# kenm-28/Semilayer-Wise-Mixed-Precision-Quantization

Hardware: NVIDIA B200
Metric: ResNet-50 mixed 8/4-bit images/s (higher is better)
Workload: dtype u8

## Files before the change

include/slq.h:

```cpp
#ifndef SLQ_H_
#define SLQ_H_

#include <stdint.h>

#ifdef __cplusplus
extern "C" {
#endif

#define SLQ_ABI_VERSION 1

#if defined(__GNUC__)
#define SLQ_API __attribute__((visibility("default")))
#else
#define SLQ_API
#endif

#define SLQ_OK 0
#define SLQ_ERR_INVALID 1
#define SLQ_ERR_CUDA 2
#define SLQ_ERR_ZERO_RANGE 3
#define SLQ_ERR_UNSUPPORTED 4

#define SLQ_ROW_OK 0
#define SLQ_ROW_ZERO_RANGE 1
#define SLQ_ROW_CODE_RANGE 2

#define SLQ_DIV_TRUE 0
#define SLQ_DIV_RECIP 1

SLQ_API const char *slq_last_error(void);
SLQ_API int slq_abi_version(void);
SLQ_API int slq_device_info(int32_t *sm_count, int32_t *cc_major, int32_t *cc_minor);


SLQ_API int64_t slq_packed_row_bytes(int64_t K, int32_t bit);

SLQ_API int slq_quantize_rows(float *w, int64_t n_rows, int64_t K, const int32_t *rows, const int32_t *bits,
                      int32_t n_jobs, int32_t div_mode, int32_t write_back, uint8_t *codes,
                      const int64_t *code_offsets, int32_t *z, float *s32, int32_t *status,
                      void *stream);

SLQ_API int slq_quantize_rows_host(float *w, int64_t n_rows, int64_t K, const int32_t *rows,
                           const int32_t *bits, int32_t n_jobs, int32_t div_mode, int32_t write_back,
                           uint8_t *codes, const int64_t *code_offsets, int32_t *z, float *s32,
                           int32_t *status);

typedef struct slq_qjob {
  float *row;
  uint8_t *codes;
  int32_t K;
  int32_t bit;
} slq_qjob;
SLQ_API int slq_quantize_jobs(const slq_qjob *jobs, int32_t n_small, int32_t n_mid, int32_t n_large,
                              int32_t div_mode, int32_t write_back, int32_t *z, float *s32, int32_t *status,
                              void *stream);

SLQ_API int slq_decode_rows(const uint8_t *codes, const int64_t *code_offsets, const int32_t *bit,
                            const int32_t *z, const float *s, int64_t n_rows, int64_t K, float *w, void *stream);

SLQ_API int slq_classify_rows(const float *w, int64_t n_rows, int64_t K, int32_t *bit, int32_t *z, float *s,
                      int32_t *exact, void *stream);

SLQ_API int slq_encode_rows(const float *w, int64_t n_rows, int64_t K, const int32_t *bit, const int32_t *z,
                    const float *s, uint8_t *codes, const int64_t *code_offsets, void *stream);


#define SLQ_IMPL_UMMA 0
#define SLQ_IMPL_SIMT 1

#define SLQ_A_AUTO 0
#define SLQ_A_IM2COL 1
#define SLQ_A_TILED 2

#define SLQ_OUT_U8 0
#define SLQ_OUT_F32 1
#define SLQ_OUT_ACC 2
#define SLQ_OUT_S8 3

typedef struct slq_conv_desc {
  int32_t N, H, W, Cin;
  int32_t Cout, kh, kw, stride, pad;
  int32_t w16;
  int32_t impl;
  int32_t a_mode;
} slq_conv_desc;

typedef struct slq_conv slq_conv;

SLQ_API int64_t slq_gemm_weight_rows(const slq_conv_desc *d);

SLQ_API int slq_build_gemm_weights(const slq_conv_desc *d, const uint8_t *codes, const int64_t *code_offsets,
                           const int32_t *bit, uint8_t *wg, void *stream);

SLQ_API int slq_conv_create(const slq_conv_desc *d, const uint8_t *in, const uint8_t *wg, slq_conv **out);

SLQ_API int slq_conv_tiling(const slq_conv_desc *d, int32_t *bn_cols, int32_t *n_tiles, int32_t *k_block,
                            int32_t *num_kb, int32_t *resident);
SLQ_API int slq_build_packed_gemm_weights(const slq_conv_desc *d, const uint8_t *codes, const int64_t *code_offsets,
                                          const int32_t *bit, const int64_t *tile_base, const int32_t *seg_bytes,
                                          const uint16_t *row_offsets, uint8_t *wgp, void *stream);
SLQ_API int slq_conv_set_packed_weights(slq_conv *c, const uint8_t *wgp, const int64_t *tile_base,
                                        const int32_t *seg_bytes, const uint16_t *row_offsets);
SLQ_API void slq_conv_destroy(slq_conv *c);

typedef struct slq_epilogue {
  const float *wscale;
  const float *zf;
  const float *bias;
  const float *act_scales;
  int32_t in_id, out_id, res_id;
  const uint8_t *res;
  int32_t res_signed;
  void *out;
  int32_t *out_S;
  int32_t out_mode;
  int32_t relu;
  const uint32_t *in_rowsum;
  uint32_t *out_rowsum;
  int32_t in_planes;
  int64_t in_plane_stride;
} slq_epilogue;

SLQ_API int slq_debug_set_trace(int64_t *buf, int32_t capacity_events);

SLQ_API int32_t slq_conv_rowsum_planes(const slq_conv *c, int32_t has_residual);
SLQ_API int32_t slq_conv_needs_rowsum(const slq_conv *c, int32_t has_residual);

SLQ_API int slq_conv_launch(slq_conv *c, const slq_epilogue *e, void *stream);

typedef struct slq_blocktail_desc {
  int32_t N, H, W, Cin;
  int32_t stride;
  int32_t Cmid;
  int32_t Cout;
  int32_t impl;
} slq_blocktail_desc;

typedef struct slq_blocktail slq_blocktail;

typedef struct slq_blocktail_epilogue {
  const float *wscale3, *zf3, *bias3;
  const float *wscaled, *zfd, *biasd;
  const float *act_scales;
  int32_t in3_id, ind_id, out_id;
  void *out;
  int32_t out_mode;
  uint32_t *out_rowsum;
} slq_blocktail_epilogue;

SLQ_API int slq_blocktail_create(const slq_blocktail_desc *d, const uint8_t *y2, const uint8_t *x, const uint8_t *wg3,
                                 const uint8_t *wgd, slq_blocktail **out);
SLQ_API void slq_blocktail_destroy(slq_blocktail *h);
SLQ_API int32_t slq_blocktail_rowsum_planes(const slq_blocktail *h);
SLQ_API int slq_blocktail_launch(slq_blocktail *h, const slq_blocktail_epilogue *e, void *stream);


SLQ_API int slq_stem_forward(const float *x, int32_t N, int32_t H, int32_t W, const float *w,
                     const float *bn_a, const float *bn_b, const float *act_scales, int32_t out_id,
                     float *scratch, void *out, int32_t out_mode, uint32_t *out_rowsum, void *stream);

typedef struct slq_stem slq_stem;
SLQ_API int64_t slq_stem_workspace_bytes(int32_t N, int32_t H, int32_t W);
SLQ_API int slq_stem_create(int32_t N, int32_t H, int32_t W, void *workspace, slq_stem **out);
SLQ_API void slq_stem_destroy(slq_stem *s);
SLQ_API int slq_stem_set_weights(slq_stem *s, const float *w, void *stream);
SLQ_API int slq_stem_launch(slq_stem *s, const float *x, const float *bn_a, const float *bn_b,
                            const float *act_scales, int32_t out_id, void *out, int32_t out_mode,
                            float *f32_scratch, uint32_t *out_rowsum, void *stream);
#define SLQ_IN_F32 0
#define SLQ_IN_F16 1
#define SLQ_IN_U8 2
SLQ_API int slq_stem_launch_in(slq_stem *s, const void *x, int32_t in_kind, const float *norm,
                               const float *bn_a, const float *bn_b, const float *act_scales, int32_t out_id,
                               void *out, int32_t out_mode, float *f32_scratch, uint32_t *out_rowsum, void *stream);

SLQ_API int64_t slq_tail_workspace_bytes(int32_t N, int32_t C, int32_t O);
SLQ_API int slq_tail_split_weights(const float *fc_w, int32_t O, int32_t C, float *fc_w_split, void *stream);
SLQ_API int slq_tail_forward(const uint8_t *x, int32_t N, int32_t HW, int32_t C, const float *act_scales,
                     int32_t in_id, const float *fc_w_split, const float *fc_b, int32_t O, float *workspace,
                     float *logits, void *stream);

SLQ_API int slq_absmax_scale(const float *y, int64_t n, float *act_scales, int32_t id, int32_t qmax,
                     uint32_t *tmp, void *stream);
SLQ_API int slq_quantize_act(const float *y, int64_t n, const float *act_scales, int32_t id,
                     int32_t is_signed, uint8_t *out, void *stream);


SLQ_API int slq_eval_tail(const float *logits, const int64_t *labels, int32_t B, int32_t C, float *probs_out,
                          const float *ref_probs, float *rows, double *accum, void *stream);
SLQ_API int slq_kl_rows(const float *p, const float *q, int32_t B, int32_t C, float *rows, double *accum,
                        void *stream);


SLQ_API int slq_probe_i8_peak(int32_t iters, int64_t *ops_out, void *stream);

#ifdef __cplusplus
}
#endif
#endif
```

semilayer-wise-mixed-precision-quantization_b200/csrc/block_tail.cu:

```cuda
#include <algorithm>
#include <new>

#include "conv_common.cuh"
#include "umma_ptx.cuh"

struct slq_blocktail {
  slq_blocktail_desc d;
  int Ho, Wo, swz, k3_blocks, kd_blocks, stages, smem_bytes, grid, n_tiles;
  long long M;
  const uint8_t *y2, *x, *wg3, *wgd;
  CUtensorMap tmA3, tmAd, tmB3, tmBd, tmO;
  const void *out_ptr;
};

namespace slq {

constexpr int kBtThreads = 640;
constexpr int kBtCrew = 512;
constexpr int kBtStage = 3;
constexpr int kBtN3 = 80;
constexpr int kBtNd = 144;
constexpr int kBtAccCols = 256;
constexpr int kBtMaxStages = 4;

struct BtArgs {
  long long M;
  int N, H, W, Ho, Wo, stride, Cin, Cmid, Cout;
  int k3_blocks, kd_blocks, stages, m_tiles, n_tiles, d_im2col;
  int b3_off, bd_off, ring_off, out_off, prm_off, bar_off;
  const float *wscale3, *zf3, *bias3, *wscaled, *zfd, *biasd, *act_scales;
  int in3_id, ind_id, out_id, out_mode;
  void *out;
  uint32_t *out_rowsum;
  long long *stats;
  int dbg;
};
#define BT_DBG(a) (kDebugTrace ? (a).dbg : 0)
__device__ __forceinline__ void bt_wait(uint32_t bar, uint32_t parity, long long *acc, bool on) {
  if (!kDebugTrace || !on) { mbar_wait(bar, parity); return; }
  const long long t0 = clock64();
  mbar_wait(bar, parity);
  *acc += clock64() - t0;
}

struct BtChan { float a3, z3, ad, zd, b; };
__host__ __device__ inline BtChan bt_chan(float wscale3, float zf3, float bias3, float wscaled, float zfd, float biasd,
                                          float s_y2, float s_x, float inv, bool quantised) {
  BtChan c;
#ifdef __CUDA_ARCH__
  c.a3 = __fmul_rn(wscale3, s_y2);
  c.ad = __fmul_rn(wscaled, s_x);
  c.b = __fadd_rn(bias3, biasd);
  if (quantised) { c.a3 = __fmul_rn(c.a3, inv); c.ad = __fmul_rn(c.ad, inv); c.b = __fmul_rn(c.b, inv); }
  c.z3 = __fmul_rn(zf3, c.a3);
  c.zd = __fmul_rn(zfd, c.ad);
#else
  c.a3 = wscale3 * s_y2; c.ad = wscaled * s_x; c.b = bias3 + biasd;
  if (quantised) { c.a3 *= inv; c.ad *= inv; c.b *= inv; }
  c.z3 = zf3 * c.a3; c.zd = zfd * c.ad;
#endif
  return c;
}

template <int SWZ, int OUT>
__global__ void __launch_bounds__(kBtThreads, 1)
block_tail_kernel(const __grid_constant__ CUtensorMap tmA3, const __grid_constant__ CUtensorMap tmAd,
                  const __grid_constant__ CUtensorMap tmB3, const __grid_constant__ CUtensorMap tmBd,
                  const __grid_constant__ CUtensorMap tmO, const BtArgs a) {
  extern __shared__ uint8_t smem_raw[];
  const uint32_t smem_base = (smem_u32(smem_raw) + 1023u) & ~1023u;
  uint8_t *smem = smem_raw + (smem_base - smem_u32(smem_raw));
  constexpr int kABytes = kTileM * SWZ;
  const uint32_t bar_base = smem_base + a.bar_off;
  auto full_bar = [&](int p, int s) { return bar_base + 8u * (p * 2 * kBtMaxStages + s); };
  auto empty_bar = [&](int p, int s) { return bar_base + 8u * (p * 2 * kBtMaxStages + kBtMaxStages + s); };
  auto tfull_bar = [&](int p) { return bar_base + 8u * (4 * kBtMaxStages + p); };
  auto tempty_bar = [&](int p) { return bar_base + 8u * (4 * kBtMaxStages + 2 + p); };
  const uint32_t bfull_bar = bar_base + 8u * (4 * kBtMaxStages + 4);
  volatile uint32_t *tmem_slot = reinterpret_cast<volatile uint32_t *>(smem + a.bar_off + 8 * (4 * kBtMaxStages + 5));
  const int warp = __shfl_sync(0xffffffffu, (int)(threadIdx.x >> 5), 0), lane = threadIdx.x & 31;

  const int per_n = (int)gridDim.x / a.n_tiles;
  const int my_n = (int)blockIdx.x % a.n_tiles;
  const int first_m = (int)blockIdx.x / a.n_tiles;
  const int count = first_m < a.m_tiles ? (a.m_tiles - first_m + per_n - 1) / per_n : 0;
  const int kb_tile = a.k3_blocks + a.kd_blocks;

  asm volatile("griddepcontrol.launch_dependents;" ::: "memory");
  if (warp == 0 && lane == 0) {
    prefetch_tmap(&tmA3); prefetch_tmap(&tmAd); prefetch_tmap(&tmB3); prefetch_tmap(&tmBd);
    if (OUT == SLQ_OUT_U8) prefetch_tmap(&tmO);
  }
  if (warp == 1 && lane == 0) {
    for (int p = 0; p < 2; ++p) {
      for (int s = 0; s < a.stages; ++s) { mbar_init(full_bar(p, s), 1); mbar_init(empty_bar(p, s), 1); }
      mbar_init(tfull_bar(p), 1);
      mbar_init(tempty_bar(p), kBtCrew / 32);
    }
    mbar_init(bfull_bar, 1);
    fence_barrier_init();
  }
  if (warp == 2) {
    asm volatile("tcgen05.alloc.cta_group::1.sync.aligned.shared::cta.b32 [%0], %1;" ::"r"(
                     smem_u32((const void *)tmem_slot)), "r"(512) : "memory");
    asm volatile("tcgen05.relinquish_alloc_permit.cta_group::1.sync.aligned;" ::: "memory");
  }
  for (int i = threadIdx.x; i < kb_tile * 16 * (SWZ / 16); i += blockDim.x) {
    const int t = i / (16 * (SWZ / 16)), rem = i % (16 * (SWZ / 16));
    const int row = rem / (SWZ / 16), chunk = rem % (SWZ / 16);
    const uint4 v = row == 0 ? make_uint4(0x01010101u, 0x01010101u, 0x01010101u, 0x01010101u) : make_uint4(0, 0, 0, 0);
    const int base = t < a.k3_blocks ? a.b3_off + t * (kBtN3 * SWZ) + 64 * SWZ
                                     : a.bd_off + (t - a.k3_blocks) * (kBtNd * SWZ) + 128 * SWZ;
    *reinterpret_cast<uint4 *>(smem + base + row * SWZ + chunk * 16) = v;
  }
  fence_proxy_async_smem();
  tc_fence_before();
  __syncthreads();
  tc_fence_after();
  const uint32_t tmem_base = *tmem_slot;

  if (warp == 0 || warp == 2) {
    const int p = warp >> 1;
    if (p == 0 && count > 0) {
      if (elect_one()) {
        mbar_expect_tx(bfull_bar, (uint32_t)(a.k3_blocks * 64 * SWZ + a.kd_blocks * 128 * SWZ));
        for (int kb = 0; kb < a.k3_blocks; ++kb)
          tma_load_2d(smem_base + a.b3_off + kb * (kBtN3 * SWZ), &tmB3, bfull_bar, kb * SWZ, my_n * 64);
        for (int kb = 0; kb < a.kd_blocks; ++kb)
          tma_load_2d(smem_base + a.bd_off + kb * (kBtNd * SWZ), &tmBd, bfull_bar, kb * SWZ, my_n * 128);
      }
      __syncwarp();
    }
    grid_dependency_wait();
    int c = 0;
    long long w_empty = 0;
    const bool st_on = kDebugTrace && a.stats != nullptr && blockIdx.x == 0;
    const long long t_begin = clock64();
    for (int i = p; i < count; i += 2) {
      const int m0 = (first_m + i * per_n) * kTileM;
      int dn = 0, dh = 0, dw = 0;
      if (a.d_im2col) {
        const int hw = a.Ho * a.Wo;
        dn = m0 / hw;
        const int rem = m0 - dn * hw, ph = rem / a.Wo;
        dh = ph * a.stride;
        dw = (rem - ph * a.Wo) * a.stride;
      }
      for (int kb = 0; kb < kb_tile; ++kb, ++c) {
        const int s = c % a.stages;
        bt_wait(empty_bar(p, s), (uint32_t)(((c / a.stages) & 1) ^ 1), &w_empty, st_on);
        if (elect_one()) {
          const uint32_t dst = smem_base + a.ring_off + (p * a.stages + s) * kABytes;
          mbar_expect_tx(full_bar(p, s), kABytes);
          if (kb < a.k3_blocks) tma_load_2d(dst, &tmA3, full_bar(p, s), kb * SWZ, m0);
          else if (a.d_im2col) tma_load_im2col_4d(dst, &tmAd, full_bar(p, s), (kb - a.k3_blocks) * SWZ, dw, dh, dn, 0, 0);
          else tma_load_2d(dst, &tmAd, full_bar(p, s), (kb - a.k3_blocks) * SWZ, m0);
        }
        __syncwarp();
      }
    }
    if (st_on && lane == 0) { a.stats[p] = w_empty; a.stats[2 + p] = clock64() - t_begin; }
  } else if (warp == 1 || warp == 3) {
    const int p = warp >> 1;
    const uint32_t tmem_u = __shfl_sync(0xffffffffu, tmem_base, 0) + p * kBtAccCols;
    const uint32_t idesc3 = (2u << 4) | ((uint32_t)(kBtN3 >> 3) << 17) | ((uint32_t)(kTileM >> 4) << 24);
    const uint32_t idescd = (2u << 4) | ((uint32_t)(kBtNd >> 3) << 17) | ((uint32_t)(kTileM >> 4) << 24);
    if (count > p) {
      mbar_wait(bfull_bar, 0);
      tc_fence_after();
    }
    int c = 0, t = 0;
    long long w_full = 0, w_tempty = 0;
    const bool st_on = kDebugTrace && a.stats != nullptr && blockIdx.x == 0;
    const long long t_begin = clock64();
    for (int i = p; i < count; i += 2, ++t) {
      if (t >= 1) bt_wait(tempty_bar(p), (uint32_t)((t - 1) & 1), &w_tempty, st_on);
      tc_fence_after();
      for (int kb = 0; kb < kb_tile; ++kb, ++c) {
        const int s = c % a.stages;
        bt_wait(full_bar(p, s), (uint32_t)((c / a.stages) & 1), &w_full, st_on);
        tc_fence_after();
        if (elect_one()) {
          const uint64_t da = make_smem_desc<SWZ>(smem_base + a.ring_off + (p * a.stages + s) * kABytes);
          const bool is3 = kb < a.k3_blocks;
          const uint64_t db = make_smem_desc<SWZ>(smem_base + (is3 ? a.b3_off + kb * (kBtN3 * SWZ)
                                                                   : a.bd_off + (kb - a.k3_blocks) * (kBtNd * SWZ)));
          const bool first = is3 ? kb == 0 : kb == a.k3_blocks;
#pragma unroll
          for (int k = 0; k < SWZ / 32 && !(!is3 && (BT_DBG(a) & 8)); ++k)
            umma_i8(tmem_u + (is3 ? 0 : kBtN3), da + 2 * k, db + 2 * k, is3 ? idesc3 : idescd, (uint32_t)(!first || k != 0));
          umma_commit(empty_bar(p, s));
          if (kb == kb_tile - 1) umma_commit(tfull_bar(p));
        }
        __syncwarp();
      }
    }
    if (st_on && lane == 0) { a.stats[4 + p] = w_full; a.stats[6 + p] = w_tempty; a.stats[8 + p] = clock64() - t_begin; }
  } else if (warp >= 4) {
    grid_dependency_wait();
    const int slice = (warp - 4) >> 2;
    const int wq = warp & 3;
    const int et = threadIdx.x - 128;
    const int row = wq * 32 + lane;
    constexpr bool kQuant = OUT == SLQ_OUT_U8;
    float *prm = reinterpret_cast<float *>(smem + a.prm_off);
    const uint32_t prm_s = smem_base + a.prm_off + (uint32_t)slice * 64;
    volatile uint32_t *rs_base = reinterpret_cast<volatile uint32_t *>(smem + a.prm_off + 5 * 64 * 4);
    const uint32_t row_byte = (uint32_t)(row * 64), row_sw = (uint32_t)((row >> 1) & 3);
    if (et < 64) {
      const int oc = my_n * 64 + et;
      const float inv = kQuant ? __fdiv_rn(1.0f, a.act_scales[a.out_id]) : 1.0f;
      const BtChan c = bt_chan(a.wscale3[oc], a.zf3[oc], a.bias3[oc], a.wscaled[oc], a.zfd[oc], a.biasd[oc],
                               a.act_scales[a.in3_id], a.act_scales[a.ind_id], inv, kQuant);
      prm[et] = c.a3; prm[64 + et] = c.z3; prm[128 + et] = c.ad; prm[192 + et] = c.zd; prm[256 + et] = c.b;
    }
    named_bar_sync(1, kBtCrew);
    const uint32_t tlane = tmem_base + ((uint32_t)(wq * 32) << 16);
    const int c0 = slice * 16;
    const bool want_rs = kQuant && a.out_rowsum != nullptr;
    long long w_tfull = 0, w_bar = 0, seg[6] = {0, 0, 0, 0, 0, 0}, tseg = 0;
#define BT_SEG(k) do { if (st_on) { const long long now__ = clock64(); seg[k] += now__ - tseg; tseg = now__; } } while (0)
    const bool st_on = kDebugTrace && a.stats != nullptr && blockIdx.x == 0 && et == 0;
    const long long t_begin = clock64();
    for (int i = 0; i < count; ++i) {
      const int p = i & 1, t = i >> 1;
      const int m_tile = first_m + i * per_n;
      const long long m = (long long)m_tile * kTileM + row;
      const bool valid = m < a.M;
      const uint32_t tcol = tlane + p * kBtAccCols;
      bt_wait(tfull_bar(p), (uint32_t)(t & 1), &w_tfull, st_on);
      if (st_on) tseg = clock64();
      tc_fence_after();
      uint32_t a3[16], lo[16], hi[16];
      tmem_ld16(tcol + c0, a3);
      if (!(BT_DBG(a) & 2)) {
        tmem_ld16(tcol + kBtN3 + c0, lo);
        tmem_ld16(tcol + kBtN3 + 64 + c0, hi);
      } else {
#pragma unroll
        for (int j = 0; j < 16; ++j) { lo[j] = a3[(j + 1) & 15]; hi[j] = a3[(j + 2) & 15]; }
      }
      const float S3 = (float)(int)tmem_ld1(tcol + 64);
      const float Sd = (float)(int)tmem_ld1(tcol + kBtN3 + 128);
      tmem_ld_wait();
      BT_SEG(0);
      tc_fence_before();
      __syncwarp();
      if (lane == 0) mbar_arrive(tempty_bar(p));
      BT_SEG(1);
      uint32_t pk[4];
      float *of = reinterpret_cast<float *>(a.out) + m * a.Cout + my_n * 64 + c0;
#pragma unroll
      for (int q4 = 0; q4 < 4; ++q4) {
        const uint32_t pofs = prm_s + (uint32_t)q4 * 16;
        uint4 pa3, pz3, pad, pzd, pb;
        if (!(BT_DBG(a) & 1)) {
          pa3 = lds128(pofs); pz3 = lds128(pofs + 256); pad = lds128(pofs + 512); pzd = lds128(pofs + 768); pb = lds128(pofs + 1024);
        } else {
          pa3 = pz3 = pad = pzd = pb = make_uint4(0x3a000000u + q4, 0x3a100000u, 0x3a200000u, 0x3a300000u);
        }
        const uint32_t va3[4] = {pa3.x, pa3.y, pa3.z, pa3.w}, vz3[4] = {pz3.x, pz3.y, pz3.z, pz3.w};
        const uint32_t vad[4] = {pad.x, pad.y, pad.z, pad.w}, vzd[4] = {pzd.x, pzd.y, pzd.z, pzd.w};
        const uint32_t vb[4] = {pb.x, pb.y, pb.z, pb.w};
        float v[4];
#pragma unroll
        for (int b = 0; b < 4; b += 2) {
          const int j = 4 * q4 + b;
          const float2 f3 = make_float2((float)(int)a3[j], (float)(int)a3[j + 1]);
          const float2 fd = ffma2(make_float2((float)(int)hi[j], (float)(int)hi[j + 1]), make_float2(256.0f, 256.0f),
                                  make_float2((float)(int)lo[j], (float)(int)lo[j + 1]));
          float2 y = ffma2(make_float2(S3, S3), make_float2(__uint_as_float(vz3[b]), __uint_as_float(vz3[b + 1])),
                           make_float2(__uint_as_float(vb[b]), __uint_as_float(vb[b + 1])));
          y = ffma2(make_float2(Sd, Sd), make_float2(__uint_as_float(vzd[b]), __uint_as_float(vzd[b + 1])), y);
          y = ffma2(f3, make_float2(__uint_as_float(va3[b]), __uint_as_float(va3[b + 1])), y);
          y = ffma2(fd, make_float2(__uint_as_float(vad[b]), __uint_as_float(vad[b + 1])), y);
          v[b] = y.x; v[b + 1] = y.y;
        }
        if (BT_DBG(a) & 32) { v[0] = __uint_as_float(a3[4 * q4] ^ lo[4 * q4]); v[1] = v[2] = v[3] = __uint_as_float(hi[4 * q4]); }
        if (!kQuant) {
          if (valid) reinterpret_cast<float4 *>(of)[q4] = make_float4(fmaxf(v[0], 0.f), fmaxf(v[1], 0.f), fmaxf(v[2], 0.f), fmaxf(v[3], 0.f));
        } else {
          pk[q4] = epi_pack4<false>(v[0], v[1], v[2], v[3]);
        }
      }
      if (kQuant) {
        const uint32_t stg = smem_base + a.out_off + (uint32_t)(i % kBtStage) * (kTileM * 64);
        if (!(BT_DBG(a) & 4)) sts128(stg + row_byte + (((uint32_t)slice ^ row_sw) << 4), make_uint4(pk[0], pk[1], pk[2], pk[3]));
        else if ((pk[0] ^ pk[1] ^ pk[2] ^ pk[3]) == 0x12345679u) sts128(stg, make_uint4(pk[0], pk[1], pk[2], pk[3]));
        uint32_t rsum = 0;
        volatile uint32_t *rs_scratch = rs_base + (i & 1) * 384;
        if (want_rs) {
          rsum = __dp4a(pk[0], 0x01010101u, __dp4a(pk[1], 0x01010101u, __dp4a(pk[2], 0x01010101u, __dp4a(pk[3], 0x01010101u, 0u))));
          if (slice != 0) rs_scratch[(slice - 1) * 128 + row] = rsum;
        }
        BT_SEG(2);
        fence_proxy_async_smem();
        BT_SEG(3);
        const long long tb0 = st_on ? clock64() : 0;
        named_bar_sync(1, kBtCrew);
        if (st_on) w_bar += clock64() - tb0;
        BT_SEG(4);
        if (et == 0 && !(BT_DBG(a) & 4)) {
          tma_store_2d(&tmO, stg, my_n * 64, m_tile * kTileM);
          tma_store_commit();
          asm volatile("cp.async.bulk.wait_group.read 1;" ::: "memory");
        }
        if (want_rs && slice == 0) {
          if (valid) a.out_rowsum[(long long)my_n * a.M + m] = rsum + rs_scratch[row] + rs_scratch[128 + row] + rs_scratch[256 + row];
        }
        BT_SEG(5);
      }
    }
    if (st_on) {
      a.stats[10] = w_tfull; a.stats[11] = w_bar; a.stats[12] = clock64() - t_begin; a.stats[13] = count;
      for (int k = 0; k < 6; ++k) a.stats[16 + k] = seg[k];
    }
    if (kQuant && et == 0) tma_store_wait_all();
  }
  tc_fence_before();
  __syncthreads();
  if (warp == 2) {
    tc_fence_after();
    asm volatile("tcgen05.dealloc.cta_group::1.sync.aligned.b32 %0, %1;" ::"r"(tmem_base), "r"(512) : "memory");
  }
}

__global__ void __launch_bounds__(128) block_tail_simt_kernel(BtArgs a, const uint8_t *__restrict__ y2,
                                                              const uint8_t *__restrict__ x,
                                                              const uint8_t *__restrict__ wg3,
                                                              const uint8_t *__restrict__ wgd) {
  const int oc = blockIdx.y * 32 + (threadIdx.x & 31);
  const long long m = (long long)blockIdx.x * 4 + (threadIdx.x >> 5);
  if (m >= a.M || oc >= a.Cout) return;
  const int wo = (int)(m % a.Wo), ho = (int)((m / a.Wo) % a.Ho), n = (int)(m / ((long long)a.Wo * a.Ho));
  unsigned acc3 = 0, S3 = 0, lo = 0, hi = 0, Sd = 0;
  const uint32_t *yp = reinterpret_cast<const uint32_t *>(y2 + m * a.Cmid);
  const uint32_t *w3 = reinterpret_cast<const uint32_t *>(wg3 + (long long)oc * a.Cmid);
  for (int c4 = 0; c4 < a.Cmid / 4; ++c4) {
    const uint32_t v = __ldg(yp + c4);
    acc3 = __dp4a(v, __ldg(w3 + c4), acc3);
    S3 = __dp4a(v, 0x01010101u, S3);
  }
  const uint32_t *xp = reinterpret_cast<const uint32_t *>(x + (((long long)n * a.H + ho * a.stride) * a.W + wo * a.stride) * a.Cin);
  const uint32_t *wl = reinterpret_cast<const uint32_t *>(wgd + (long long)gemm_row_of(oc, 0, 1) * a.Cin);
  const uint32_t *wh = reinterpret_cast<const uint32_t *>(wgd + (long long)gemm_row_of(oc, 1, 1) * a.Cin);
  for (int c4 = 0; c4 < a.Cin / 4; ++c4) {
    const uint32_t v = __ldg(xp + c4);
    lo = __dp4a(v, __ldg(wl + c4), lo);
    hi = __dp4a(v, __ldg(wh + c4), hi);
    Sd = __dp4a(v, 0x01010101u, Sd);
  }
  const bool quantised = a.out_mode == SLQ_OUT_U8;
  const float inv = quantised ? __fdiv_rn(1.0f, a.act_scales[a.out_id]) : 1.0f;
  const BtChan c = bt_chan(a.wscale3[oc], a.zf3[oc], a.bias3[oc], a.wscaled[oc], a.zfd[oc], a.biasd[oc],
                           a.act_scales[a.in3_id], a.act_scales[a.ind_id], inv, quantised);
  const float fd = __fmaf_rn((float)(int)hi, 256.0f, (float)(int)lo);
  float y = __fmaf_rn((float)(int)S3, c.z3, c.b);
  y = __fmaf_rn((float)(int)Sd, c.zd, y);
  y = __fmaf_rn((float)(int)acc3, c.a3, y);
  y = __fmaf_rn(fd, c.ad, y);
  if (quantised) reinterpret_cast<uint8_t *>(a.out)[m * a.Cout + oc] = (uint8_t)epi_quant_u8(y);
  else reinterpret_cast<float *>(a.out)[m * a.Cout + oc] = fmaxf(y, 0.f);
}

typedef CUresult (*BtEncodeTiledFn)(CUtensorMap *, CUtensorMapDataType, cuuint32_t, void *, const cuuint64_t *,
                                    const cuuint64_t *, const cuuint32_t *, const cuuint32_t *, CUtensorMapInterleave,
                                    CUtensorMapSwizzle, CUtensorMapL2promotion, CUtensorMapFloatOOBfill);
typedef CUresult (*BtEncodeIm2colFn)(CUtensorMap *, CUtensorMapDataType, cuuint32_t, void *, const cuuint64_t *,
                                     const cuuint64_t *, const int *, const int *, cuuint32_t, cuuint32_t,
                                     const cuuint32_t *, CUtensorMapInterleave, CUtensorMapSwizzle,
                                     CUtensorMapL2promotion, CUtensorMapFloatOOBfill);

static int bt_encoders(BtEncodeTiledFn *tiled, BtEncodeIm2colFn *im2col) {
  static BtEncodeTiledFn f_tiled = nullptr;
  static BtEncodeIm2colFn f_im2col = nullptr;
  if (!f_tiled || !f_im2col) {
    void *p = nullptr;
    cudaDriverEntryPointQueryResult qr;
    SLQ_CUDA(cudaGetDriverEntryPoint("cuTensorMapEncodeTiled", &p, cudaEnableDefault, &qr));
    SLQ_CHECK_ARG(qr == cudaDriverEntryPointSuccess && p, "cuTensorMapEncodeTiled not available from the driver");
    f_tiled = (BtEncodeTiledFn)p;
    p = nullptr;
    SLQ_CUDA(cudaGetDriverEntryPoint("cuTensorMapEncodeIm2col", &p, cudaEnableDefault, &qr));
    SLQ_CHECK_ARG(qr == cudaDriverEntryPointSuccess && p, "cuTensorMapEncodeIm2col not available from the driver");
    f_im2col = (BtEncodeIm2colFn)p;
  }
  *tiled = f_tiled;
  *im2col = f_im2col;
  return SLQ_OK;
}

static int bt_tiled_u8(CUtensorMap *tm, const void *ptr, long long rows, int cols, int box_cols, int box_rows,
                       CUtensorMapSwizzle sw, const char *what) {
  BtEncodeTiledFn enc;
  BtEncodeIm2colFn enc2;
  int rc = bt_encoders(&enc, &enc2);
  if (rc != SLQ_OK) return rc;
  cuuint64_t dims[2] = {(cuuint64_t)cols, (cuuint64_t)rows};
  cuuint64_t strides[1] = {(cuuint64_t)cols};
  cuuint32_t box[2] = {(cuuint32_t)box_cols, (cuuint32_t)box_rows};
  cuuint32_t es[2] = {1, 1};
  const CUresult r = enc(tm, CU_TENSOR_MAP_DATA_TYPE_UINT8, 2, const_cast<void *>(ptr), dims, strides, box, es,
                         CU_TENSOR_MAP_INTERLEAVE_NONE, sw, CU_TENSOR_MAP_L2_PROMOTION_L2_256B, CU_TENSOR_MAP_FLOAT_OOB_FILL_NONE);
  if (r != CUDA_SUCCESS) {
    set_error("cuTensorMapEncodeTiled(%s) failed: CUresult %d", what, (int)r);
    return SLQ_ERR_CUDA;
  }
  return SLQ_OK;
}

template <int SWZ, int OUT>
static int bt_launch(slq_blocktail *h, const BtArgs &a, cudaStream_t st) {
  static bool attr_done[kMaxDevices] = {false};
  const int dev = current_device();
  if (dev >= kMaxDevices || !attr_done[dev]) {
    SLQ_CUDA(cudaFuncSetAttribute(block_tail_kernel<SWZ, OUT>, cudaFuncAttributeMaxDynamicSharedMemorySize, 232448));
    if (dev < kMaxDevices) attr_done[dev] = true;
  }
  cudaLaunchConfig_t cfg = {};
  cfg.gridDim = dim3((unsigned)h->grid);
  cfg.blockDim = dim3(kBtThreads);
  cfg.dynamicSmemBytes = (size_t)h->smem_bytes;
  cfg.stream = st;
  cudaLaunchAttribute attr[1];
  attr[0].id = cudaLaunchAttributeProgrammaticStreamSerialization;
  attr[0].val.programmaticStreamSerializationAllowed = 1;
  cfg.attrs = attr;
  cfg.numAttrs = 1;
  SLQ_CUDA(cudaLaunchKernelEx(&cfg, block_tail_kernel<SWZ, OUT>, h->tmA3, h->tmAd, h->tmB3, h->tmBd, h->tmO, a));
  return SLQ_OK;
}

}

using namespace slq;

static int bt_plan(const slq_blocktail_desc *d, int swz, int *stages, int off[6]) {
  const int k3 = d->Cmid / swz, kd = d->Cin / swz;
  const int b3 = k3 * kBtN3 * swz, bd = kd * kBtNd * swz;
  const int fixed = b3 + bd + kBtStage * kTileM * 64 + (5 * 64 * 4 + 2 * 3 * 128 * 4) + 512 + 1024;
  const int a_bytes = kTileM * swz;
  int st = std::min(kBtMaxStages, (232448 - fixed) / (2 * a_bytes));
  if (st < 2) return -1;
  *stages = st;
  off[0] = 0;
  off[1] = b3;
  off[2] = b3 + bd;
  off[3] = off[2] + 2 * st * a_bytes;
  off[4] = off[3] + kBtStage * kTileM * 64;
  off[5] = off[4] + 5 * 64 * 4 + 2 * 3 * 128 * 4;
  return 1024 + off[5] + 512;
}

extern "C" int slq_blocktail_create(const slq_blocktail_desc *d, const uint8_t *y2, const uint8_t *x, const uint8_t *wg3,
                                    const uint8_t *wgd, slq_blocktail **out) {
  SLQ_CHECK_ARG(d && y2 && x && wg3 && wgd && out, "slq_blocktail_create: null pointer argument");
  SLQ_CHECK_ARG(d->N > 0 && d->H > 0 && d->W > 0 && (d->stride == 1 || d->stride == 2), "slq_blocktail_create: bad shape");
  SLQ_CHECK_ARG(d->Cin % 64 == 0 && d->Cmid % 64 == 0 && d->Cout % 64 == 0 && d->Cin > 0 && d->Cmid > 0 && d->Cout > 0,
                "slq_blocktail_create: channel counts must be multiples of 64");
  SLQ_CHECK_ARG(d->impl == SLQ_IMPL_UMMA || d->impl == SLQ_IMPL_SIMT, "slq_blocktail_create: impl %d", d->impl);
  const int swz = (d->Cmid % 128 == 0 && d->Cin % 128 == 0) ? 128 : 64;
  int stages = 0, off[6];
  const int smem = bt_plan(d, swz, &stages, off);
  if (smem < 0) {
    set_error("slq_blocktail_create: the weights of one n-tile (Cmid %d, Cin %d) do not fit in shared memory", d->Cmid, d->Cin);
    return SLQ_ERR_UNSUPPORTED;
  }
  slq_blocktail *h = new (std::nothrow) slq_blocktail();
  SLQ_CHECK_ARG(h != nullptr, "slq_blocktail_create: out of host memory");
  h->d = *d;
  h->Ho = (d->H - 1) / d->stride + 1;
  h->Wo = (d->W - 1) / d->stride + 1;
  h->M = (long long)d->N * h->Ho * h->Wo;
  h->swz = swz;
  h->k3_blocks = d->Cmid / swz;
  h->kd_blocks = d->Cin / swz;
  h->stages = stages;
  h->smem_bytes = smem;
  h->n_tiles = d->Cout / 64;
  h->y2 = y2; h->x = x; h->wg3 = wg3; h->wgd = wgd;
  h->out_ptr = nullptr;
  const long long m_tiles = ceil_div(h->M, kTileM);
  h->grid = (int)(std::min<long long>(std::max(sm_count() / h->n_tiles, 1), m_tiles)) * h->n_tiles;
  if (d->impl == SLQ_IMPL_UMMA) {
    const CUtensorMapSwizzle sw = swz == 128 ? CU_TENSOR_MAP_SWIZZLE_128B : CU_TENSOR_MAP_SWIZZLE_64B;
    int rc = bt_tiled_u8(&h->tmA3, y2, h->M, d->Cmid, swz, kTileM, sw, "y2");
    if (rc == SLQ_OK) rc = bt_tiled_u8(&h->tmB3, wg3, d->Cout, d->Cmid, swz, 64, sw, "W3");
    if (rc == SLQ_OK) rc = bt_tiled_u8(&h->tmBd, wgd, (long long)h->n_tiles * 128, d->Cin, swz, 128, sw, "Wd");
    if (rc == SLQ_OK) {
      if (d->stride == 1) {
        rc = bt_tiled_u8(&h->tmAd, x, h->M, d->Cin, swz, kTileM, sw, "x");
      } else {
        BtEncodeTiledFn enc;
        BtEncodeIm2colFn enc2;
        rc = bt_encoders(&enc, &enc2);
        if (rc == SLQ_OK) {
          cuuint64_t dims[4] = {(cuuint64_t)d->Cin, (cuuint64_t)d->W, (cuuint64_t)d->H, (cuuint64_t)d->N};
          cuuint64_t strides[3] = {(cuuint64_t)d->Cin, (cuuint64_t)d->W * d->Cin, (cuuint64_t)d->H * d->W * d->Cin};
          int lower[2] = {0, 0}, upper[2] = {0, 0};
          cuuint32_t es[4] = {1, (cuuint32_t)d->stride, (cuuint32_t)d->stride, 1};
          const CUresult r = enc2(&h->tmAd, CU_TENSOR_MAP_DATA_TYPE_UINT8, 4, const_cast<uint8_t *>(x), dims, strides, lower, upper,
                                  (cuuint32_t)swz, (cuuint32_t)kTileM, es, CU_TENSOR_MAP_INTERLEAVE_NONE, sw,
                                  CU_TENSOR_MAP_L2_PROMOTION_L2_256B, CU_TENSOR_MAP_FLOAT_OOB_FILL_NONE);
          if (r != CUDA_SUCCESS) {
            set_error("cuTensorMapEncodeIm2col(x) failed: CUresult %d", (int)r);
            rc = SLQ_ERR_CUDA;
          }
          int drv = 0;
          if (rc == SLQ_OK && cudaDriverGetVersion(&drv) == cudaSuccess && drv <= 13010 &&
              (long long)d->N * d->H * d->W * d->Cin < 131072)
            reinterpret_cast<uint64_t *>(&h->tmAd)[1] &= ~(1ull << 21);
        }
      }
    }
    if (rc != SLQ_OK) {
      delete h;
      return rc;
    }
    h->tmO = h->tmB3;
  }
  *out = h;
  return SLQ_OK;
}

extern "C" void slq_blocktail_destroy(slq_blocktail *h) { delete h; }

extern "C" int32_t slq_blocktail_rowsum_planes(const slq_blocktail *h) {
  return (h && h->d.impl == SLQ_IMPL_UMMA) ? h->n_tiles : 0;
}

extern "C" int slq_blocktail_launch(slq_blocktail *h, const slq_blocktail_epilogue *e, void *stream) {
  SLQ_CHECK_ARG(h && e, "slq_blocktail_launch: null handle/epilogue");
  SLQ_CHECK_ARG(e->wscale3 && e->zf3 && e->bias3 && e->wscaled && e->zfd && e->biasd && e->act_scales && e->out,
                "slq_blocktail_launch: epilogue vectors missing");
  SLQ_CHECK_ARG(e->out_mode == SLQ_OUT_U8 || e->out_mode == SLQ_OUT_F32, "slq_blocktail_launch: out_mode %d", e->out_mode);
  SLQ_CHECK_ARG(reinterpret_cast<uintptr_t>(e->out) % 16 == 0, "slq_blocktail_launch: out must be 16-byte aligned");
  const slq_blocktail_desc &d = h->d;
  BtArgs a{};
  a.M = h->M; a.N = d.N; a.H = d.H; a.W = d.W; a.Ho = h->Ho; a.Wo = h->Wo; a.stride = d.stride;
  a.Cin = d.Cin; a.Cmid = d.Cmid; a.Cout = d.Cout;
  a.k3_blocks = h->k3_blocks; a.kd_blocks = h->kd_blocks; a.stages = h->stages;
  a.m_tiles = (int)ceil_div(h->M, kTileM); a.n_tiles = h->n_tiles; a.d_im2col = d.stride != 1;
  a.wscale3 = e->wscale3; a.zf3 = e->zf3; a.bias3 = e->bias3; a.wscaled = e->wscaled; a.zfd = e->zfd; a.biasd = e->biasd;
  a.act_scales = e->act_scales; a.in3_id = e->in3_id; a.ind_id = e->ind_id; a.out_id = e->out_id; a.out_mode = e->out_mode;
  a.out = e->out; a.out_rowsum = e->out_mode == SLQ_OUT_U8 ? e->out_rowsum : nullptr;
  a.dbg = 0;
  a.stats = nullptr;
#if SLQ_DEBUG_TRACE
  {
    int cap = 0;
    debug_trace_buffer(&a.stats, &cap);
    if (cap > -16) a.stats = nullptr;
  }
  if (const char *d = getenv("SLQ_BT_DBG")) a.dbg = atoi(d);
#endif
  cudaStream_t st = (cudaStream_t)stream;
  if (d.impl == SLQ_IMPL_SIMT) {
    dim3 grid((unsigned)ceil_div(h->M, 4), (unsigned)ceil_div(d.Cout, 32));
    block_tail_simt_kernel<<<grid, 128, 0, st>>>(a, h->y2, h->x, h->wg3, h->wgd);
    SLQ_LAUNCH_CHECK();
    return SLQ_OK;
  }
  int stages = 0, off[6];
  bt_plan(&d, h->swz, &stages, off);
  a.b3_off = off[0]; a.bd_off = off[1]; a.ring_off = off[2]; a.out_off = off[3]; a.prm_off = off[4]; a.bar_off = off[5];
  if (e->out_mode == SLQ_OUT_U8 && h->out_ptr != e->out) {
    int rc = bt_tiled_u8(&h->tmO, e->out, h->M, d.Cout, 64, kTileM, CU_TENSOR_MAP_SWIZZLE_64B, "out");
    if (rc != SLQ_OK) return rc;
    h->out_ptr = e->out;
  }
  if (h->swz == 128)
    return e->out_mode == SLQ_OUT_U8 ? bt_launch<128, SLQ_OUT_U8>(h, a, st) : bt_launch<128, SLQ_OUT_F32>(h, a, st);
  return e->out_mode == SLQ_OUT_U8 ? bt_launch<64, SLQ_OUT_U8>(h, a, st) : bt_launch<64, SLQ_OUT_F32>(h, a, st);
}
```

semilayer-wise-mixed-precision-quantization_b200/csrc/conv_common.cuh:

```cuda
#pragma once
#include <cuda.h>

#include "common.cuh"
#include "epilogue.cuh"

namespace slq {

constexpr int kTileM = 128;

struct ConvGeom {
  int N, H, W, Cin, Cout, kh, kw, stride, pad;
  int Ho, Wo, w16;
  int bn_ch;
  int bn_cols;
  int n_tiles;
  int gemm_rows;
  long long M;
  int Ktot;
};

inline ConvGeom make_geom(const slq_conv_desc &d, int wide = 0) {
  ConvGeom g{};
  g.N = d.N; g.H = d.H; g.W = d.W; g.Cin = d.Cin; g.Cout = d.Cout;
  g.kh = d.kh; g.kw = d.kw; g.stride = d.stride; g.pad = d.pad; g.w16 = d.w16 ? 1 : 0;
  g.Ho = (d.H + 2 * d.pad - d.kh) / d.stride + 1;
  g.Wo = (d.W + 2 * d.pad - d.kw) / d.stride + 1;
  g.bn_ch = g.w16 ? 64 : (d.Cout > 64 ? 128 : 64);
  if (wide && !g.w16 && d.Cout % 256 == 0) g.bn_ch = 256;
  g.bn_cols = g.w16 ? 128 : g.bn_ch;
  g.n_tiles = (d.Cout + g.bn_ch - 1) / g.bn_ch;
  g.gemm_rows = g.n_tiles * g.bn_cols;
  g.M = (long long)d.N * g.Ho * g.Wo;
  g.Ktot = d.kh * d.kw * d.Cin;
  return g;
}

__host__ __device__ inline int gemm_row_of(int oc, int limb, int w16) {
  return w16 ? ((oc >> 6) * 128 + limb * 64 + (oc & 63)) : oc;
}

int validate_desc(const slq_conv_desc *d);

void debug_trace_buffer(long long **buf, int *cap);

int launch_conv_simt(const ConvGeom &g, const uint8_t *in, const uint8_t *wg, const EpiDev &e,
                     cudaStream_t st);

int launch_stem_pool(const float *y, int N, int Hc, int Wc, int Hp, int Wp, const float *act_scales,
                     int out_id, void *out, int out_mode, uint32_t *out_rowsum, cudaStream_t st);

}

struct slq_conv {
  slq_conv_desc desc;
  slq::ConvGeom g;
  slq::ConvGeom g_wide;
  int wide_ok;
  CUtensorMap tmB_wide;
  const uint8_t *wgp;
  const long long *wgp_tile;
  const int *wgp_seg;
  const uint16_t *wgp_rowoff;
  const uint8_t *in;
  const uint8_t *wg;
  int a_im2col;
  int swizzle;
  CUtensorMap tmA;
  CUtensorMap tmB;
  CUtensorMap tmO;
  CUtensorMap tmR;
  const void *out_ptr;
  const void *res_ptr;
  int num_ctas;
  int smem_bytes;
};
```

semilayer-wise-mixed-precision-quantization_b200/csrc/conv_umma.cu:

```cuda
#include <algorithm>
#include <cstdlib>
#include <new>

#include "conv_common.cuh"
#include "umma_ptx.cuh"

namespace slq {

constexpr int kThreads = 640;
constexpr int kTeam = 256;
inline int out_tile_bytes(const ConvGeom &g) {
#ifdef SLQ_OUT_TILE_16K
  return kTileM * 128;
#endif
  return kTileM * (g.bn_ch < 128 ? g.bn_ch : 128);
}

constexpr int kMaxStages = 8;
constexpr int kSmemLimit = 232448;

struct SmemPlan {
  int stages;
  int stage_bytes;
  int group;
  int a_bytes;
  int b_tile_bytes;
  int b_resident;
  int mma_warps;
  int b_off;
  int res_bufs;
  int out_bufs;
  int out_tile;
  int out_off, res_off, prm_off, bar_off;
  int total;
};

constexpr int kMaxResBufs = 4;
constexpr int kPrmBytes = 2 * 3 * 256 * 4 + 4 * 128 * 4;
constexpr int kMaxGroup = 4;

inline SmemPlan make_plan(const ConvGeom &g, int swz, bool has_res) {
  SmemPlan p{};
  p.a_bytes = kTileM * swz;
  const int kOutTileBytes = p.out_tile = out_tile_bytes(g);
  p.b_tile_bytes = (g.bn_cols + (g.bn_cols < 256 ? 16 : 0)) * swz;
  const int num_kb = g.Ktot / swz;
  const long long b_all = (long long)num_kb * p.b_tile_bytes;
#if SLQ_DEBUG_TRACE
  static const int force_group = getenv("SLQ_GROUP") ? atoi(getenv("SLQ_GROUP")) : 0;
  static const int force_mma = getenv("SLQ_MMA_WARPS") ? atoi(getenv("SLQ_MMA_WARPS")) : 0;
#else
  constexpr int force_group = 0, force_mma = 0;
#endif
  p.stages = 0;
  for (int rb = has_res ? kMaxResBufs : 0; g.bn_ch != 256 && p.stages == 0 && rb >= (has_res ? 2 : 0); rb -= 2) {
    const int fixed = (2 + rb) * kOutTileBytes + kPrmBytes + 512 + 1024;
    const long long room = (long long)kSmemLimit - fixed - b_all;
    for (int grp = std::min(kMaxGroup, num_kb); grp >= 1; --grp) {
      if (num_kb % grp != 0 || (force_group && grp > force_group)) continue;
      const int st = (int)std::min<long long>(kMaxStages, room / ((long long)grp * p.a_bytes)) & ~1;
      if (st >= (grp == 1 ? 4 : 4)) {
        p.b_resident = 1; p.group = grp; p.stages = st; p.stage_bytes = grp * p.a_bytes; p.res_bufs = rb; p.out_bufs = 2;
        const int st4 = (int)std::min<long long>(kMaxStages, (room - 2 * kOutTileBytes) / ((long long)grp * p.a_bytes)) & ~1;
        if (st4 >= st || (has_res && st4 >= 4)) { p.out_bufs = 4; p.stages = st4; }
        break;
      }
    }
    if (!has_res) break;
  }
  if (p.stages == 0) {
    p.res_bufs = has_res ? kMaxResBufs : 0;
    p.out_bufs = g.bn_ch == 256 ? 0 : 1;
    const int fixed = (p.out_bufs + p.res_bufs) * kOutTileBytes + kPrmBytes + 512 + 1024;
    p.b_resident = 0;
    p.group = 1;
    p.stage_bytes = p.a_bytes + p.b_tile_bytes;
    p.stages = std::min(kMaxStages, (kSmemLimit - fixed) / p.stage_bytes) & ~1;
  }
  p.mma_warps = force_mma ? force_mma : 2;
  p.b_off = p.stages * p.stage_bytes;
  p.out_off = p.b_off + (p.b_resident ? (int)b_all : 0);
  p.res_off = p.out_off + p.out_bufs * kOutTileBytes;
  p.prm_off = p.res_off + p.res_bufs * kOutTileBytes;
  p.bar_off = p.prm_off + kPrmBytes;
  p.total = 1024 + p.bar_off + 512;
  return p;
}

inline int plan_grid(const ConvGeom &g, const SmemPlan &p, int sms) {
  const long long m_tiles = (g.M + kTileM - 1) / kTileM;
  if (p.b_resident) {
    const int per_n = (int)std::min<long long>(std::max(sms / g.n_tiles, 1), m_tiles);
    return per_n * g.n_tiles;
  }
  return (int)std::min<long long>(m_tiles * g.n_tiles, sms);
}

struct KernelArgs {
  ConvGeom g;
  EpiDev e;
  SmemPlan sp;
  int a_im2col;
  int num_kb;
  int num_grp;
  int chunks_per_tap;
  int tma_out;
  int mma_warps_per_tile;
  int tile_alt;
  int acc_bufs, acc_stride;
  const uint8_t *wgp;
  const long long *wgp_tile;
  const int *wgp_seg;
  const uint16_t *wgp_rowoff;
  long long m_tiles;
  int half_b;
  long long *trace;
  int trace_cap;
};

constexpr int kTraceIssuers = 24;
__device__ __forceinline__ void mbar_wait_stat(uint32_t bar, uint32_t parity, long long &sum, bool stats) {
  if (!kDebugTrace || !stats) { mbar_wait(bar, parity); return; }
  const long long t0 = clock64();
  mbar_wait(bar, parity);
  sum += clock64() - t0;
}
__device__ __forceinline__ void trace_ev(const KernelArgs &a, int issuer, int &n, int ev, int idx) {
  if (!kDebugTrace || a.trace == nullptr || a.trace_cap < 0 || blockIdx.x != 0) return;
  const int per = a.trace_cap / kTraceIssuers;
  if (n < per) {
    long long *p = a.trace + 3LL * (issuer * per + n);
    p[0] = ev + 1;
    p[1] = idx;
    p[2] = clock64();
    ++n;
  }
}

struct TileWalk {
  int count, first_m, step_m;
  int first, step;
  int n_tiles, fixed_n, my_n;
  __device__ TileWalk(const KernelArgs &a) {
    n_tiles = a.g.n_tiles;
    fixed_n = a.sp.b_resident;
    const int m_tiles = (int)a.m_tiles;
    if (fixed_n) {
      const int per_n = (int)gridDim.x / n_tiles;
      my_n = (int)blockIdx.x % n_tiles;
      first_m = (int)blockIdx.x / n_tiles;
      step_m = per_n;
      count = first_m < m_tiles ? (m_tiles - first_m + per_n - 1) / per_n : 0;
      first = step = 0;
    } else {
      const int total = m_tiles * n_tiles;
      first = (int)blockIdx.x;
      step = (int)gridDim.x;
      count = first < total ? (total - first + step - 1) / step : 0;
      my_n = 0; first_m = step_m = 0;
    }
  }
  __device__ void at(int i, int &m_tile, int &n_tile) const {
    if (fixed_n) { n_tile = my_n; m_tile = first_m + i * step_m; }
    else { const int t = first + i * step; m_tile = t / n_tiles; n_tile = t - m_tile * n_tiles; }
  }
};

constexpr int kTileBars = 6;
constexpr int kTmemCols = 512;

__device__ __forceinline__ uint32_t stage_off(int r, int c, int bn_ch) {
  return bn_ch == 128 ? (uint32_t)(r * 128 + ((c ^ (r & 7)) << 4))
                      : (uint32_t)(r * 64 + ((c ^ ((r >> 1) & 3)) << 4));
}

__device__ __forceinline__ float2 res_pair(uint32_t w, int b, bool is_signed) {
  const uint32_t b0 = (w >> (8 * b)) & 255u, b1 = (w >> (8 * b + 8)) & 255u;
  if (is_signed) return make_float2((float)(int)(int8_t)b0, (float)(int)(int8_t)b1);
  if (b == 2) return make_float2((float)b0, (float)b1);
  const uint32_t m0 = __byte_perm(w, 0x4B000000u, 0x7440), m1 = __byte_perm(w, 0x4B000000u, 0x7441);
  return ffma2(make_float2(__uint_as_float(m0), __uint_as_float(m1)), make_float2(1.0f, 1.0f),
               make_float2(-8388608.0f, -8388608.0f));
}

constexpr int kResNone = 0, kResU8 = 1, kResS8 = 2, kResDyn = 3;
constexpr int kResWide = 4;

template <int SWZ, bool W16, int OUT, int RES>
__global__ void __launch_bounds__(kThreads, 1)
conv_umma_kernel(const __grid_constant__ CUtensorMap tmA, const __grid_constant__ CUtensorMap tmB,
                 const __grid_constant__ CUtensorMap tmO, const __grid_constant__ CUtensorMap tmR,
                 const KernelArgs a) {
  extern __shared__ uint8_t smem_raw[];
  const uint32_t smem_base = (smem_u32(smem_raw) + 1023u) & ~1023u;
  uint8_t *smem = smem_raw + (smem_base - smem_u32(smem_raw));
  const SmemPlan &sp = a.sp;
  const uint32_t bar_base = smem_base + sp.bar_off;
  auto full_bar = [&](int s) { return bar_base + 8u * s; };
  auto empty_bar = [&](int s) { return bar_base + 8u * (kMaxStages + s); };
  auto tfull_bar = [&](int b) { return bar_base + 8u * (2 * kMaxStages + b); };
  auto tempty_bar = [&](int b) { return bar_base + 8u * (2 * kMaxStages + kTileBars + b); };
  auto tstart_bar = [&](int b) { return bar_base + 8u * (2 * kMaxStages + 2 * kTileBars + b); };
  auto rfull_bar = [&](int b) { return bar_base + 8u * (2 * kMaxStages + 3 * kTileBars + b); };
  auto rempty_bar = [&](int b) { return bar_base + 8u * (2 * kMaxStages + 3 * kTileBars + kMaxResBufs + b); };
  const uint32_t bfull_bar = bar_base + 8u * (2 * kMaxStages + 3 * kTileBars + 2 * kMaxResBufs);
  auto stfree_bar = [&](int t) { return bar_base + 8u * (2 * kMaxStages + 3 * kTileBars + 2 * kMaxResBufs + 2 + t); };
  const uint32_t bready_bar = bar_base + 8u * (2 * kMaxStages + 3 * kTileBars + 2 * kMaxResBufs + 4);
  volatile uint32_t *tmem_slot = reinterpret_cast<volatile uint32_t *>(
      smem + sp.bar_off + 8 * (2 * kMaxStages + 3 * kTileBars + 2 * kMaxResBufs + 1));

  const int warp = __shfl_sync(0xffffffffu, (int)(threadIdx.x >> 5), 0), lane = threadIdx.x & 31;
  const ConvGeom &g = a.g;
  const EpiDev &e = a.e;
  const int bn_cols = g.bn_cols;
  const bool ones_row = bn_cols < 256;
  const int umma_n = bn_cols + (ones_row ? 16 : 0);
  constexpr bool kWide = RES == kResWide;
  const bool has_res = RES == kResDyn ? (e.res != nullptr) : (RES != kResNone && RES != kResWide);
  const TileWalk walk(a);

  asm volatile("griddepcontrol.launch_dependents;" ::: "memory");
  const long long t_entry = clock64();
  if (warp == 0 && lane == 0) {
    prefetch_tmap(&tmA);
    prefetch_tmap(&tmB);
    if (!kWide && a.tma_out) prefetch_tmap(&tmO);
    if (has_res) prefetch_tmap(&tmR);
  }
  if (warp == 1 && lane == 0) {
    for (int s = 0; s < sp.stages; ++s) {
      mbar_init(full_bar(s), 1);
      mbar_init(empty_bar(s), 1);
    }
    for (int b = 0; b < kTileBars; ++b) {
      mbar_init(tfull_bar(b), (uint32_t)a.mma_warps_per_tile);
      mbar_init(tempty_bar(b), kTeam / 32);
      mbar_init(tstart_bar(b), 1);
    }
    for (int b = 0; b < sp.res_bufs; ++b) {
      mbar_init(rfull_bar(b), 1);
      mbar_init(rempty_bar(b), kTeam / 32);
    }
    mbar_init(bfull_bar, 1);
    mbar_init(bready_bar, 2 * kTeam);
    mbar_init(stfree_bar(0), 1);
    mbar_init(stfree_bar(1), 1);
    fence_barrier_init();
  }
  if (warp == 2) {
    asm volatile("tcgen05.alloc.cta_group::1.sync.aligned.shared::cta.b32 [%0], %1;" ::"r"(
                     smem_u32((const void *)tmem_slot)),
                 "r"(kTmemCols)
                 : "memory");
    asm volatile("tcgen05.relinquish_alloc_permit.cta_group::1.sync.aligned;" ::: "memory");
  }
  if (ones_row) {
    const int b_tiles = sp.b_resident ? a.num_kb : sp.stages;
    const int b_stride = sp.b_resident ? sp.b_tile_bytes : sp.stage_bytes;
    const int b_first = sp.b_resident ? sp.b_off : sp.a_bytes;
    for (int i = threadIdx.x; i < b_tiles * 16 * (SWZ / 16); i += blockDim.x) {
      const int t = i / (16 * (SWZ / 16));
      const int rem = i % (16 * (SWZ / 16));
      const int row = rem / (SWZ / 16), chunk = rem % (SWZ / 16);
      uint4 v = row == 0 ? make_uint4(0x01010101u, 0x01010101u, 0x01010101u, 0x01010101u) : make_uint4(0, 0, 0, 0);
      *reinterpret_cast<uint4 *>(smem + b_first + t * b_stride + (bn_cols + row) * SWZ + chunk * 16) = v;
    }
  }
  fence_proxy_async_smem();
  tc_fence_before();
  __syncthreads();
  tc_fence_after();
  const uint32_t tmem_base = *tmem_slot;

  const int w_mma1 = sp.mma_warps == 2 ? 3 : -1;
  const int a_idx = warp == 0 ? 0 : (warp == 2 ? 1 : -1);
  if (a_idx >= 0) {
    const uint32_t b_bytes = (uint32_t)(bn_cols * SWZ);
    const int grp = sp.group;
    const uint32_t tx_bytes = (uint32_t)(grp * sp.a_bytes) + (sp.b_resident ? 0u : b_bytes);
    if (warp == 0 && sp.b_resident && walk.count > 0) {
      if (elect_one()) {
        if (a.wgp != nullptr) {
          const uint32_t seg = (uint32_t)a.wgp_seg[walk.my_n];
          const uint8_t *src = a.wgp + a.wgp_tile[walk.my_n];
          mbar_expect_tx(bfull_bar, seg * (uint32_t)a.num_kb);
          for (int kb = 0; kb < a.num_kb; ++kb)
            bulk_g2s(smem_base + sp.b_off + kb * sp.b_tile_bytes + bn_cols * SWZ - seg, src + (long long)kb * seg, seg, bfull_bar);
        } else {
          mbar_expect_tx(bfull_bar, b_bytes * (uint32_t)a.num_kb);
          for (int kb = 0; kb < a.num_kb; ++kb)
            tma_load_2d(smem_base + sp.b_off + kb * sp.b_tile_bytes, &tmB, bfull_bar, kb * SWZ, walk.my_n * bn_cols);
        }
      }
      __syncwarp();
    }
    grid_dependency_wait();
    const int ngrp = a.num_grp, cpt = a.chunks_per_tap;
    const int items = walk.count * ngrp;
    int tn = 0;
    const int tid_ = a_idx * 4;
    const int first = a_idx;
    constexpr int step = 2;
    int i = first / ngrp, gi = first - i * ngrp;
    int stage = first % sp.stages;
    uint32_t phase = (uint32_t)((first / sp.stages) & 1);
    uint32_t sa = smem_base + (uint32_t)(stage * sp.stage_bytes);
    const uint32_t sa_step = (uint32_t)(step * sp.stage_bytes), sa_end = smem_base + (uint32_t)(sp.stages * sp.stage_bytes);
    int cur_i = -1, n_tile = 0, m0 = 0, cw = 0, chh = 0, cn = 0;
    int kb0 = 0, tap_r = 0, tap_s = 0, cchunk = 0;
    const int kb_step = step * grp;
    const bool tracing = kDebugTrace && a.trace != nullptr && a.trace_cap >= 0;
    const bool stats = kDebugTrace && a.trace != nullptr && a.trace_cap < 0 && blockIdx.x == 0;
    long long wsum = 0;
    const long long tstart_clk = clock64();
    const bool im2col = a.a_im2col != 0, streamed = !sp.b_resident;
    const int kw = g.kw;
    const bool res_warp = has_res && warp == 0;
    const uint32_t res_bytes = (uint32_t)(kTileM * g.bn_ch);
    int res_next = 0, res_buf = 0;
    uint32_t res_ph = 0;
    auto issue_residuals = [&](int upto) {
      for (; res_next <= upto && res_next < walk.count; ++res_next) {
        int mt, nt;
        walk.at(res_next, mt, nt);
        mbar_wait(rempty_bar(res_buf), res_ph ^ 1);
        if (elect_one()) {
          mbar_expect_tx(rfull_bar(res_buf), res_bytes);
          tma_load_2d(smem_base + sp.res_off + res_buf * sp.out_tile, &tmR, rfull_bar(res_buf), nt * g.bn_ch,
                      mt * kTileM);
        }
        __syncwarp();
        if (++res_buf == sp.res_bufs) { res_buf = 0; res_ph ^= 1; }
      }
    };
    for (int c = first; c < items; c += step) {
      if (i != cur_i) {
        if (res_warp) issue_residuals(i + sp.res_bufs - 3);
        int m_tile;
        walk.at(i, m_tile, n_tile);
        m0 = m_tile * kTileM;
        kb0 = gi * grp;
        if (im2col) {
          const int hw = g.Wo * g.Ho;
          cn = m0 / hw;
          const int rem = m0 - cn * hw;
          const int p = rem / g.Wo;
          cw = (rem - p * g.Wo) * g.stride - g.pad;
          chh = p * g.stride - g.pad;
          const int tap = kb0 / cpt;
          cchunk = kb0 - tap * cpt;
          tap_r = tap / kw;
          tap_s = tap - tap_r * kw;
        }
        cur_i = i;
      }
      const uint32_t fb = full_bar(stage);
      mbar_wait_stat(empty_bar(stage), phase ^ 1, wsum, stats);
      if (tracing && lane == 0) trace_ev(a, tid_, tn, 0, c);
      const bool skip_b = kDebugTrace && a.half_b && (c & 2);
      if (elect_one()) {
        mbar_expect_tx(fb, skip_b ? tx_bytes - b_bytes : tx_bytes);
        if (im2col) {
          int cc = cchunk, ts = tap_s, tr = tap_r;
          for (int j = 0; j < grp; ++j) {
            tma_load_im2col_4d(sa + j * sp.a_bytes, &tmA, fb, cc * SWZ, cw, chh, cn, (uint16_t)ts, (uint16_t)tr);
            if (++cc == cpt) { cc = 0; if (++ts == kw) { ts = 0; ++tr; } }
          }
        } else {
          for (int j = 0; j < grp; ++j) tma_load_2d(sa + j * sp.a_bytes, &tmA, fb, (kb0 + j) * SWZ, m0);
        }
        if (streamed && !skip_b) tma_load_2d(sa + sp.a_bytes, &tmB, fb, kb0 * SWZ, n_tile * bn_cols);
      }
      __syncwarp();
      if (tracing && lane == 0) trace_ev(a, tid_, tn, 1, c);
      gi += step;
      kb0 += kb_step;
      if (gi >= ngrp) {
        do { gi -= ngrp; ++i; } while (gi >= ngrp);
      } else if (im2col) {
        cchunk += kb_step;
        while (cchunk >= cpt) { cchunk -= cpt; if (++tap_s == kw) { tap_s = 0; ++tap_r; } }
      }
      stage += step; sa += sa_step;
      if (stage >= sp.stages) { stage -= sp.stages; sa -= sa_end - smem_base; phase ^= 1; }
    }
    if (res_warp) issue_residuals(walk.count - 1);
    if (stats && lane == 0) { a.trace[a_idx] = wsum; a.trace[8 + a_idx] = clock64() - tstart_clk; if (a_idx == 0) a.trace[14] = tstart_clk - t_entry; }
  } else if (warp == 1 || warp == w_mma1) {
    const int w = warp == 1 ? 0 : 1;
    const int nmw = sp.mma_warps;
    const uint32_t idesc = (2u << 4) | ((uint32_t)(umma_n >> 3) << 17) | ((uint32_t)(kTileM >> 4) << 24);
    const uint32_t tmem_u = __shfl_sync(0xffffffffu, tmem_base, 0);
    const uint64_t desc_hi = make_smem_desc<SWZ>(0) & 0xffffffff00000000ull;
    const uint32_t desc_lo0 = (uint32_t)(make_smem_desc<SWZ>(0) & 0xffffffffull);
    const int n_stages = sp.stages, ngrp = a.num_grp, grp = sp.group;
    const int nw = a.mma_warps_per_tile;
    const uint32_t stage16 = (uint32_t)sp.stage_bytes >> 4, a16 = (uint32_t)sp.a_bytes >> 4;
    const uint32_t btile16 = (uint32_t)sp.b_tile_bytes >> 4;
    const uint32_t a_lo_first = desc_lo0 | ((smem_base & 0x3FFFFu) >> 4);
    const uint32_t b_lo_first = desc_lo0 | (((smem_base + (uint32_t)sp.b_off) & 0x3FFFFu) >> 4);
    const bool resident = sp.b_resident != 0;
    const bool tracing = kDebugTrace && a.trace != nullptr && a.trace_cap >= 0;
    const bool stats = kDebugTrace && a.trace != nullptr && a.trace_cap < 0 && blockIdx.x == 0;
    long long wfull = 0, wacc = 0;
    const long long tstart_clk = clock64();
    const int items = walk.count * ngrp;
    int tn = 0;
    if (resident && walk.count > 0) {
      mbar_wait(a.wgp != nullptr ? bready_bar : bfull_bar, 0);
      tc_fence_after();
    }
    const bool tile_alt = a.tile_alt != 0;
    int i = tile_alt ? w : w / ngrp, gi = tile_alt ? 0 : w - i * ngrp;
    int c0 = tile_alt ? w * ngrp : w;
    int stage = c0 % n_stages;
    uint32_t phase = (uint32_t)((c0 / n_stages) & 1);
    int cur_i = -1, acc = 0, tb = 0;
    for (int c = c0; c < items;) {
      if (i != cur_i) {
        cur_i = i;
        acc = i % a.acc_bufs;
        tb = i % kTileBars;
        if (gi == 0) {
          if (i >= a.acc_bufs) mbar_wait_stat(tempty_bar((i - a.acc_bufs) % kTileBars), (uint32_t)(((i - a.acc_bufs) / kTileBars) & 1), wacc, stats);
        } else {
          mbar_wait_stat(tstart_bar(tb), (uint32_t)((i / kTileBars) & 1), wacc, stats);
        }
        tc_fence_after();
      }
      const uint32_t tmem_d = tmem_u + acc * a.acc_stride;
      const uint32_t a_lo = a_lo_first + (uint32_t)stage * stage16;
      const uint32_t b_lo = resident ? b_lo_first + (uint32_t)(gi * grp) * btile16 : a_lo + a16;
      const bool last_mine = tile_alt ? gi + 1 == ngrp : gi + nmw >= ngrp;
      if (tracing && lane == 0) trace_ev(a, 16 + 3 * w, tn, 7, c);
      mbar_wait_stat(full_bar(stage), phase, wfull, stats);
      tc_fence_after();
      if (tracing && lane == 0) trace_ev(a, 16 + 3 * w, tn, 4, c);
      if (elect_one()) {
        for (int j = 0; j < grp; ++j) {
          const uint64_t da = desc_hi | (a_lo + (uint32_t)j * a16), db = desc_hi | (b_lo + (uint32_t)j * btile16);
#pragma unroll
          for (int k = 0; k < SWZ / 32; ++k)
            umma_i8(tmem_d, da + 2 * k, db + 2 * k, idesc, (uint32_t)(gi | j | k) != 0u);
        }
        umma_commit(empty_bar(stage));
        if (gi == 0 && nw > 1) umma_commit(tstart_bar(tb));
        if (last_mine) umma_commit(tfull_bar(tb));
      }
      __syncwarp();
      if (tile_alt) {
        int adv = 1;
        if (++gi == ngrp) { gi = 0; i += 2; adv += ngrp; }
        c += adv; stage += adv;
        while (stage >= n_stages) { stage -= n_stages; phase ^= 1; }
      } else {
        c += nmw;
        gi += nmw;
        while (gi >= ngrp) { gi -= ngrp; ++i; }
        stage += nmw;
        if (stage >= n_stages) { stage -= n_stages; phase ^= 1; }
      }
    }
    if (stats && lane == 0) { a.trace[2 + w] = wfull; a.trace[4 + w] = wacc; a.trace[10 + w] = clock64() - tstart_clk; }
  } else if (warp >= 4) {
    grid_dependency_wait();
    constexpr bool kQuant = OUT == SLQ_OUT_U8 || OUT == SLQ_OUT_S8;
    constexpr int CW = W16 ? 16 : 32;
    const int team = (warp - 4) >> 3;
    const int half = ((warp - 4) >> 2) & 1;
    const int wq = warp & 3;
    const int et = threadIdx.x - 128 - team * kTeam;
    const int row = wq * 32 + lane;
    float *prm = reinterpret_cast<float *>(smem + sp.prm_off) + team * 768;
    volatile uint32_t *rs_base = reinterpret_cast<volatile uint32_t *>(smem + sp.prm_off + 2 * 3072) + team * 256;
    const uint32_t prm_s = smem_base + sp.prm_off + team * 3072;
    const bool shared_stg = sp.out_bufs == 1;
    const bool dbl_stg = sp.out_bufs == 4;
    const uint32_t stg_base = smem_base + sp.out_off + (shared_stg ? 0 : team * (dbl_stg ? 2 : 1)) * sp.out_tile;
    float s_in = 1.f, s_res = 0.f, inv_out = 1.f;
    if (OUT != SLQ_OUT_ACC) {
      s_in = e.act_scales[e.in_id];
      if (kQuant) inv_out = __fdiv_rn(1.0f, e.act_scales[e.out_id]);
      if (has_res) s_res = kQuant ? __fmul_rn(e.act_scales[e.res_id], inv_out) : e.act_scales[e.res_id];
    }
    const bool res_signed = RES == kResDyn ? (e.res_signed != 0) : (RES == kResS8);
    const uint32_t row_byte = (uint32_t)(row * g.bn_ch);
    const uint32_t row_sw = g.bn_ch == 128 ? (uint32_t)(row & 7) : (uint32_t)((row >> 1) & 3);
    const int units = g.bn_ch / CW;
    const int u0 = half * (units >> 1), u1 = u0 + (units >> 1);
    int last_n_tile = -1;
    int tn = 0;
    long long wepi = 0;
    const long long tstart_clk = clock64();
    const bool same_grid = g.kh == 1 && g.stride == 1;
    const float inv_hw = __frcp_rn((float)(g.Ho * g.Wo)), inv_wo = __frcp_rn((float)g.Wo);
    auto window_sum = [&](int mm) -> uint32_t {
      if (mm >= g.M) return 0u;
      if (same_grid) {
        uint32_t sum = 0;
        for (int pl = 0; pl < e.in_planes; ++pl) sum += __ldg(e.in_rowsum + (long long)pl * e.in_plane_stride + mm);
        return sum;
      }
      const int hw = g.Ho * g.Wo;
      int n_img, rem, ho, wo;
      if (g.M < (1 << 24)) {
        n_img = (int)((float)mm * inv_hw);
        rem = mm - n_img * hw;
        if (rem < 0) { --n_img; rem += hw; } else if (rem >= hw) { ++n_img; rem -= hw; }
        ho = (int)((float)rem * inv_wo);
        wo = rem - ho * g.Wo;
        if (wo < 0) { --ho; wo += g.Wo; } else if (wo >= g.Wo) { ++ho; wo -= g.Wo; }
      } else {
        n_img = mm / hw; rem = mm - n_img * hw;
        ho = rem / g.Wo; wo = rem - ho * g.Wo;
      }
      uint32_t sum = 0;
      for (int pl = 0; pl < e.in_planes; ++pl) {
        const uint32_t *rs = e.in_rowsum + (long long)pl * e.in_plane_stride + (long long)n_img * g.H * g.W;
        if (g.kh == 1) { sum += __ldg(rs + (ho * g.stride) * g.W + wo * g.stride); continue; }
        const int h0 = ho * g.stride - g.pad, w0 = wo * g.stride - g.pad;
#pragma unroll
        for (int r = 0; r < 3; ++r) {
          const int hi = h0 + r;
          if (hi < 0 || hi >= g.H) continue;
#pragma unroll
          for (int q = 0; q < 3; ++q) {
            const int wi = w0 + q;
            if (wi >= 0 && wi < g.W) sum += __ldg(rs + hi * g.W + wi);
          }
        }
      }
      return sum;
    };
    if (a.wgp != nullptr && sp.b_resident && walk.count > 0) {
      const int tid = threadIdx.x - 128;
      constexpr int kChunks = SWZ / 16;
      const int n_chunks = bn_cols * kChunks;
      const uint32_t seg = (uint32_t)a.wgp_seg[walk.my_n];
      const uint16_t *rowoff = a.wgp_rowoff + (long long)walk.my_n * (bn_cols + 1);
      uint32_t src_off[4], src_len[4];
#pragma unroll
      for (int j = 0; j < 4; ++j) {
        const int idx = tid + 512 * j;
        src_off[j] = 0; src_len[j] = 0;
        if (idx < n_chunks) {
          const int r = idx / kChunks, c = idx % kChunks;
          const uint32_t o0 = rowoff[r], o1 = rowoff[r + 1];
          const bool half = (o1 - o0) == (uint32_t)(SWZ / 2);
          src_len[j] = half ? 8u : 16u;
          src_off[j] = o0 + (uint32_t)c * src_len[j];
        }
      }
      mbar_wait(bfull_bar, 0);
      for (int kb = 0; kb < a.num_kb; ++kb) {
        const uint32_t tile_s = smem_base + sp.b_off + kb * sp.b_tile_bytes;
        const uint32_t raw_s = tile_s + (uint32_t)(bn_cols * SWZ) - seg;
        uint4 v[4];
#pragma unroll
        for (int j = 0; j < 4; ++j) {
          if (src_len[j] == 16u) v[j] = lds128(raw_s + src_off[j]);
          else if (src_len[j] == 8u) {
            uint2 w;
            asm volatile("ld.shared.v2.u32 {%0, %1}, [%2];" : "=r"(w.x), "=r"(w.y) : "r"(raw_s + src_off[j]));
            const uint32_t l0 = w.x & 0x0f0f0f0fu, h0 = (w.x >> 4) & 0x0f0f0f0fu;
            const uint32_t l1 = w.y & 0x0f0f0f0fu, h1 = (w.y >> 4) & 0x0f0f0f0fu;
            v[j] = make_uint4(__byte_perm(l0, h0, 0x5140), __byte_perm(l0, h0, 0x7362), __byte_perm(l1, h1, 0x5140),
                              __byte_perm(l1, h1, 0x7362));
          }
        }
        named_bar_sync(3, 2 * kTeam);
#pragma unroll
        for (int j = 0; j < 4; ++j) {
          const int idx = tid + 512 * j;
          if (src_len[j] != 0u) {
            const int r = idx / kChunks, c = idx % kChunks;
            const uint32_t sw = SWZ == 128 ? (uint32_t)(c ^ (r & 7)) : (uint32_t)(c ^ ((r >> 1) & 3));
            sts128(tile_s + (uint32_t)r * SWZ + (sw << 4), v[j]);
          }
        }
      }
      fence_proxy_async_smem();
      mbar_arrive(bready_bar);
    }
    const bool seg_on = kDebugTrace && a.trace != nullptr && a.trace_cap < 0 && blockIdx.x == 0 && warp == 4;
    long long seg_t = 0, seg_sum[6] = {0, 0, 0, 0, 0, 0};
    auto seg = [&](int k) {
      if (seg_on) { const long long t = clock64(); seg_sum[k] += t - seg_t; seg_t = t; }
    };
    if (seg_on) seg_t = clock64();
    uint32_t S_next = 0;
    if (!ones_row && team < walk.count) {
      int mt0, nt0;
      walk.at(team, mt0, nt0);
      S_next = window_sum(mt0 * kTileM + row);
    }
    for (int it = team; it < walk.count; it += 2) {
      int m_tile, n_tile;
      walk.at(it, m_tile, n_tile);
      const int acc = it % a.acc_bufs, tb = it % kTileBars;
      const uint32_t ph = (uint32_t)((it / kTileBars) & 1);
      const uint32_t stg = stg_base + (dbl_stg ? (uint32_t)((it >> 1) & 1) * sp.out_tile : 0u);
      volatile uint32_t *rs_scratch = rs_base + ((it >> 1) & 1) * 128;
      if ((!dbl_stg && (kWide || a.tma_out)) || (n_tile != last_n_tile && OUT != SLQ_OUT_ACC)) {
        if (!kWide && a.tma_out && et == 0 && !dbl_stg) tma_store_wait_read();
        named_bar_sync(1 + team, kTeam);
      }
      if (n_tile != last_n_tile && OUT != SLQ_OUT_ACC) {
        if (et < g.bn_ch) {
          const int oc = n_tile * g.bn_ch + et;
          ChanParam p = {0.f, 0.f, 0.f, 0.f};
          if (oc < g.Cout) p = make_chan_param(e.wscale[oc], e.zf[oc], e.bias[oc], s_in, inv_out, kQuant);
          prm[et] = p.wsc; prm[256 + et] = p.zw; prm[512 + et] = p.bias;
        }
        last_n_tile = n_tile;
        named_bar_sync(1 + team, kTeam);
      }
      const long long m = (long long)m_tile * kTileM + row;
      const bool valid = m < g.M;
      uint32_t S_raw = S_next;
      if (!ones_row && it + 2 < walk.count) {
        int mt2, nt2;
        walk.at(it + 2, mt2, nt2);
        S_next = window_sum(mt2 * kTileM + row);
      }
      seg(0);
      mbar_wait_stat(tfull_bar(tb), ph, wepi, kDebugTrace && a.trace != nullptr && a.trace_cap < 0 && blockIdx.x == 0);
      tc_fence_after();
      seg(1);
      if (kDebugTrace && a.trace != nullptr && et == 0) trace_ev(a, 17 + team, tn, 5, (int)it);
      const int rbuf = has_res ? (int)(it % sp.res_bufs) : 0;
      const uint32_t rsb = smem_base + sp.res_off + rbuf * sp.out_tile;
      if (has_res) mbar_wait(rfull_bar(rbuf), (uint32_t)((it / sp.res_bufs) & 1));
      const uint32_t trow = tmem_base + ((uint32_t)(wq * 32) << 16) + acc * a.acc_stride;
      if (ones_row) {
        S_raw = tmem_ld1(trow + bn_cols);
        tmem_ld_wait();
      }
      seg(2);
      const float Sf = (float)S_raw;
      uint32_t rsum = 0;
      const bool want_rs_any = e.out_rowsum != nullptr;
      if (OUT == SLQ_OUT_ACC && e.out_S && valid && n_tile == 0 && half == 0) e.out_S[m] = (int)S_raw;
      for (int u = u0; u < u1; ++u) {
        uint32_t lo[CW], hi[CW];
        tmem_ld<CW>(trow + u * CW, lo);
        if constexpr (W16) tmem_ld<CW>(trow + 64 + u * CW, hi);
        uint32_t rw[CW / 4];
        if (has_res) {
#pragma unroll
          for (int i = 0; i < CW / 16; ++i) {
            const uint4 r = lds128(rsb + row_byte + ((((uint32_t)(u * (CW / 16) + i)) ^ row_sw) << 4));
            rw[4 * i] = r.x; rw[4 * i + 1] = r.y; rw[4 * i + 2] = r.z; rw[4 * i + 3] = r.w;
          }
        }
        tmem_ld_wait();
        const int cb = n_tile * g.bn_ch + u * CW;
        if (OUT == SLQ_OUT_ACC) {
          if (!valid || cb >= g.Cout) continue;
          const long long ld = (long long)(W16 ? 2 : 1) * g.Cout;
          int4 *o = reinterpret_cast<int4 *>(reinterpret_cast<int32_t *>(e.out) + m * ld + cb);
#pragma unroll
          for (int j = 0; j < CW / 4; ++j) o[j] = make_int4(lo[4 * j], lo[4 * j + 1], lo[4 * j + 2], lo[4 * j + 3]);
          if (W16) {
            int4 *oh = reinterpret_cast<int4 *>(reinterpret_cast<int32_t *>(e.out) + m * ld + g.Cout + cb);
#pragma unroll
            for (int j = 0; j < CW / 4; ++j) oh[j] = make_int4(hi[4 * j], hi[4 * j + 1], hi[4 * j + 2], hi[4 * j + 3]);
          }
          continue;
        }
        const bool store_ok = valid && cb < g.Cout;
        float4 *of = reinterpret_cast<float4 *>(reinterpret_cast<float *>(e.out) + m * g.Cout + cb);
        uint32_t pk[CW / 4];
        const float2 S2 = make_float2(Sf, Sf), R2 = make_float2(s_res, s_res);
#pragma unroll
        for (int q4 = 0; q4 < CW / 4; ++q4) {
          float v[4];
          const uint32_t pofs = prm_s + (uint32_t)(u * CW + 4 * q4) * 4;
          const uint4 pa = lds128(pofs), pz = lds128(pofs + 1024), pb = lds128(pofs + 2048);
          const uint32_t pav[4] = {pa.x, pa.y, pa.z, pa.w}, pzv[4] = {pz.x, pz.y, pz.z, pz.w}, pbv[4] = {pb.x, pb.y, pb.z, pb.w};
#pragma unroll
          for (int b = 0; b < 4; b += 2) {
            const int j = 4 * q4 + b;
            float2 accf = make_float2((float)(int)lo[j], (float)(int)lo[j + 1]);
            if (W16) accf = ffma2(make_float2((float)(int)hi[j], (float)(int)hi[j + 1]), make_float2(256.0f, 256.0f), accf);
            const float2 c2 = ffma2(S2, make_float2(__uint_as_float(pzv[b]), __uint_as_float(pzv[b + 1])),
                                    make_float2(__uint_as_float(pbv[b]), __uint_as_float(pbv[b + 1])));
            float2 y = ffma2(accf, make_float2(__uint_as_float(pav[b]), __uint_as_float(pav[b + 1])), c2);
            if (has_res) {
              y = ffma2(res_pair(rw[q4], b, res_signed), R2, y);
            }
            v[b] = y.x; v[b + 1] = y.y;
          }
          if (!kQuant) {
            if (e.relu) {
#pragma unroll
              for (int b = 0; b < 4; ++b) v[b] = fmaxf(v[b], 0.f);
            }
            if (store_ok) of[q4] = make_float4(v[0], v[1], v[2], v[3]);
          } else {
            pk[q4] = epi_pack4<OUT == SLQ_OUT_S8>(v[0], v[1], v[2], v[3]);
          }
        }
        if (OUT == SLQ_OUT_U8 && want_rs_any) {
#pragma unroll
          for (int q4 = 0; q4 < CW / 4; ++q4) rsum = __dp4a(pk[q4], 0x01010101u, rsum);
        }
        if (kQuant) {
          if (!kWide && a.tma_out) {
            if (shared_stg && u == u0 && it >= 1) mbar_wait(stfree_bar(team ^ 1), (uint32_t)(((it - 1) >> 1) & 1));
#pragma unroll
            for (int i = 0; i < CW / 16; ++i)
              sts128(stg + row_byte + ((((uint32_t)(u * (CW / 16) + i)) ^ row_sw) << 4),
                     make_uint4(pk[4 * i], pk[4 * i + 1], pk[4 * i + 2], pk[4 * i + 3]));
          } else if (store_ok) {
            uint4 *o = reinterpret_cast<uint4 *>(reinterpret_cast<uint8_t *>(e.out) + m * g.Cout + cb);
#pragma unroll
            for (int i = 0; i < CW / 16; ++i) o[i] = make_uint4(pk[4 * i], pk[4 * i + 1], pk[4 * i + 2], pk[4 * i + 3]);
          }
        }
      }
      seg(3);
      const bool want_rs = OUT == SLQ_OUT_U8 && e.out_rowsum != nullptr;
      if (want_rs && half == 1) rs_scratch[row] = rsum;
      tc_fence_before();
      if (kDebugTrace && a.trace != nullptr && et == 0) trace_ev(a, 17 + team, tn, 6, (int)it);
      __syncwarp();
      if (lane == 0) {
        mbar_arrive(tempty_bar(tb));
        if (has_res) mbar_arrive(rempty_bar(rbuf));
      }
      if (kWide || !a.tma_out) {
        if (want_rs) named_bar_sync(1 + team, kTeam);
      } else {
        fence_proxy_async_smem();
        if (dbl_stg && et == 0) tma_store_wait_read();
        named_bar_sync(1 + team, kTeam);
        if (et == 0) {
          tma_store_2d(&tmO, stg, n_tile * g.bn_ch, (int)(m_tile * kTileM));
          tma_store_commit();
          if (shared_stg) {
            tma_store_wait_read();
            mbar_arrive(stfree_bar(team));
          }
        }
      }
      seg(4);
      if (OUT == SLQ_OUT_U8 && e.out_rowsum != nullptr && half == 0 && valid)
        e.out_rowsum[(long long)n_tile * g.M + m] = rsum + rs_scratch[row];
      seg(5);
    }
    if (seg_on && lane == 0) {
      for (int k = 0; k < 6; ++k) a.trace[56 + k] = seg_sum[k];
      a.trace[62] = (walk.count + 1 - team) / 2;
    }
    if (!kWide && a.tma_out && et == 0) tma_store_wait_all();
    if (kDebugTrace && a.trace != nullptr && a.trace_cap < 0 && blockIdx.x == 0 && et == 0) { a.trace[6 + team] = wepi; a.trace[12 + team] = clock64() - tstart_clk; }
  }

  tc_fence_before();
  __syncthreads();
  if (kDebugTrace && a.trace != nullptr && a.trace_cap < 0 && threadIdx.x == 0) {
    if (blockIdx.x == 0) a.trace[15] = clock64() - t_entry;
    if (blockIdx.x < 32) a.trace[16 + blockIdx.x] = clock64() - t_entry;
    if (blockIdx.x >= gridDim.x - 8) a.trace[48 + blockIdx.x - (gridDim.x - 8)] = clock64() - t_entry;
  }
  if (warp == 2) {
    tc_fence_after();
    asm volatile("tcgen05.dealloc.cta_group::1.sync.aligned.b32 %0, %1;" ::"r"(tmem_base), "r"(kTmemCols) : "memory");
  }
}

typedef CUresult (*EncodeTiledFn)(CUtensorMap *, CUtensorMapDataType, cuuint32_t, void *, const cuuint64_t *,
                                  const cuuint64_t *, const cuuint32_t *, const cuuint32_t *,
                                  CUtensorMapInterleave, CUtensorMapSwizzle, CUtensorMapL2promotion,
                                  CUtensorMapFloatOOBfill);
typedef CUresult (*EncodeIm2colFn)(CUtensorMap *, CUtensorMapDataType, cuuint32_t, void *, const cuuint64_t *,
                                   const cuuint64_t *, const int *, const int *, cuuint32_t, cuuint32_t,
                                   const cuuint32_t *, CUtensorMapInterleave, CUtensorMapSwizzle,
                                   CUtensorMapL2promotion, CUtensorMapFloatOOBfill);

static int get_encoders(EncodeTiledFn *tiled, EncodeIm2colFn *im2col) {
  static EncodeTiledFn f_tiled = nullptr;
  static EncodeIm2colFn f_im2col = nullptr;
  if (!f_tiled || !f_im2col) {
    void *p = nullptr;
    cudaDriverEntryPointQueryResult qr;
    SLQ_CUDA(cudaGetDriverEntryPoint("cuTensorMapEncodeTiled", &p, cudaEnableDefault, &qr));
    if (qr != cudaDriverEntryPointSuccess || !p) {
      set_error("cuTensorMapEncodeTiled not available from the driver");
      return SLQ_ERR_CUDA;
    }
    f_tiled = (EncodeTiledFn)p;
    p = nullptr;
    SLQ_CUDA(cudaGetDriverEntryPoint("cuTensorMapEncodeIm2col", &p, cudaEnableDefault, &qr));
    if (qr != cudaDriverEntryPointSuccess || !p) {
      set_error("cuTensorMapEncodeIm2col not available from the driver");
      return SLQ_ERR_CUDA;
    }
    f_im2col = (EncodeIm2colFn)p;
  }
  *tiled = f_tiled;
  *im2col = f_im2col;
  return SLQ_OK;
}

static int encode_out_map(CUtensorMap *tm, const void *ptr, const ConvGeom &g, const char *what) {
  EncodeTiledFn enc_tiled;
  EncodeIm2colFn enc_im2col;
  int rc = get_encoders(&enc_tiled, &enc_im2col);
  if (rc != SLQ_OK) return rc;
  cuuint64_t dims[2] = {(cuuint64_t)g.Cout, (cuuint64_t)g.M};
  cuuint64_t strides[1] = {(cuuint64_t)g.Cout};
  cuuint32_t box[2] = {(cuuint32_t)g.bn_ch, (cuuint32_t)kTileM};
  cuuint32_t es[2] = {1, 1};
  CUresult r = enc_tiled(tm, CU_TENSOR_MAP_DATA_TYPE_UINT8, 2, const_cast<void *>(ptr), dims, strides, box, es,
                         CU_TENSOR_MAP_INTERLEAVE_NONE,
                         g.bn_ch == 128 ? CU_TENSOR_MAP_SWIZZLE_128B : CU_TENSOR_MAP_SWIZZLE_64B,
                         CU_TENSOR_MAP_L2_PROMOTION_L2_256B, CU_TENSOR_MAP_FLOAT_OOB_FILL_NONE);
  if (r != CUDA_SUCCESS) {
    set_error("cuTensorMapEncodeTiled(%s) failed: CUresult %d", what, (int)r);
    return SLQ_ERR_CUDA;
  }
  return SLQ_OK;
}

static int build_tensor_maps(slq_conv *c) {
  EncodeTiledFn enc_tiled;
  EncodeIm2colFn enc_im2col;
  int rc = get_encoders(&enc_tiled, &enc_im2col);
  if (rc != SLQ_OK) return rc;
  const ConvGeom &g = c->g;
  const int swz = c->swizzle;
  const CUtensorMapSwizzle sw = swz == 128 ? CU_TENSOR_MAP_SWIZZLE_128B : CU_TENSOR_MAP_SWIZZLE_64B;
  CUresult r;
  for (int wide = 0; wide <= (c->wide_ok ? 1 : 0); ++wide) {
    const ConvGeom &gb = wide ? c->g_wide : c->g;
    cuuint64_t dims[2] = {(cuuint64_t)gb.Ktot, (cuuint64_t)gb.gemm_rows};
    cuuint64_t strides[1] = {(cuuint64_t)gb.Ktot};
    cuuint32_t box[2] = {(cuuint32_t)swz, (cuuint32_t)gb.bn_cols};
    cuuint32_t es[2] = {1, 1};
    r = enc_tiled(wide ? &c->tmB_wide : &c->tmB, CU_TENSOR_MAP_DATA_TYPE_UINT8, 2, (void *)c->wg, dims, strides, box, es,
                  CU_TENSOR_MAP_INTERLEAVE_NONE, sw, CU_TENSOR_MAP_L2_PROMOTION_L2_256B,
                  CU_TENSOR_MAP_FLOAT_OOB_FILL_NONE);
    if (r != CUDA_SUCCESS) {
      set_error("cuTensorMapEncodeTiled(B) failed: CUresult %d", (int)r);
      return SLQ_ERR_CUDA;
    }
  }
  if (!c->a_im2col) {
    cuuint64_t dims[2] = {(cuuint64_t)g.Cin, (cuuint64_t)g.M};
    cuuint64_t strides[1] = {(cuuint64_t)g.Cin};
    cuuint32_t box[2] = {(cuuint32_t)swz, (cuuint32_t)kTileM};
    cuuint32_t es[2] = {1, 1};
    r = enc_tiled(&c->tmA, CU_TENSOR_MAP_DATA_TYPE_UINT8, 2, (void *)c->in, dims, strides, box, es,
                  CU_TENSOR_MAP_INTERLEAVE_NONE, sw, CU_TENSOR_MAP_L2_PROMOTION_L2_256B,
                  CU_TENSOR_MAP_FLOAT_OOB_FILL_NONE);
    if (r != CUDA_SUCCESS) {
      set_error("cuTensorMapEncodeTiled(A) failed: CUresult %d", (int)r);
      return SLQ_ERR_CUDA;
    }
  } else {
    cuuint64_t dims[4] = {(cuuint64_t)g.Cin, (cuuint64_t)g.W, (cuuint64_t)g.H, (cuuint64_t)g.N};
    cuuint64_t strides[3] = {(cuuint64_t)g.Cin, (cuuint64_t)g.W * g.Cin, (cuuint64_t)g.H * g.W * g.Cin};
    int lower[2] = {-g.pad, -g.pad};
    int upper[2] = {g.pad - (g.kw - 1), g.pad - (g.kh - 1)};
    cuuint32_t es[4] = {1, (cuuint32_t)g.stride, (cuuint32_t)g.stride, 1};
    r = enc_im2col(&c->tmA, CU_TENSOR_MAP_DATA_TYPE_UINT8, 4, (void *)c->in, dims, strides, lower, upper,
                   (cuuint32_t)swz, (cuuint32_t)kTileM, es, CU_TENSOR_MAP_INTERLEAVE_NONE, sw,
                   CU_TENSOR_MAP_L2_PROMOTION_L2_256B, CU_TENSOR_MAP_FLOAT_OOB_FILL_NONE);
    if (r != CUDA_SUCCESS) {
      set_error("cuTensorMapEncodeIm2col(A) failed: CUresult %d", (int)r);
      return SLQ_ERR_CUDA;
    }
    int drv = 0;
    if (cudaDriverGetVersion(&drv) == cudaSuccess && drv <= 13010 &&
        (long long)g.N * g.H * g.W * g.Cin < 131072)
      reinterpret_cast<uint64_t *>(&c->tmA)[1] &= ~(1ull << 21);
  }
  return SLQ_OK;
}

static long long *g_trace = nullptr;
static int g_trace_cap = 0;
void debug_trace_buffer(long long **buf, int *cap) { *buf = g_trace; *cap = g_trace_cap; }

template <int SWZ, bool W16, int OUT, int RES>
static int launch_one(slq_conv *c, const EpiDev &e, int tma_out, cudaStream_t st) {
  static bool attr_done[kMaxDevices] = {false};
  const int dev = current_device();
  if (dev >= kMaxDevices || !attr_done[dev]) {
    SLQ_CUDA(cudaFuncSetAttribute(conv_umma_kernel<SWZ, W16, OUT, RES>,
                                  cudaFuncAttributeMaxDynamicSharedMemorySize, kSmemLimit));
    if (dev < kMaxDevices) attr_done[dev] = true;
  }
  const bool wide = c->wide_ok && e.res == nullptr && !W16;
  const ConvGeom &geom = wide ? c->g_wide : c->g;
  KernelArgs a;
  a.g = geom;
  a.e = e;
  a.sp = make_plan(geom, SWZ, e.res != nullptr);
  a.acc_bufs = wide ? 2 : 3;
  a.acc_stride = wide ? 256 : 160;
  const bool packed = c->wgp != nullptr && a.sp.b_resident && !W16 && !wide;
  a.wgp = packed ? c->wgp : nullptr;
  a.wgp_tile = c->wgp_tile; a.wgp_seg = c->wgp_seg; a.wgp_rowoff = c->wgp_rowoff;
  if (wide) tma_out = 0;
  const int grid = plan_grid(geom, a.sp, sm_count());
  a.trace = g_trace;
  a.trace_cap = g_trace_cap;
  a.half_b = 0;
#if SLQ_DEBUG_TRACE
  a.half_b = getenv("SLQ_HALF_B") != nullptr;
#endif
  a.a_im2col = c->a_im2col;
  a.chunks_per_tap = geom.Cin / SWZ;
  a.num_kb = geom.kh * geom.kw * a.chunks_per_tap;
  a.num_grp = a.num_kb / a.sp.group;
  a.tile_alt = (a.sp.mma_warps == 2 && a.num_grp >= 2 && a.sp.stages % (2 * a.num_grp) == 0) ? 1 : 0;
  a.mma_warps_per_tile = (a.sp.mma_warps == 2 && a.num_grp >= 2 && !a.tile_alt) ? 2 : 1;
  a.m_tiles = ceil_div(geom.M, kTileM);
  a.tma_out = tma_out;
  const bool pdl = true;
  cudaLaunchConfig_t cfg = {};
  cfg.gridDim = dim3((unsigned)grid);
  cfg.blockDim = dim3(kThreads);
  cfg.dynamicSmemBytes = (size_t)a.sp.total;
  cfg.stream = st;
  cudaLaunchAttribute attr[1];
  attr[0].id = cudaLaunchAttributeProgrammaticStreamSerialization;
  attr[0].val.programmaticStreamSerializationAllowed = 1;
  cfg.attrs = attr;
  cfg.numAttrs = pdl ? 1 : 0;
  SLQ_CUDA(cudaLaunchKernelEx(&cfg, conv_umma_kernel<SWZ, W16, OUT, RES>, c->tmA, wide ? c->tmB_wide : c->tmB, c->tmO,
                              c->tmR, a));
  return SLQ_OK;
}

template <int SWZ, bool W16>
static int launch_umma(slq_conv *c, const EpiDev &e, int tma_out, cudaStream_t st) {
  const int res = e.res == nullptr ? kResNone : (e.res_signed ? kResS8 : kResU8);
  if constexpr (SWZ == 128 && !W16) {
    if (c->wide_ok && res == kResNone) {
      if (e.out_mode == SLQ_OUT_U8) return launch_one<SWZ, W16, SLQ_OUT_U8, kResWide>(c, e, 0, st);
      if (e.out_mode == SLQ_OUT_S8) return launch_one<SWZ, W16, SLQ_OUT_S8, kResWide>(c, e, 0, st);
    }
  }
  switch (e.out_mode) {
    case SLQ_OUT_U8:
      if (res == kResNone) return launch_one<SWZ, W16, SLQ_OUT_U8, kResNone>(c, e, tma_out, st);
      if (res == kResU8) return launch_one<SWZ, W16, SLQ_OUT_U8, kResU8>(c, e, tma_out, st);
      return launch_one<SWZ, W16, SLQ_OUT_U8, kResS8>(c, e, tma_out, st);
    case SLQ_OUT_S8:
      if (res == kResNone) return launch_one<SWZ, W16, SLQ_OUT_S8, kResNone>(c, e, tma_out, st);
      if (res == kResU8) return launch_one<SWZ, W16, SLQ_OUT_S8, kResU8>(c, e, tma_out, st);
      return launch_one<SWZ, W16, SLQ_OUT_S8, kResS8>(c, e, tma_out, st);
    case SLQ_OUT_F32:
      return launch_one<SWZ, W16, SLQ_OUT_F32, kResDyn>(c, e, tma_out, st);
    default:
      return launch_one<SWZ, W16, SLQ_OUT_ACC, kResNone>(c, e, tma_out, st);
  }
}

}

using namespace slq;

extern "C" int slq_conv_create(const slq_conv_desc *d, const uint8_t *in, const uint8_t *wg, slq_conv **out) {
  int rc = validate_desc(d);
  if (rc != SLQ_OK) return rc;
  SLQ_CHECK_ARG(in && wg && out, "slq_conv_create: null pointer argument");
  SLQ_CHECK_ARG(d->impl == SLQ_IMPL_UMMA || d->impl == SLQ_IMPL_SIMT, "slq_conv_create: impl %d", d->impl);
  SLQ_CHECK_ARG(reinterpret_cast<uintptr_t>(in) % 16 == 0 && reinterpret_cast<uintptr_t>(wg) % 16 == 0,
                "slq_conv_create: buffers must be 16-byte aligned");
  slq_conv *c = new (std::nothrow) slq_conv();
  SLQ_CHECK_ARG(c != nullptr, "slq_conv_create: out of host memory");
  c->desc = *d;
  c->g = make_geom(*d);
  if (c->g.M > 0x7fff0000LL) {
    delete c;
    set_error("slq_conv_create: more than 2^31 output pixels");
    return SLQ_ERR_UNSUPPORTED;
  }
  c->in = in;
  c->wg = wg;
  c->swizzle = (d->Cin % 128 == 0) ? 128 : 64;
  c->g_wide = make_geom(*d, 1);
  c->wide_ok = (d->impl == SLQ_IMPL_UMMA && c->g_wide.bn_ch == 256 && c->swizzle == 128 &&
                !make_plan(c->g, c->swizzle, false).b_resident) ? 1 : 0;
#if SLQ_DEBUG_TRACE
  if (getenv("SLQ_NO_WIDE")) c->wide_ok = 0;
#endif
  c->out_ptr = nullptr;
  c->res_ptr = nullptr;
  c->wgp = nullptr; c->wgp_tile = nullptr; c->wgp_seg = nullptr; c->wgp_rowoff = nullptr;
  const bool can_tile = d->kh == 1 && d->kw == 1 && d->stride == 1 && d->pad == 0;
  if (d->a_mode == SLQ_A_TILED && !can_tile) {
    delete c;
    set_error("slq_conv_create: SLQ_A_TILED needs a 1x1 stride-1 layer");
    return SLQ_ERR_INVALID;
  }
  c->a_im2col = (d->a_mode == SLQ_A_IM2COL) ? 1 : (d->a_mode == SLQ_A_TILED ? 0 : (can_tile ? 0 : 1));
  if (d->impl == SLQ_IMPL_UMMA) {
    if (d->Cout % 64 != 0) {
      delete c;
      set_error("slq_conv_create: the tcgen05 path needs Cout %% 64 == 0 (got %d)", d->Cout);
      return SLQ_ERR_UNSUPPORTED;
    }
    rc = build_tensor_maps(c);
    if (rc != SLQ_OK) {
      delete c;
      return rc;
    }
    c->tmO = c->tmB;
    c->tmR = c->tmB;
    const long long tiles = ceil_div(c->g.M, kTileM) * c->g.n_tiles;
    c->num_ctas = (int)std::min<long long>(tiles, sm_count());
    c->smem_bytes = make_plan(c->g, c->swizzle, true).total;
  }
  *out = c;
  return SLQ_OK;
}

extern "C" void slq_conv_destroy(slq_conv *c) { delete c; }

extern "C" int slq_debug_set_trace(int64_t *buf, int32_t capacity_events) {
  if (!kDebugTrace && buf != nullptr) {
    set_error("slq_debug_set_trace: this library was built without SLQ_DEBUG_TRACE (python slq_build.py --debug)");
    return SLQ_ERR_UNSUPPORTED;
  }
  g_trace = reinterpret_cast<long long *>(buf);
  g_trace_cap = buf ? capacity_events : 0;
  return SLQ_OK;
}

extern "C" int slq_conv_launch(slq_conv *c, const slq_epilogue *ep, void *stream) {
  SLQ_CHECK_ARG(c && ep, "slq_conv_launch: null handle/epilogue");
  SLQ_CHECK_ARG(ep->out != nullptr, "slq_conv_launch: out is NULL");
  SLQ_CHECK_ARG(ep->out_mode >= SLQ_OUT_U8 && ep->out_mode <= SLQ_OUT_S8, "slq_conv_launch: out_mode %d", ep->out_mode);
  if (ep->out_mode != SLQ_OUT_ACC) {
    SLQ_CHECK_ARG(ep->wscale && ep->zf && ep->bias && ep->act_scales, "slq_conv_launch: epilogue vectors missing");
    SLQ_CHECK_ARG(!ep->res || ep->res_id >= 0, "slq_conv_launch: residual without res_id");
  }
  SLQ_CHECK_ARG(reinterpret_cast<uintptr_t>(ep->out) % 16 == 0 &&
                    (!ep->res || reinterpret_cast<uintptr_t>(ep->res) % 16 == 0),
                "slq_conv_launch: out/res must be 16-byte aligned");
  EpiDev e;
  e.wscale = ep->wscale; e.zf = ep->zf; e.bias = ep->bias; e.act_scales = ep->act_scales;
  e.in_rowsum = ep->in_rowsum; e.out_rowsum = ep->out_rowsum;
  e.in_planes = ep->in_planes; e.in_plane_stride = ep->in_plane_stride;
  e.res = ep->out_mode == SLQ_OUT_ACC ? nullptr : ep->res;
  e.out = ep->out; e.out_S = ep->out_S;
  e.in_id = ep->in_id; e.out_id = ep->out_id; e.res_id = ep->res_id;
  e.out_mode = ep->out_mode; e.relu = ep->relu; e.res_signed = ep->res_signed;
  e.Cout = c->g.Cout; e.w16 = c->g.w16; e.M = c->g.M;
  cudaStream_t st = (cudaStream_t)stream;
  if (c->desc.impl == SLQ_IMPL_SIMT) return launch_conv_simt(c->g, c->in, c->wg, e, st);
  const bool wide_launch = c->wide_ok && ep->res == nullptr && !c->g.w16;
  SLQ_CHECK_ARG(!wide_launch || (ep->in_rowsum != nullptr && ep->in_planes >= 1 &&
                                 ep->in_plane_stride >= (int64_t)c->g.N * c->g.H * c->g.W),
                "slq_conv_launch: this layer runs 256-channel tiles and needs in_rowsum (per-pixel channel sums of its "
                "input: planes, plane stride; slq_conv_needs_rowsum)");
  const int tma_out = (ep->out_mode == SLQ_OUT_U8 || ep->out_mode == SLQ_OUT_S8) ? 1 : 0;
  if (tma_out && c->out_ptr != ep->out) {
    int rc = encode_out_map(&c->tmO, ep->out, c->g, "out");
    if (rc != SLQ_OK) return rc;
    c->out_ptr = ep->out;
  }
  if (e.res && c->res_ptr != e.res) {
    int rc = encode_out_map(&c->tmR, e.res, c->g, "residual");
    if (rc != SLQ_OK) return rc;
    c->res_ptr = e.res;
  }
  if (c->swizzle == 128)
    return c->g.w16 ? launch_umma<128, true>(c, e, tma_out, st) : launch_umma<128, false>(c, e, tma_out, st);
  return c->g.w16 ? launch_umma<64, true>(c, e, tma_out, st) : launch_umma<64, false>(c, e, tma_out, st);
}

extern "C" int slq_conv_tiling(const slq_conv_desc *d, int32_t *bn_cols, int32_t *n_tiles, int32_t *k_block,
                               int32_t *num_kb, int32_t *resident) {
  int rc = validate_desc(d);
  if (rc != SLQ_OK) return rc;
  const ConvGeom g = make_geom(*d);
  const int swz = (d->Cin % 128 == 0) ? 128 : 64;
  if (bn_cols) *bn_cols = g.bn_cols;
  if (n_tiles) *n_tiles = g.n_tiles;
  if (k_block) *k_block = swz;
  if (num_kb) *num_kb = g.Ktot / swz;
  if (resident) *resident = (make_plan(g, swz, true).b_resident && make_plan(g, swz, false).b_resident && !g.w16) ? 1 : 0;
  return SLQ_OK;
}

extern "C" int slq_conv_set_packed_weights(slq_conv *c, const uint8_t *wgp, const int64_t *tile_base,
                                           const int32_t *seg_bytes, const uint16_t *row_offsets) {
  SLQ_CHECK_ARG(c != nullptr, "slq_conv_set_packed_weights: null handle");
  SLQ_CHECK_ARG(wgp == nullptr || (tile_base && seg_bytes && row_offsets), "slq_conv_set_packed_weights: layout tables missing");
  SLQ_CHECK_ARG(reinterpret_cast<uintptr_t>(wgp) % 16 == 0, "slq_conv_set_packed_weights: wgp must be 16-byte aligned");
  c->wgp = wgp;
  c->wgp_tile = reinterpret_cast<const long long *>(tile_base);
  c->wgp_seg = seg_bytes;
  c->wgp_rowoff = row_offsets;
  return SLQ_OK;
}

extern "C" int32_t slq_conv_needs_rowsum(const slq_conv *c, int32_t has_residual) {
  if (!c || c->desc.impl != SLQ_IMPL_UMMA) return 0;
  return (c->wide_ok && !has_residual && !c->g.w16) ? 1 : 0;
}

extern "C" int32_t slq_conv_rowsum_planes(const slq_conv *c, int32_t has_residual) {
  if (!c) return -1;
  if (c->desc.impl != SLQ_IMPL_UMMA) return 0;
  return (c->wide_ok && !has_residual && !c->g.w16) ? c->g_wide.n_tiles : c->g.n_tiles;
}
```

semilayer-wise-mixed-precision-quantization_b200/csrc/epilogue.cuh:

```cuda
#pragma once
#include <cstdint>

#include "slq.h"

namespace slq {

struct EpiDev {
  const float *wscale, *zf, *bias, *act_scales;
  const uint8_t *res;
  void *out;
  int32_t *out_S;
  const uint32_t *in_rowsum;
  uint32_t *out_rowsum;
  int in_planes;
  long long in_plane_stride;
  int in_id, out_id, res_id;
  int out_mode, relu, res_signed;
  int Cout, w16;
  long long M;
};

struct ChanParam {
  float wsc, zw, bias, pad;
};

__device__ __forceinline__ ChanParam make_chan_param(float wscale, float zf, float bias, float s_in,
                                                     float inv_out, bool quantised) {
  ChanParam p;
  p.wsc = __fmul_rn(wscale, s_in);
  p.zw = __fmul_rn(zf, p.wsc);
  p.bias = bias;
  p.pad = 0.f;
  if (quantised) {
    p.wsc = __fmul_rn(p.wsc, inv_out);
    p.zw = __fmul_rn(p.zw, inv_out);
    p.bias = __fmul_rn(p.bias, inv_out);
  }
  return p;
}

template <bool W16>
__device__ __forceinline__ float epi_value(int acc_lo, int acc_hi, float Sf, const ChanParam &p) {
  float accf = (float)acc_lo;
  if (W16) accf = __fmaf_rn((float)acc_hi, 256.0f, accf);
  const float c2 = __fmaf_rn(Sf, p.zw, p.bias);
  return __fmaf_rn(accf, p.wsc, c2);
}

__device__ __forceinline__ float epi_add_res(float y, uint32_t res_byte, bool res_signed, float s_res) {
  const float r = res_signed ? (float)(int)(int8_t)res_byte : (float)res_byte;
  return __fmaf_rn(r, s_res, y);
}

__device__ __forceinline__ float2 ffma2(float2 a, float2 b, float2 c) {
#ifdef SLQ_NO_FFMA2
  return make_float2(__fmaf_rn(a.x, b.x, c.x), __fmaf_rn(a.y, b.y, c.y));
#endif
  uint64_t ra, rb, rc, rd;
  asm("mov.b64 %0, {%1, %2};" : "=l"(ra) : "f"(a.x), "f"(a.y));
  asm("mov.b64 %0, {%1, %2};" : "=l"(rb) : "f"(b.x), "f"(b.y));
  asm("mov.b64 %0, {%1, %2};" : "=l"(rc) : "f"(c.x), "f"(c.y));
  asm("fma.rn.f32x2 %0, %1, %2, %3;" : "=l"(rd) : "l"(ra), "l"(rb), "l"(rc));
  float2 d;
  asm("mov.b64 {%0, %1}, %2;" : "=f"(d.x), "=f"(d.y) : "l"(rd));
  return d;
}

__device__ __forceinline__ uint32_t epi_quant_u8(float y) {
  uint32_t q;
  asm("cvt.rni.sat.u8.f32 %0, %1;" : "=r"(q) : "f"(y));
  return q;
}
__device__ __forceinline__ uint32_t epi_quant_s8(float y) {
  int q;
  asm("cvt.rni.sat.s8.f32 %0, %1;" : "=r"(q) : "f"(y));
  return (uint32_t)q & 0xffu;
}
template <bool SIGNED>
__device__ __forceinline__ uint32_t epi_pack4(float y0, float y1, float y2, float y3) {
  int i0, i1, i2, i3;
  asm("cvt.rni.s32.f32 %0, %1;" : "=r"(i0) : "f"(y0));
  asm("cvt.rni.s32.f32 %0, %1;" : "=r"(i1) : "f"(y1));
  asm("cvt.rni.s32.f32 %0, %1;" : "=r"(i2) : "f"(y2));
  asm("cvt.rni.s32.f32 %0, %1;" : "=r"(i3) : "f"(y3));
  uint32_t hi2, w;
  if (SIGNED) {
    asm("cvt.pack.sat.s8.s32.b32 %0, %1, %2, 0;" : "=r"(hi2) : "r"(i3), "r"(i2));
    asm("cvt.pack.sat.s8.s32.b32 %0, %1, %2, %3;" : "=r"(w) : "r"(i1), "r"(i0), "r"(hi2));
  } else {
    asm("cvt.pack.sat.u8.s32.b32 %0, %1, %2, 0;" : "=r"(hi2) : "r"(i3), "r"(i2));
    asm("cvt.pack.sat.u8.s32.b32 %0, %1, %2, %3;" : "=r"(w) : "r"(i1), "r"(i0), "r"(hi2));
  }
  return w;
}

}
```

semilayer-wise-mixed-precision-quantization_b200/slq_build.py:

```python
import hashlib
import os
import subprocess
import sys

HERE = os.path.dirname(os.path.abspath(__file__))
ROOT = os.path.dirname(HERE)
CSRC = os.path.join(HERE, "csrc")
LIB = os.path.join(HERE, "libslq_b200.so")
STAMP = os.path.join(HERE, "build", "sources.sha256")
SOURCES = ["quantizer.cu", "layers.cu", "conv_umma.cu", "stem_umma.cu", "eval_tail.cu", "probe.cu", "tail_umma.cu",
           "block_tail.cu"]
NVCC_FLAGS = [
    "-gencode", "arch=compute_100a,code=sm_100a", "-lineinfo", "-O3", "-std=c++17",
    "-Xcompiler", "-fPIC", "-Xcompiler", "-fvisibility=hidden",
    "-I", os.path.join(ROOT, "include"), "-I", CSRC,
]


def _digest():
    h = hashlib.sha256()
    names = sorted(os.listdir(CSRC)) + ["../../include/slq.h"]
    for n in names:
        p = os.path.join(CSRC, n)
        if os.path.isfile(p):
            h.update(n.encode())
            h.update(open(p, "rb").read())
    h.update(" ".join(f.replace(ROOT, "<root>") for f in NVCC_FLAGS).encode())
    return h.hexdigest()


def needs_build():
    if not os.path.exists(LIB) or not os.path.exists(STAMP):
        return True
    return open(STAMP).read().strip() != _digest()


def build(force=False, verbose=False, debug=False):
    if debug:
        return _build_debug(verbose)
    if not force and not needs_build():
        return LIB
    os.makedirs(os.path.join(HERE, "build"), exist_ok=True)
    import fcntl
    with open(os.path.join(HERE, "build", ".lock"), "w") as lock:
        fcntl.flock(lock, fcntl.LOCK_EX)
        if not force and not needs_build():
            return LIB
        return _build_locked(verbose)


def _build_locked(verbose):
    nvcc = os.environ.get("NVCC", "/usr/local/cuda/bin/nvcc")
    objs = []
    procs = []
    for src in SOURCES:
        obj = os.path.join(HERE, "build", src.replace(".cu", ".o"))
        cmd = [nvcc] + NVCC_FLAGS + ["-c", os.path.join(CSRC, src), "-o", obj]
        if verbose:
            print(" ".join(cmd))
        procs.append((src, subprocess.Popen(cmd, stdout=subprocess.PIPE, stderr=subprocess.STDOUT)))
        objs.append(obj)
    for src, p in procs:
        out, _ = p.communicate()
        if p.returncode != 0:
            sys.stderr.write(out.decode())
            raise RuntimeError("nvcc failed on %s" % src)
    cmd = [nvcc, "-shared", "-o", LIB + ".tmp"] + objs + ["-gencode", "arch=compute_100a,code=sm_100a"]
    subprocess.check_call(cmd)
    os.replace(LIB + ".tmp", LIB)
    with open(STAMP, "w") as f:
        f.write(_digest())
    return LIB


LIB_DBG = os.path.join(HERE, "libslq_b200_dbg.so")


def _build_debug(verbose=False):
    stamp = os.path.join(HERE, "build", "dbg", "sources.sha256")
    if os.path.exists(LIB_DBG) and os.path.exists(stamp) and open(stamp).read().strip() == _digest():
        return LIB_DBG
    nvcc = os.environ.get("NVCC", "/usr/local/cuda/bin/nvcc")
    os.makedirs(os.path.join(HERE, "build", "dbg"), exist_ok=True)
    procs, objs = [], []
    for src in SOURCES:
        obj = os.path.join(HERE, "build", "dbg", src.replace(".cu", ".o"))
        cmd = [nvcc] + NVCC_FLAGS + ["-DSLQ_DEBUG_TRACE=1", "-c", os.path.join(CSRC, src), "-o", obj]
        if verbose:
            print(" ".join(cmd))
        procs.append((src, subprocess.Popen(cmd, stdout=subprocess.PIPE, stderr=subprocess.STDOUT)))
        objs.append(obj)
    for src, p in procs:
        out, _ = p.communicate()
        if p.returncode != 0:
            sys.stderr.write(out.decode())
            raise RuntimeError("nvcc failed on %s" % src)
    subprocess.check_call([nvcc, "-shared", "-o", LIB_DBG] + objs + ["-gencode", "arch=compute_100a,code=sm_100a"])
    with open(stamp, "w") as f:
        f.write(_digest())
    return LIB_DBG


def build_variant(name, defines, verbose=False):
    lib = os.path.join(HERE, "libslq_b200_%s.so" % name)
    nvcc = os.environ.get("NVCC", "/usr/local/cuda/bin/nvcc")
    bdir = os.path.join(HERE, "build", name)
    os.makedirs(bdir, exist_ok=True)
    procs, objs = [], []
    for src in SOURCES:
        obj = os.path.join(bdir, src.replace(".cu", ".o"))
        cmd = [nvcc] + NVCC_FLAGS + ["-D%s" % d for d in defines] + ["-c", os.path.join(CSRC, src), "-o", obj]
        if verbose:
            print(" ".join(cmd))
        procs.append((src, subprocess.Popen(cmd, stdout=subprocess.PIPE, stderr=subprocess.STDOUT)))
        objs.append(obj)
    for src, p in procs:
        out, _ = p.communicate()
        if p.returncode != 0:
            sys.stderr.write(out.decode())
            raise RuntimeError("nvcc failed on %s" % src)
    subprocess.check_call([nvcc, "-shared", "-o", lib] + objs + ["-gencode", "arch=compute_100a,code=sm_100a"])
    return lib


if __name__ == "__main__":
    if "--variant" in sys.argv:
        i = sys.argv.index("--variant")
        print(build_variant(sys.argv[i + 1], sys.argv[i + 2:], verbose=True))
        sys.exit(0)
    print(build(force="--force" in sys.argv, verbose=True, debug="--debug" in sys.argv))
```

semilayer-wise-mixed-precision-quantization_b200/slq_engine.py:

```python
import ctypes
import os

import numpy as np
import torch

import slq_lib as L


def engine_batch(net, n):
    for (N, _h, _w, _d), _eng in getattr(net, "_slq_engines", {}).items():
        if N >= n:
            return N
    return n


def _align(v, a):
    return (v + a - 1) // a * a


class PackedLayer:

    def __init__(self, bits, z, s, offsets, blob, K):
        self.bits, self.z, self.s, self.offsets, self.blob, self.K = bits, z, s, offsets, blob, K

    @property
    def nbytes(self):
        return int(self.blob.numel())


def packed_offsets(bits_host, K):
    lib = L.lib()
    sizes = np.array([_align(lib.slq_packed_row_bytes(K, int(b)), 16) for b in bits_host], np.int64)
    offs = np.zeros(len(sizes), np.int64)
    if len(sizes) > 1:
        offs[1:] = np.cumsum(sizes)[:-1]
    return offs, int(sizes.sum())


def classify_weights(weights, stream=None):
    lib = L.lib()
    stream = L.current_stream() if stream is None else stream
    metas = []
    for w in weights:
        rows, K = w.shape[0], w[0].numel()
        meta = torch.empty((2, rows), dtype=torch.int32, device=w.device)
        z = torch.empty(rows, dtype=torch.int32, device=w.device)
        s = torch.empty(rows, dtype=torch.float32, device=w.device)
        L.check(lib.slq_classify_rows(w.data_ptr(), rows, K, meta[0].data_ptr(), z.data_ptr(), s.data_ptr(),
                                      meta[1].data_ptr(), stream))
        metas.append((meta, z, s))
    all_meta = torch.cat([m[0] for m in metas], dim=1).cpu().numpy()
    out, pos = [], 0
    for (meta, z, s) in metas:
        n = meta.shape[1]
        out.append((meta[0], z, s, all_meta[0, pos:pos + n], bool(all_meta[1, pos:pos + n].all())))
        pos += n
    return out


class PackedGemm:

    def __init__(self, blob, tile_base, seg_bytes, row_offsets):
        self.blob, self.tile_base, self.seg_bytes, self.row_offsets = blob, tile_base, seg_bytes, row_offsets
        self.used_bytes = 0

    @property
    def nbytes(self):
        return self.used_bytes


def conv_tiling(desc):
    lib = L.lib()
    v = [ctypes.c_int32(0) for _ in range(5)]
    L.check(lib.slq_conv_tiling(ctypes.byref(desc), *[ctypes.addressof(x) for x in v]))
    return tuple(int(x.value) for x in v)


def alloc_packed_gemm(desc, device):
    bn_cols, n_tiles, k_block, num_kb, resident = conv_tiling(desc)
    if not resident:
        return None
    blob = torch.zeros(bn_cols * n_tiles * k_block * num_kb, dtype=torch.uint8, device=device)
    return PackedGemm(blob, torch.zeros(n_tiles, dtype=torch.int64, device=device),
                      torch.zeros(n_tiles, dtype=torch.int32, device=device),
                      torch.zeros((n_tiles, bn_cols + 1), dtype=torch.int16, device=device))


def build_packed_gemm(desc, packed, bits_host, device, stream=None, into=None):
    lib = L.lib()
    bn_cols, n_tiles, k_block, num_kb, resident = conv_tiling(desc)
    if not resident or int(bits_host.max()) > 8:
        return None
    stream = L.current_stream() if stream is None else stream
    pg = into if into is not None else alloc_packed_gemm(desc, device)
    rows = bn_cols * n_tiles
    bits = np.full(rows, 4, np.int64)
    bits[:len(bits_host)] = bits_host
    seg = np.where(bits <= 4, k_block // 2, k_block).reshape(n_tiles, bn_cols)
    row_off = np.zeros((n_tiles, bn_cols + 1), np.int64)
    row_off[:, 1:] = np.cumsum(seg, axis=1)
    seg_bytes = row_off[:, -1].astype(np.int32)
    tile_base = np.zeros(n_tiles, np.int64)
    tile_base[1:] = np.cumsum(num_kb * seg_bytes.astype(np.int64))[:-1]
    pg.used_bytes = int(num_kb * seg_bytes.astype(np.int64).sum())
    assert row_off.max() < 65536 and pg.used_bytes <= pg.blob.numel()
    pg.tile_base.copy_(torch.from_numpy(tile_base), non_blocking=False)
    pg.seg_bytes.copy_(torch.from_numpy(seg_bytes), non_blocking=False)
    pg.row_offsets.copy_(torch.from_numpy(row_off.astype(np.uint16).view(np.int16)), non_blocking=False)
    L.check(lib.slq_build_packed_gemm_weights(ctypes.byref(desc), packed.blob.data_ptr(), packed.offsets.data_ptr(),
                                              packed.bits.data_ptr(), pg.tile_base.data_ptr(), pg.seg_bytes.data_ptr(),
                                              pg.row_offsets.data_ptr(), pg.blob.data_ptr(), stream))
    return pg


def encode_weight(w, bit, z, s, bits_host, stream=None):
    lib = L.lib()
    stream = L.current_stream() if stream is None else stream
    rows, K = w.shape[0], w[0].numel()
    offs, total = packed_offsets(bits_host, K)
    offsets = torch.from_numpy(offs).to(w.device)
    blob = torch.empty(max(total, 16), dtype=torch.uint8, device=w.device)
    L.check(lib.slq_encode_rows(w.data_ptr(), rows, K, bit.data_ptr(), z.data_ptr(), s.data_ptr(),
                                blob.data_ptr(), offsets.data_ptr(), stream))
    return PackedLayer(bit, z, s, offsets, blob, K)


class _ConvOp:
    pass


class _BlockTail:

    def __init__(self, dop, op3):
        self.dop, self.op3 = dop, op3
        self.handle, self.unsupported, self.fused, self.epi = None, False, False, {}


class Engine:
    def __init__(self, net, N, H, W, device, impl=L.IMPL_UMMA, a_mode=L.A_AUTO, stem="umma", packed_b=True,
                 fuse_tail=True):
        if device.type != "cuda":
            raise RuntimeError("slq Engine needs a CUDA device")
        self.lib = L.lib()
        self.net, self.N, self.H, self.W, self.device = net, N, H, W, device
        self.impl, self.a_mode = impl, a_mode
        self.packed_b = packed_b
        self.fuse_tail = fuse_tail
        self.stem_kind = stem
        self.stem = None
        self.epoch = -1
        self.kernel_launches = 0
        self._graphs, self._seen = {}, set()
        self.use_graphs = os.environ.get("SLQ_NO_GRAPHS") is None
        with torch.cuda.device(device):
            self._plan()

    @classmethod
    def for_module(cls, net, x, **kw):
        key = (tuple(x.shape), x.device.index)
        cached = getattr(net, "_slq_engine", None)
        if cached is None or cached[0] != key:
            eng = cls(net, x.shape[0], x.shape[2], x.shape[3], x.device, **kw)
            net._slq_engine = cached = (key, eng)
        eng = cached[1]
        eng.sync_weights()
        if not eng.calibrated:
            eng.calibrate(x)
        return eng

    def _new_act(self, shape_nhwc, signed=False):
        self.act.append(None)
        self.act_shapes.append(tuple(int(v) for v in shape_nhwc))
        self.act_signed.append(signed)
        return len(self.act) - 1

    def _alloc_acts(self):
        sizes = [_align(int(np.prod(s)), 1024) for s in self.act_shapes]
        self.act_arena = torch.empty(max(sum(sizes), 1024), dtype=torch.uint8, device=self.device)
        off = 0
        for i, (s, n) in enumerate(zip(self.act_shapes, sizes)):
            self.act[i] = self.act_arena[off:off + int(np.prod(s))].view(s)
            off += n

    def _plan(self):
        net, N, dev = self.net, self.N, self.device
        if not net.conv1.weight.is_cuda:
            raise RuntimeError("model parameters must live on the CUDA device (call net.to(device))")
        Hc, Wc = (self.H + 6 - 7) // 2 + 1, (self.W + 6 - 7) // 2 + 1
        Hp, Wp = (Hc + 2 - 3) // 2 + 1, (Wc + 2 - 3) // 2 + 1
        self.act, self.act_shapes, self.act_signed, self.ops, self.tails, self.schedule = [], [], [], [], [], []
        self.stem_scratch = torch.empty(N * Hc * Wc * 64, dtype=torch.float32, device=dev)
        if self.stem_kind == "umma" and Wc > 128:
            self.stem_kind = "simt"
        if self.stem_kind == "umma":
            nbytes = self.lib.slq_stem_workspace_bytes(N, self.H, self.W)
            self.stem_ws = torch.empty(nbytes, dtype=torch.uint8, device=dev)
            h = ctypes.c_void_p()
            L.check(self.lib.slq_stem_create(N, self.H, self.W, self.stem_ws.data_ptr(), ctypes.byref(h)))
            self.stem = h
        x_id = self._new_act((N, Hp, Wp, 64))
        h, w = Hp, Wp
        max_out = N * Hp * Wp * 64
        for stage in (net.layer1, net.layer2, net.layer3, net.layer4):
            for blk in stage:
                convs = [c for c in ("conv1", "conv2", "conv3") if hasattr(blk, c)]
                res_id, res_signed = x_id, False
                cur, ch, cw = x_id, h, w
                pending = []
                for i, cname in enumerate(convs):
                    conv, bn = getattr(blk, cname), getattr(blk, "bn%d" % (i + 1))
                    op = self._make_op(conv, bn, cur, ch, cw, relu=True)
                    pending.append(op)
                    cur, ch, cw = op.out_id, op.Ho, op.Wo
                if blk.downsample is not None:
                    dop = self._make_op(blk.downsample[0], blk.downsample[1], x_id, h, w, relu=False, signed=True)
                    res_id, res_signed = dop.out_id, True
                    pending.insert(len(pending) - 1, dop)
                    if len(convs) == 3 and pending[-1].k == 1 and dop.k == 1:
                        self.tails.append(_BlockTail(dop, pending[-1]))
                last = pending[-1]
                last.res_id, last.res_signed = res_id, res_signed
                self.ops += pending
                x_id, h, w = last.out_id, last.Ho, last.Wo
        self._alloc_acts()
        for op in self.ops:
            max_out = max(max_out, op.M * op.Cout)
        self.final_id, self.final_hw, self.final_c = x_id, h * w, self.act[x_id].shape[3]
        self.rowsum, self.rowsum_planes = {}, {}
        self.f32_scratch = torch.empty(max_out, dtype=torch.float32, device=dev)
        self.act_scales = torch.ones(len(self.act), dtype=torch.float32, device=dev)
        self.absmax_tmp = torch.zeros(1, dtype=torch.int32, device=dev)
        self.tail_ws = torch.empty(self.lib.slq_tail_workspace_bytes(N, self.final_c, net.fc.out_features) // 4,
                                   dtype=torch.float32, device=dev)
        self.logits = torch.empty((N, net.fc.out_features), dtype=torch.float32, device=dev)
        self.stem_w = torch.zeros_like(net.conv1.weight, dtype=torch.float32, device=dev)
        self.stem_a = torch.zeros(64, dtype=torch.float32, device=dev)
        self.stem_b = torch.zeros(64, dtype=torch.float32, device=dev)
        self.fc_w = torch.zeros_like(net.fc.weight, dtype=torch.float32, device=dev)
        self.fc_w_split = torch.zeros((2,) + tuple(net.fc.weight.shape), dtype=torch.float32, device=dev)
        self.fc_b = torch.zeros_like(net.fc.bias, dtype=torch.float32, device=dev)
        self.ends_sig = None
        self.weights_version = 0
        self.calibrated = False
        self.calib_hw = (self.H, self.W)
        self._graphs, self._seen = {}, set()

    def adopt_scales(self, other):
        self.act_scales.copy_(other.act_scales)
        self.calibrated = True

    def _make_op(self, conv, bn, in_id, h, w, relu, signed=False):
        op = _ConvOp()
        op.conv, op.bn, op.in_id, op.relu, op.signed = conv, bn, in_id, relu, signed
        op.Cin, op.Cout = conv.in_channels, conv.out_channels
        op.k, op.stride, op.pad = conv.kernel_size[0], conv.stride[0], conv.padding[0]
        op.H, op.W = h, w
        op.Ho = (h + 2 * op.pad - op.k) // op.stride + 1
        op.Wo = (w + 2 * op.pad - op.k) // op.stride + 1
        op.M = self.N * op.Ho * op.Wo
        op.out_id = self._new_act((self.N, op.Ho, op.Wo, op.Cout), signed)
        op.res_id, op.res_signed = -1, False
        op.handle, op.w16 = None, None
        op.variants = {}
        op.packed_gemm = None
        op.wsig = op.bsig = None
        dev = self.device
        op.wscale = torch.zeros(op.Cout, dtype=torch.float32, device=dev)
        op.zf = torch.zeros(op.Cout, dtype=torch.float32, device=dev)
        op.bias = torch.zeros(op.Cout, dtype=torch.float32, device=dev)
        op.epi = {}
        return op

    @staticmethod
    def _sig(*tensors):
        import resnet
        return tuple((t.data_ptr(), t._version, resnet.weight_write_count(t)) for t in tensors)

    @staticmethod
    def _bn_tensors(bn):
        return (bn.weight, bn.bias, bn.running_mean, bn.running_var)

    def refresh_weights(self):
        self.sync_weights(force=True)

    def sync_weights(self, force=False):
        import resnet
        lib, dev = self.lib, self.device
        if self.epoch != resnet.WEIGHT_EPOCH[0]:
            force = True
            self.epoch = resnet.WEIGHT_EPOCH[0]
        todo, bn_todo = [], []
        for op in self.ops:
            wsig = self._sig(op.conv.weight)
            bsig = self._sig(*self._bn_tensors(op.bn))
            if force or wsig != op.wsig:
                todo.append((op, wsig, bsig))
            elif bsig != op.bsig:
                bn_todo.append((op, bsig))
        ends_sig = self._sig(self.net.conv1.weight, *self._bn_tensors(self.net.bn1), self.net.fc.weight, self.net.fc.bias)
        if not todo and not bn_todo and ends_sig == self.ends_sig and not force:
            return 0
        with torch.cuda.device(dev), torch.no_grad():
            stream = L.current_stream(dev)
            if todo:
                ws = [op.conv.weight.detach().to(torch.float32).reshape(op.Cout, -1).contiguous() for op, _, _ in todo]
                metas = classify_weights(ws, stream)
                for (op, wsig, bsig), w2d, (bit, z, s, bits_host, exact) in zip(todo, ws, metas):
                    op.packed = encode_weight(w2d, bit, z, s, bits_host, stream)
                    op.bits_host, op.packed_exact = bits_host, exact
                    w16 = 1 if int(bits_host.max()) > 8 else 0
                    var = op.variants.get(w16)
                    if var is None:
                        desc = L.ConvDesc(self.N, op.H, op.W, op.Cin, op.Cout, op.k, op.k, op.stride, op.pad,
                                          w16, self.impl, self.a_mode)
                        rows = lib.slq_gemm_weight_rows(ctypes.byref(desc))
                        wg = torch.empty((rows, op.k * op.k * op.Cin), dtype=torch.uint8, device=dev)
                        h = ctypes.c_void_p()
                        L.check(lib.slq_conv_create(ctypes.byref(desc), self.act[op.in_id].data_ptr(),
                                                    wg.data_ptr(), ctypes.byref(h)))
                        pgbuf = None
                        if w16 == 0 and self.packed_b and self.impl == L.IMPL_UMMA:
                            pgbuf = alloc_packed_gemm(desc, dev)
                            if pgbuf is not None:
                                L.check(lib.slq_conv_set_packed_weights(h, pgbuf.blob.data_ptr(), pgbuf.tile_base.data_ptr(),
                                                                        pgbuf.seg_bytes.data_ptr(), pgbuf.row_offsets.data_ptr()))
                        var = op.variants[w16] = (desc, wg, h, pgbuf)
                    desc, wg, h, pgbuf = var
                    L.check(lib.slq_build_gemm_weights(ctypes.byref(desc), op.packed.blob.data_ptr(),
                                                       op.packed.offsets.data_ptr(), op.packed.bits.data_ptr(),
                                                       wg.data_ptr(), stream))
                    if pgbuf is not None:
                        build_packed_gemm(desc, op.packed, bits_host, dev, stream, into=pgbuf)
                    if op.w16 != w16:
                        self._graphs, self._seen = {}, set()
                    op.packed_gemm = pgbuf
                    op.handle, op.w16, op.desc, op.wg = h, w16, desc, wg
                    op.s_dev, op.z_dev = s, z
                    self._fold_into(op)
                    op.wsig, op.bsig = wsig, bsig
            for op, bsig in bn_todo:
                self._fold_into(op)
                op.bsig = bsig
            if force or ends_sig != self.ends_sig:
                self.stem_w.copy_(self.net.conv1.weight.detach())
                if self.stem is not None:
                    L.check(lib.slq_stem_set_weights(self.stem, self.stem_w.data_ptr(), stream))
                a, b = self._fold_bn(self.net.bn1)
                self.stem_a.copy_(a)
                self.stem_b.copy_(b)
                self.fc_w.copy_(self.net.fc.weight.detach())
                L.check(lib.slq_tail_split_weights(self.fc_w.data_ptr(), self.fc_w.shape[0], self.fc_w.shape[1],
                                                   self.fc_w_split.data_ptr(), stream))
                self.fc_b.copy_(self.net.fc.bias.detach())
                self.ends_sig = ends_sig
        changed = False
        for bt in self.tails:
            want = self.fuse_tail and bt.op3.w16 == 0 and bt.dop.w16 == 1 and not bt.unsupported
            if want and bt.handle is None:
                dop, op3 = bt.dop, bt.op3
                desc = L.BlockTailDesc(self.N, dop.H, dop.W, dop.Cin, dop.stride, op3.Cin, op3.Cout, self.impl)
                h = ctypes.c_void_p()
                rc = lib.slq_blocktail_create(ctypes.byref(desc), self.act[op3.in_id].data_ptr(),
                                              self.act[dop.in_id].data_ptr(), op3.variants[0][1].data_ptr(),
                                              dop.variants[1][1].data_ptr(), ctypes.byref(h))
                if rc == L.SLQ_ERR_UNSUPPORTED:
                    bt.unsupported, want = True, False
                else:
                    L.check(rc)
                    bt.handle = h
            if want != bt.fused:
                bt.fused, changed = want, True
        inside = {id(o): bt for bt in self.tails if bt.fused for o in (bt.dop, bt.op3)}
        self.schedule = []
        for op in self.ops:
            bt = inside.get(id(op))
            if bt is None:
                self.schedule.append(("conv", op))
            elif op is bt.op3:
                self.schedule.append(("tail", bt))
        need = {op.in_id for kind, op in self.schedule if kind == "conv"
                and lib.slq_conv_needs_rowsum(op.handle, 1 if op.res_id >= 0 else 0)}
        planes = {0: 1}
        for kind, it in self.schedule:
            if kind == "tail":
                planes[it.op3.out_id] = max(int(lib.slq_blocktail_rowsum_planes(it.handle)), 1)
            elif not it.signed:
                planes[it.out_id] = max(int(lib.slq_conv_rowsum_planes(it.handle, 1 if it.res_id >= 0 else 0)), 1)
        changed = changed or set(self.rowsum) != need
        for i in need:
            if i not in self.rowsum:
                n_, h_, w_, c_ = self.act[i].shape
                self.rowsum[i] = torch.zeros((max(c_ // 64, 1), n_ * h_ * w_), dtype=torch.int32, device=dev)
            if self.rowsum_planes.get(i) != planes[i]:
                self.rowsum_planes[i], changed = planes[i], True
        for i in [i for i in self.rowsum if i not in need]:
            del self.rowsum[i]
            self.rowsum_planes.pop(i, None)
        if changed:
            for op in self.ops:
                op.epi = {}
            for bt in self.tails:
                bt.epi = {}
            self._graphs, self._seen = {}, set()
        self.weights_version += 1
        return len(todo)

    def _fold_into(self, op):
        a, b = self._fold_bn(op.bn)
        op.wscale.copy_(op.s_dev * a)
        op.zf.copy_(op.z_dev.to(torch.float32))
        op.bias.copy_(b)

    @staticmethod
    def _fold_bn(bn):
        a = (bn.weight.detach() / torch.sqrt(bn.running_var.detach() + bn.eps)).to(torch.float32)
        b = (bn.bias.detach() - bn.running_mean.detach() * a).to(torch.float32)
        return a.contiguous(), b.contiguous()

    def _epilogue(self, op, mode, out_ptr, out_S=None):
        key = (mode, out_ptr)
        e = op.epi.get(key)
        if e is None:
            res = self.act[op.res_id].data_ptr() if op.res_id >= 0 else None
            rs_out = self.rowsum.get(op.out_id) if mode == L.OUT_U8 else None
            rs_in = self.rowsum.get(op.in_id)
            e = L.Epilogue(op.wscale.data_ptr(), op.zf.data_ptr(), op.bias.data_ptr(),
                           self.act_scales.data_ptr(), op.in_id, op.out_id, op.res_id, res,
                           1 if op.res_signed else 0, out_ptr, out_S, mode, 1 if op.relu else 0,
                           L.ptr(rs_in), L.ptr(rs_out), self.rowsum_planes.get(op.in_id, 0),
                           rs_in.shape[1] if rs_in is not None else 0)
            op.epi[key] = e
        return e

    def _tail_epilogue(self, bt, mode, out_ptr):
        key = (mode, out_ptr)
        e = bt.epi.get(key)
        if e is None:
            o3, od = bt.op3, bt.dop
            rs_out = self.rowsum.get(o3.out_id) if mode == L.OUT_U8 else None
            e = L.BlockTailEpilogue(o3.wscale.data_ptr(), o3.zf.data_ptr(), o3.bias.data_ptr(),
                                    od.wscale.data_ptr(), od.zf.data_ptr(), od.bias.data_ptr(),
                                    self.act_scales.data_ptr(), o3.in_id, od.in_id, o3.out_id, out_ptr, mode,
                                    L.ptr(rs_out))
            bt.epi[key] = e
        return e

    def launch_item(self, item, st, mode=None, out_ptr=None):
        kind, it = item
        if kind == "tail":
            mode = L.OUT_U8 if mode is None else mode
            out_ptr = self.act[it.op3.out_id].data_ptr() if out_ptr is None else out_ptr
            L.check(self.lib.slq_blocktail_launch(it.handle, ctypes.byref(self._tail_epilogue(it, mode, out_ptr)), st))
        else:
            mode = (L.OUT_S8 if it.signed else L.OUT_U8) if mode is None else mode
            out_ptr = self.act[it.out_id].data_ptr() if out_ptr is None else out_ptr
            L.check(self.lib.slq_conv_launch(it.handle, ctypes.byref(self._epilogue(it, mode, out_ptr)), st))

    def item_info(self, item):
        kind, it = item
        if kind == "tail":
            o3, od = it.op3, it.dop
            return dict(kind="tail", Cin=od.Cin, Cmid=o3.Cin, Cout=o3.Cout, k=1, stride=od.stride, H=od.H, M=o3.M,
                        w16=1, res=0, ops=2.0 * o3.M * o3.Cout * (o3.Cin + od.Cin),
                        bytes=self.act[o3.in_id].numel() + self.act[od.in_id].numel() + self.act[o3.out_id].numel()
                        + o3.wg.numel() + od.wg.numel())
        return dict(kind="conv", Cin=it.Cin, Cmid=0, Cout=it.Cout, k=it.k, stride=it.stride, H=it.H, M=it.M,
                    w16=it.w16, res=1 if it.res_id >= 0 else 0, ops=2.0 * it.M * it.Cout * it.k * it.k * it.Cin,
                    bytes=self.act[it.in_id].numel() + self.act[it.out_id].numel() + it.wg.numel()
                    + (self.act[it.res_id].numel() if it.res_id >= 0 else 0))

    IN_KINDS = {torch.float32: L.IN_F32, torch.float16: L.IN_F16, torch.uint8: L.IN_U8}

    def _check_x(self, x):
        if tuple(x.shape) != (self.N, 3, self.H, self.W) or x.dtype not in self.IN_KINDS or not x.is_cuda:
            raise ValueError("engine compiled for fp32 / fp16 / u8 CUDA input %s, got %s %s" %
                             ((self.N, 3, self.H, self.W), tuple(x.shape), x.dtype))
        kind = self.IN_KINDS[x.dtype]
        if kind != L.IN_F32 and self.stem is None:
            raise ValueError("fp16 / u8 inputs need the tensor-core stem (input width <= 256)")
        if kind == L.IN_U8:
            norm = getattr(self.net, "input_norm", None)
            if norm is None:
                raise ValueError("u8 input needs net.input_norm = (mean[3], std[3])")
            self.norm = (ctypes.c_float * 6)(*[float(v) for v in tuple(norm[0]) + tuple(norm[1])])
        self.in_kind = kind
        return x.contiguous()

    def calibrate(self, x, accumulate=False, headroom=1.0):
        lib = self.lib
        x = self._check_x(x)
        if any(op.handle is None for op in self.ops):
            raise RuntimeError("engine has no packed weights yet (call sync_weights())")
        accumulate = accumulate and self.calibrated
        with torch.cuda.device(self.device), torch.no_grad():
            st = L.current_stream(self.device)
            sc, tmp, f32 = self.act_scales.data_ptr(), self.absmax_tmp.data_ptr(), self.f32_scratch
            old = self.act_scales.clone() if accumulate else None

            def settle(idx):
                if headroom != 1.0:
                    self.act_scales[idx:idx + 1].mul_(headroom)
                if old is not None:
                    torch.maximum(self.act_scales[idx:idx + 1], old[idx:idx + 1], out=self.act_scales[idx:idx + 1])

            n0 = self.act[0].numel()
            self._stem(x.data_ptr(), f32.data_ptr(), L.OUT_F32, st)
            L.check(lib.slq_absmax_scale(f32.data_ptr(), n0, sc, 0, 255, tmp, st))
            settle(0)
            self._stem(x.data_ptr(), self.act[0].data_ptr(), L.OUT_U8, st)
            for item in self.schedule:
                op = item[1].op3 if item[0] == "tail" else item[1]
                if item[0] == "tail":
                    dop = item[1].dop
                    self.launch_item(("conv", dop), st, L.OUT_F32, f32.data_ptr())
                    L.check(lib.slq_absmax_scale(f32.data_ptr(), dop.M * dop.Cout, sc, dop.out_id, 127, tmp, st))
                    settle(dop.out_id)
                self.launch_item(item, st, L.OUT_F32, f32.data_ptr())
                L.check(lib.slq_absmax_scale(f32.data_ptr(), op.M * op.Cout, sc, op.out_id,
                                             127 if op.signed else 255, tmp, st))
                settle(op.out_id)
                self.launch_item(item, st)
        self.calibrated = True

    def forward(self, x):
        if not self.calibrated:
            raise RuntimeError("engine is not calibrated (call calibrate(x) after refresh_weights())")
        x = self._check_x(x)
        key = (x.data_ptr(), self.in_kind)
        g = self._graphs.get(key)
        if g is None and self.use_graphs:
            if key in self._seen:
                if len(self._graphs) >= 4:
                    self._graphs.pop(next(iter(self._graphs)))
                g = self._graphs[key] = self._capture(x)
            else:
                if len(self._seen) > 64:
                    self._seen.clear()
                self._seen.add(key)
        if g is not None:
            g.replay()
        else:
            self.launch_all(x.data_ptr(), L.current_stream(self.device))
        return self.logits

    def launch_all(self, x_ptr, st):
        lib = self.lib
        sc = self.act_scales.data_ptr()
        self._stem(x_ptr, self.act[0].data_ptr(), L.OUT_U8, st)
        for item in self.schedule:
            self.launch_item(item, st)
        L.check(lib.slq_tail_forward(self.act[self.final_id].data_ptr(), self.N, self.final_hw, self.final_c,
                                     sc, self.final_id, self.fc_w_split.data_ptr(), self.fc_b.data_ptr(),
                                     self.logits.shape[1], self.tail_ws.data_ptr(), self.logits.data_ptr(), st))
        self.kernel_launches = (1 if self.stem is not None else 2) + len(self.schedule) + 3

    def _stem(self, x_ptr, out_ptr, mode, st):
        lib, sc = self.lib, self.act_scales.data_ptr()
        if self.stem is not None:
            kind = getattr(self, "in_kind", L.IN_F32)
            norm = ctypes.cast(self.norm, ctypes.c_void_p) if kind == L.IN_U8 else None
            L.check(lib.slq_stem_launch_in(self.stem, x_ptr, kind, norm, self.stem_a.data_ptr(), self.stem_b.data_ptr(),
                                           sc, 0, out_ptr, mode, self.stem_scratch.data_ptr(),
                                           L.ptr(self.rowsum.get(0)), st))
        else:
            L.check(lib.slq_stem_forward(x_ptr, self.N, self.H, self.W, self.stem_w.data_ptr(),
                                         self.stem_a.data_ptr(), self.stem_b.data_ptr(), sc, 0,
                                         self.stem_scratch.data_ptr(), out_ptr, mode, L.ptr(self.rowsum.get(0)), st))

    def capture_graph(self, x_static):
        x_static = self._check_x(x_static)
        self.graph, self.graph_x = self._capture(x_static), x_static
        return self.graph

    def _capture(self, x_static):
        g = torch.cuda.CUDAGraph()
        s = torch.cuda.Stream(self.device)
        s.wait_stream(torch.cuda.current_stream(self.device))
        with torch.cuda.stream(s):
            self.launch_all(x_static.data_ptr(), s.cuda_stream)
        torch.cuda.current_stream(self.device).wait_stream(s)
        torch.cuda.synchronize(self.device)
        with torch.cuda.graph(g, stream=s, capture_error_mode="thread_local"):
            self.launch_all(x_static.data_ptr(), torch.cuda.current_stream(self.device).cuda_stream)
        return g

    def weight_bytes(self):
        return sum(op.packed.nbytes for op in self.ops)

    def describe(self):
        rows = []
        for op in self.ops:
            bits, counts = np.unique(op.bits_host, return_counts=True)
            rows.append(dict(Cin=op.Cin, Cout=op.Cout, k=op.k, stride=op.stride, H=op.H, M=op.M, w16=op.w16,
                             bits={int(b): int(c) for b, c in zip(bits, counts)}))
        return rows

    def __del__(self):
        try:
            for op in getattr(self, "ops", []):
                for _desc, _wg, h, _pg in getattr(op, "variants", {}).values():
                    self.lib.slq_conv_destroy(h)
                op.variants, op.handle = {}, None
            for bt in getattr(self, "tails", []):
                if bt.handle is not None:
                    self.lib.slq_blocktail_destroy(bt.handle)
                    bt.handle = None
            if getattr(self, "stem", None) is not None:
                self.lib.slq_stem_destroy(self.stem)
                self.stem = None
        except Exception:
            pass
```

semilayer-wise-mixed-precision-quantization_b200/slq_lib.py:

```python
import ctypes
import os

HERE = os.path.dirname(os.path.abspath(__file__))
LIB_PATH = os.path.join(HERE, "libslq_b200.so")

SLQ_OK, SLQ_ERR_INVALID, SLQ_ERR_CUDA, SLQ_ERR_ZERO_RANGE, SLQ_ERR_UNSUPPORTED = 0, 1, 2, 3, 4
ROW_OK, ROW_ZERO_RANGE, ROW_CODE_RANGE = 0, 1, 2
DIV_TRUE, DIV_RECIP = 0, 1
IMPL_UMMA, IMPL_SIMT = 0, 1
A_AUTO, A_IM2COL, A_TILED = 0, 1, 2
OUT_U8, OUT_F32, OUT_ACC, OUT_S8 = 0, 1, 2, 3
IN_F32, IN_F16, IN_U8 = 0, 1, 2

_i32, _i64, _vp = ctypes.c_int32, ctypes.c_int64, ctypes.c_void_p


class ConvDesc(ctypes.Structure):
    _fields_ = [(n, _i32) for n in
                ("N", "H", "W", "Cin", "Cout", "kh", "kw", "stride", "pad", "w16", "impl", "a_mode")]


class Epilogue(ctypes.Structure):
    _fields_ = [("wscale", _vp), ("zf", _vp), ("bias", _vp), ("act_scales", _vp),
                ("in_id", _i32), ("out_id", _i32), ("res_id", _i32),
                ("res", _vp), ("res_signed", _i32),
                ("out", _vp), ("out_S", _vp), ("out_mode", _i32), ("relu", _i32),
                ("in_rowsum", _vp), ("out_rowsum", _vp), ("in_planes", _i32), ("in_plane_stride", _i64)]


class BlockTailDesc(ctypes.Structure):
    _fields_ = [(n, _i32) for n in ("N", "H", "W", "Cin", "stride", "Cmid", "Cout", "impl")]


class BlockTailEpilogue(ctypes.Structure):
    _fields_ = [("wscale3", _vp), ("zf3", _vp), ("bias3", _vp), ("wscaled", _vp), ("zfd", _vp), ("biasd", _vp),
                ("act_scales", _vp), ("in3_id", _i32), ("ind_id", _i32), ("out_id", _i32),
                ("out", _vp), ("out_mode", _i32), ("out_rowsum", _vp)]


SIGNATURES = {
    "slq_last_error": (ctypes.c_char_p, []),
    "slq_abi_version": (ctypes.c_int, []),
    "slq_device_info": (ctypes.c_int, [_vp, _vp, _vp]),
    "slq_packed_row_bytes": (_i64, [_i64, _i32]),
    "slq_quantize_rows": (ctypes.c_int, [_vp, _i64, _i64, _vp, _vp, _i32, _i32, _i32, _vp, _vp, _vp, _vp, _vp, _vp]),
    "slq_quantize_rows_host": (ctypes.c_int, [_vp, _i64, _i64, _vp, _vp, _i32, _i32, _i32, _vp, _vp, _vp, _vp, _vp]),
    "slq_quantize_jobs": (ctypes.c_int, [_vp, _i32, _i32, _i32, _i32, _i32, _vp, _vp, _vp, _vp]),
    "slq_decode_rows": (ctypes.c_int, [_vp, _vp, _vp, _vp, _vp, _i64, _i64, _vp, _vp]),
    "slq_eval_tail": (ctypes.c_int, [_vp, _vp, _i32, _i32, _vp, _vp, _vp, _vp, _vp]),
    "slq_kl_rows": (ctypes.c_int, [_vp, _vp, _i32, _i32, _vp, _vp, _vp]),
    "slq_probe_i8_peak": (ctypes.c_int, [_i32, ctypes.POINTER(_i64), _vp]),
    "slq_classify_rows": (ctypes.c_int, [_vp, _i64, _i64, _vp, _vp, _vp, _vp, _vp]),
    "slq_encode_rows": (ctypes.c_int, [_vp, _i64, _i64, _vp, _vp, _vp, _vp, _vp, _vp]),
    "slq_gemm_weight_rows": (_i64, [ctypes.POINTER(ConvDesc)]),
    "slq_build_gemm_weights": (ctypes.c_int, [ctypes.POINTER(ConvDesc), _vp, _vp, _vp, _vp, _vp]),
    "slq_conv_create": (ctypes.c_int, [ctypes.POINTER(ConvDesc), _vp, _vp, ctypes.POINTER(_vp)]),
    "slq_conv_destroy": (None, [_vp]),
    "slq_conv_tiling": (ctypes.c_int, [ctypes.POINTER(ConvDesc), _vp, _vp, _vp, _vp, _vp]),
    "slq_build_packed_gemm_weights": (ctypes.c_int, [ctypes.POINTER(ConvDesc), _vp, _vp, _vp, _vp, _vp, _vp, _vp, _vp]),
    "slq_conv_set_packed_weights": (ctypes.c_int, [_vp, _vp, _vp, _vp, _vp]),
    "slq_conv_launch": (ctypes.c_int, [_vp, ctypes.POINTER(Epilogue), _vp]),
    "slq_blocktail_create": (ctypes.c_int, [ctypes.POINTER(BlockTailDesc), _vp, _vp, _vp, _vp, ctypes.POINTER(_vp)]),
    "slq_blocktail_destroy": (None, [_vp]),
    "slq_blocktail_rowsum_planes": (_i32, [_vp]),
    "slq_blocktail_launch": (ctypes.c_int, [_vp, ctypes.POINTER(BlockTailEpilogue), _vp]),
    "slq_debug_set_trace": (ctypes.c_int, [_vp, _i32]),
    "slq_stem_forward": (ctypes.c_int, [_vp, _i32, _i32, _i32, _vp, _vp, _vp, _vp, _i32, _vp, _vp, _i32, _vp, _vp]),
    "slq_conv_rowsum_planes": (_i32, [_vp, _i32]),
    "slq_conv_needs_rowsum": (_i32, [_vp, _i32]),
    "slq_stem_workspace_bytes": (_i64, [_i32, _i32, _i32]),
    "slq_stem_create": (ctypes.c_int, [_i32, _i32, _i32, _vp, ctypes.POINTER(_vp)]),
    "slq_stem_destroy": (None, [_vp]),
    "slq_stem_set_weights": (ctypes.c_int, [_vp, _vp, _vp]),
    "slq_stem_launch": (ctypes.c_int, [_vp, _vp, _vp, _vp, _vp, _i32, _vp, _i32, _vp, _vp, _vp]),
    "slq_stem_launch_in": (ctypes.c_int, [_vp, _vp, _i32, _vp, _vp, _vp, _vp, _i32, _vp, _i32, _vp, _vp, _vp]),
    "slq_tail_workspace_bytes": (_i64, [_i32, _i32, _i32]),
    "slq_tail_split_weights": (ctypes.c_int, [_vp, _i32, _i32, _vp, _vp]),
    "slq_tail_forward": (ctypes.c_int, [_vp, _i32, _i32, _i32, _vp, _i32, _vp, _vp, _i32, _vp, _vp, _vp]),
    "slq_absmax_scale": (ctypes.c_int, [_vp, _i64, _vp, _i32, _i32, _vp, _vp]),
    "slq_quantize_act": (ctypes.c_int, [_vp, _i64, _vp, _i32, _i32, _vp, _vp]),
}

_lib = None


class SlqError(RuntimeError):
    def __init__(self, code, msg):
        super().__init__("libslq_b200: error %d: %s" % (code, msg))
        self.code = code


def lib():
    global _lib, LIB_PATH
    if _lib is None:
        if os.environ.get("SLQ_DEBUG_LIB") == "1":
            import slq_build
            LIB_PATH = slq_build.build(debug=True)
        elif os.environ.get("SLQ_LIB_VARIANT"):
            LIB_PATH = os.path.join(HERE, "libslq_b200_%s.so" % os.environ["SLQ_LIB_VARIANT"])
        if not os.path.exists(LIB_PATH):
            raise RuntimeError(
                "libslq_b200.so is missing (%s). Build it with `python slq_build.py`; this package "
                "has no CPU or eager-PyTorch fallback." % LIB_PATH)
        L = ctypes.CDLL(LIB_PATH)
        for name, (res, args) in SIGNATURES.items():
            fn = getattr(L, name)
            fn.restype = res
            fn.argtypes = args
        if L.slq_abi_version() != 1:
            raise RuntimeError("libslq_b200.so ABI version mismatch")
        _lib = L
    return _lib


def check(rc):
    if rc != SLQ_OK:
        msg = lib().slq_last_error()
        raise SlqError(rc, msg.decode() if msg else "")


def ptr(t):
    return None if t is None else t.data_ptr()


def current_stream(device=None):
    import torch
    return torch.cuda.current_stream(device).cuda_stream
```

Before: 124,300.

## Fuse 3x3 conv and following 1x1 conv with residual into one chain kernel

Adds a persistent UMMA kernel that computes a bottleneck's 3x3 conv (Cmid=64), quantizes the intermediate into shared memory, then runs the 1x1 expansion conv with the residual add and output quantization. The intermediate activation no longer round-trips through global memory, and one launch replaces two. A warp-specialized pipeline with TMA im2col loads, double-buffered TMEM accumulators and a residual prefetch ring is meant to overlap the two GEMMs. It is enabled automatically when the M-tile count covers all SMs, and it restricts shapes and requires that downstream ops do not need rowsums.

```diff
diff --git a/include/slq.h b/include/slq.h
--- a/include/slq.h
+++ b/include/slq.h
@@ -154,6 +154,31 @@
 SLQ_API int32_t slq_blocktail_rowsum_planes(const slq_blocktail *h);
 SLQ_API int slq_blocktail_launch(slq_blocktail *h, const slq_blocktail_epilogue *e, void *stream);
 
+typedef struct slq_chain_desc {
+  int32_t N, H, W;
+  int32_t Cin;
+  int32_t Cmid;
+  int32_t Cout;
+  int32_t k, stride;
+  int32_t impl;
+} slq_chain_desc;
+
+typedef struct slq_chain slq_chain;
+
+typedef struct slq_chain_epilogue {
+  const float *wscale2, *zf2, *bias2;
+  const float *wscale3, *zf3, *bias3;
+  const float *act_scales;
+  int32_t in_id, mid_id, res_id, out_id;
+  void *out;
+  int32_t out_mode;
+} slq_chain_epilogue;
+
+SLQ_API int slq_chain_create(const slq_chain_desc *d, const uint8_t *x, const uint8_t *res, const uint8_t *wg2,
+                             const uint8_t *wg3, slq_chain **out);
+SLQ_API void slq_chain_destroy(slq_chain *h);
+SLQ_API int slq_chain_launch(slq_chain *h, const slq_chain_epilogue *e, void *stream);
+
 
 SLQ_API int slq_stem_forward(const float *x, int32_t N, int32_t H, int32_t W, const float *w,
                      const float *bn_a, const float *bn_b, const float *act_scales, int32_t out_id,
diff --git a/semilayer-wise-mixed-precision-quantization_b200/csrc/block_tail.cu b/semilayer-wise-mixed-precision-quantization_b200/csrc/block_tail.cu
--- a/semilayer-wise-mixed-precision-quantization_b200/csrc/block_tail.cu
+++ b/semilayer-wise-mixed-precision-quantization_b200/csrc/block_tail.cu
@@ -363,15 +363,7 @@
   else reinterpret_cast<float *>(a.out)[m * a.Cout + oc] = fmaxf(y, 0.f);
 }
 
-typedef CUresult (*BtEncodeTiledFn)(CUtensorMap *, CUtensorMapDataType, cuuint32_t, void *, const cuuint64_t *,
-                                    const cuuint64_t *, const cuuint32_t *, const cuuint32_t *, CUtensorMapInterleave,
-                                    CUtensorMapSwizzle, CUtensorMapL2promotion, CUtensorMapFloatOOBfill);
-typedef CUresult (*BtEncodeIm2colFn)(CUtensorMap *, CUtensorMapDataType, cuuint32_t, void *, const cuuint64_t *,
-                                     const cuuint64_t *, const int *, const int *, cuuint32_t, cuuint32_t,
-                                     const cuuint32_t *, CUtensorMapInterleave, CUtensorMapSwizzle,
-                                     CUtensorMapL2promotion, CUtensorMapFloatOOBfill);
-
-static int bt_encoders(BtEncodeTiledFn *tiled, BtEncodeIm2colFn *im2col) {
+int bt_encoders(BtEncodeTiledFn *tiled, BtEncodeIm2colFn *im2col) {
   static BtEncodeTiledFn f_tiled = nullptr;
   static BtEncodeIm2colFn f_im2col = nullptr;
   if (!f_tiled || !f_im2col) {
@@ -390,7 +382,7 @@
   return SLQ_OK;
 }
 
-static int bt_tiled_u8(CUtensorMap *tm, const void *ptr, long long rows, int cols, int box_cols, int box_rows,
+int bt_tiled_u8(CUtensorMap *tm, const void *ptr, long long rows, int cols, int box_cols, int box_rows,
                        CUtensorMapSwizzle sw, const char *what) {
   BtEncodeTiledFn enc;
   BtEncodeIm2colFn enc2;
diff --git a/semilayer-wise-mixed-precision-quantization_b200/csrc/chain_umma.cu b/semilayer-wise-mixed-precision-quantization_b200/csrc/chain_umma.cu
--- /dev/null
+++ b/semilayer-wise-mixed-precision-quantization_b200/csrc/chain_umma.cu
@@ -0,0 +1,482 @@
+#include <algorithm>
+#include <new>
+
+#include "conv_common.cuh"
+#include "umma_ptx.cuh"
+
+struct slq_chain {
+  slq_chain_desc d;
+  long long M;
+  int grid;
+  CUtensorMap tmA, tmB2, tmB3, tmR, tmO;
+  const void *out_ptr;
+};
+
+namespace slq {
+
+constexpr int kChThreads = 640;
+constexpr int kChCrew = 512;
+constexpr int kChCmid = 64, kChCout = 256;
+constexpr int kChN2 = kChCmid + 16;
+constexpr int kChTaps = 9;
+constexpr int kChStages = 4;
+constexpr int kChResBufs = 3;
+constexpr int kChResBytes = kTileM * kChCout;
+constexpr int kChW2 = 0;
+constexpr int kChW3 = kChW2 + kChTaps * kChN2 * 64;
+constexpr int kChRing = kChW3 + kChCout * 64;
+constexpr int kChMid = kChRing + kChStages * kTileM * 64;
+constexpr int kChRes = kChMid + 2 * kTileM * 64;
+constexpr int kChPrm = kChRes + kChResBufs * kChResBytes;
+constexpr int kChS3 = kChPrm + 3 * (kChCout + kChCmid) * 4;
+constexpr int kChBar = kChS3 + 3 * 4 * kTileM * 4;
+constexpr int kChSmem = 1024 + kChBar + 512;
+static_assert(kChSmem <= 232448, "chain kernel: shared-memory plan");
+static_assert(kChRes % 1024 == 0 && kChMid % 1024 == 0 && kChRing % 1024 == 0, "swizzled tiles need 1024-B alignment");
+
+struct ChArgs {
+  long long M;
+  int H, W, m_tiles;
+  const float *wscale2, *zf2, *bias2, *wscale3, *zf3, *bias3, *act_scales;
+  int in_id, mid_id, res_id, out_id;
+  float *out_f32;
+  long long *stats;
+};
+
+__device__ __forceinline__ void ch_wait(uint32_t bar, uint32_t parity, long long *acc, bool on) {
+  if (!kDebugTrace || !on) { mbar_wait(bar, parity); return; }
+  const long long t0 = clock64();
+  mbar_wait(bar, parity);
+  *acc += clock64() - t0;
+}
+
+template <int OUT>
+__global__ void __launch_bounds__(kChThreads, 1)
+chain_kernel(const __grid_constant__ CUtensorMap tmA, const __grid_constant__ CUtensorMap tmB2,
+             const __grid_constant__ CUtensorMap tmB3, const __grid_constant__ CUtensorMap tmR,
+             const __grid_constant__ CUtensorMap tmO, const ChArgs a) {
+  extern __shared__ uint8_t smem_raw[];
+  const uint32_t sb = (smem_u32(smem_raw) + 1023u) & ~1023u;
+  uint8_t *smem = smem_raw + (sb - smem_u32(smem_raw));
+  const uint32_t bar = sb + kChBar;
+  auto full_bar = [&](int s) { return bar + 8u * s; };
+  auto empty_bar = [&](int s) { return bar + 8u * (4 + s); };
+  auto tfull2_bar = [&](int p) { return bar + 8u * (8 + p); };
+  auto tempty2_bar = [&](int p) { return bar + 8u * (10 + p); };
+  auto midfull_bar = [&](int p) { return bar + 8u * (12 + p); };
+  const uint32_t tfull3_bar = bar + 8u * 14, tempty3_bar = bar + 8u * 15;
+  auto rfull_bar = [&](int r) { return bar + 8u * (16 + r); };
+  auto rempty_bar = [&](int r) { return bar + 8u * (19 + r); };
+  const uint32_t bfull_bar = bar + 8u * 22;
+  volatile uint32_t *tmem_slot = reinterpret_cast<volatile uint32_t *>(smem + kChBar + 8 * 24);
+  const int warp = __shfl_sync(0xffffffffu, (int)(threadIdx.x >> 5), 0), lane = threadIdx.x & 31;
+  constexpr bool kQuant = OUT == SLQ_OUT_U8;
+
+  const int first_m = (int)blockIdx.x, step_m = (int)gridDim.x;
+  const int count = first_m < a.m_tiles ? (a.m_tiles - first_m + step_m - 1) / step_m : 0;
+  const bool st_on = kDebugTrace && a.stats != nullptr && blockIdx.x == 0;
+
+  asm volatile("griddepcontrol.launch_dependents;" ::: "memory");
+  if (warp == 0 && lane == 0) {
+    prefetch_tmap(&tmA); prefetch_tmap(&tmB2); prefetch_tmap(&tmB3); prefetch_tmap(&tmR);
+    if (kQuant) prefetch_tmap(&tmO);
+  }
+  if (warp == 1 && lane == 0) {
+    for (int s = 0; s < kChStages; ++s) { mbar_init(full_bar(s), 1); mbar_init(empty_bar(s), 1); }
+    for (int p = 0; p < 2; ++p) {
+      mbar_init(tfull2_bar(p), 1);
+      mbar_init(tempty2_bar(p), kChCrew / 32);
+      mbar_init(midfull_bar(p), kChCrew / 32);
+    }
+    mbar_init(tfull3_bar, 1);
+    mbar_init(tempty3_bar, kChCrew / 32);
+    for (int r = 0; r < kChResBufs; ++r) { mbar_init(rfull_bar(r), 1); mbar_init(rempty_bar(r), 1); }
+    mbar_init(bfull_bar, 1);
+    fence_barrier_init();
+  }
+  if (warp == 2) {
+    asm volatile("tcgen05.alloc.cta_group::1.sync.aligned.shared::cta.b32 [%0], %1;" ::"r"(
+                     smem_u32((const void *)tmem_slot)), "r"(512) : "memory");
+    asm volatile("tcgen05.relinquish_alloc_permit.cta_group::1.sync.aligned;" ::: "memory");
+  }
+  for (int i = threadIdx.x; i < kChTaps * 16 * 4; i += blockDim.x) {
+    const int t = i >> 6, row = (i >> 2) & 15, chunk = i & 3;
+    const uint4 v = row == 0 ? make_uint4(0x01010101u, 0x01010101u, 0x01010101u, 0x01010101u) : make_uint4(0, 0, 0, 0);
+    *reinterpret_cast<uint4 *>(smem + kChW2 + t * (kChN2 * 64) + (kChCmid + row) * 64 + chunk * 16) = v;
+  }
+  fence_proxy_async_smem();
+  tc_fence_before();
+  __syncthreads();
+  tc_fence_after();
+  const uint32_t tmem_base = *tmem_slot;
+
+  if (warp == 0 || warp == 2) {
+    const int w = warp >> 1;
+    if (w == 0 && count > 0) {
+      if (elect_one()) {
+        mbar_expect_tx(bfull_bar, (uint32_t)(kChTaps * kChCmid * 64 + kChCout * 64));
+        for (int kb = 0; kb < kChTaps; ++kb)
+          tma_load_2d(sb + kChW2 + kb * (kChN2 * 64), &tmB2, bfull_bar, kb * 64, 0);
+        tma_load_2d(sb + kChW3, &tmB3, bfull_bar, 0, 0);
+      }
+      __syncwarp();
+    }
+    grid_dependency_wait();
+    const int hw = a.H * a.W, steps = count * kChTaps;
+    int cur = -1, cn = 0, cw = 0, chh = 0;
+    long long w_empty = 0;
+    for (int c = w; c < steps; c += 2) {
+      const int i = c / kChTaps, tap = c - i * kChTaps;
+      if (i != cur) {
+        cur = i;
+        const int m0 = (first_m + i * step_m) * kTileM;
+        cn = m0 / hw;
+        const int rem = m0 - cn * hw, ph = rem / a.W;
+        cw = rem - ph * a.W - 1;
+        chh = ph - 1;
+      }
+      const int s = c & (kChStages - 1);
+      ch_wait(empty_bar(s), (uint32_t)(((c / kChStages) & 1) ^ 1), &w_empty, st_on);
+      if (elect_one()) {
+        mbar_expect_tx(full_bar(s), kTileM * 64);
+        const int tr = tap / 3;
+        tma_load_im2col_4d(sb + kChRing + s * (kTileM * 64), &tmA, full_bar(s), 0, cw, chh, cn, (uint16_t)(tap - 3 * tr),
+                           (uint16_t)tr);
+      }
+      __syncwarp();
+    }
+    if (st_on && lane == 0) a.stats[w] = w_empty;
+  } else if (warp == 3) {
+    grid_dependency_wait();
+    long long w_empty = 0;
+    for (int i = 0; i < count; ++i) {
+      const int r = i % kChResBufs;
+      ch_wait(rempty_bar(r), (uint32_t)(((i / kChResBufs) & 1) ^ 1), &w_empty, st_on);
+      if (elect_one()) {
+        const int m0 = (first_m + i * step_m) * kTileM;
+        const uint32_t dst = sb + kChRes + r * kChResBytes;
+        mbar_expect_tx(rfull_bar(r), kChResBytes);
+        tma_load_2d(dst, &tmR, rfull_bar(r), 0, m0);
+        tma_load_2d(dst + kTileM * 128, &tmR, rfull_bar(r), 128, m0);
+      }
+      __syncwarp();
+    }
+    if (st_on && lane == 0) a.stats[2] = w_empty;
+  } else if (warp == 1) {
+    const uint32_t tm = __shfl_sync(0xffffffffu, tmem_base, 0);
+    const uint32_t idesc2 = (2u << 4) | ((uint32_t)(kChN2 >> 3) << 17) | ((uint32_t)(kTileM >> 4) << 24);
+    const uint32_t idesc3 = (2u << 4) | ((uint32_t)(kChCout >> 3) << 17) | ((uint32_t)(kTileM >> 4) << 24);
+    if (count > 0) {
+      mbar_wait(bfull_bar, 0);
+      tc_fence_after();
+    }
+    long long w_full = 0, w_acc2 = 0, w_mid = 0, w_acc3 = 0;
+    int c = 0;
+    auto conv2 = [&](int t) {
+      const int p = t & 1;
+      if (t >= 2) ch_wait(tempty2_bar(p), (uint32_t)(((t - 2) >> 1) & 1), &w_acc2, st_on);
+      tc_fence_after();
+      for (int kb = 0; kb < kChTaps; ++kb, ++c) {
+        const int s = c & (kChStages - 1);
+        ch_wait(full_bar(s), (uint32_t)((c / kChStages) & 1), &w_full, st_on);
+        tc_fence_after();
+        if (elect_one()) {
+          const uint64_t da = make_smem_desc<64>(sb + kChRing + s * (kTileM * 64));
+          const uint64_t db = make_smem_desc<64>(sb + kChW2 + kb * (kChN2 * 64));
+          umma_i8(tm + p * 128, da, db, idesc2, (uint32_t)(kb != 0));
+          umma_i8(tm + p * 128, da + 2, db + 2, idesc2, 1u);
+          umma_commit(empty_bar(s));
+          if (kb == kChTaps - 1) umma_commit(tfull2_bar(p));
+        }
+        __syncwarp();
+      }
+    };
+    auto conv3 = [&](int t) {
+      const int p = t & 1;
+      ch_wait(midfull_bar(p), (uint32_t)((t >> 1) & 1), &w_mid, st_on);
+      if (t >= 1) ch_wait(tempty3_bar, (uint32_t)((t - 1) & 1), &w_acc3, st_on);
+      tc_fence_after();
+      if (elect_one()) {
+        const uint64_t da = make_smem_desc<64>(sb + kChMid + p * (kTileM * 64));
+        const uint64_t db = make_smem_desc<64>(sb + kChW3);
+        umma_i8(tm + 256, da, db, idesc3, 0u);
+        umma_i8(tm + 256, da + 2, db + 2, idesc3, 1u);
+        umma_commit(tfull3_bar);
+      }
+      __syncwarp();
+    };
+    for (int t = 0; t < count; ++t) {
+      conv2(t);
+      if (t >= 1) conv3(t - 1);
+    }
+    if (count > 0) conv3(count - 1);
+    if (st_on && lane == 0) { a.stats[3] = w_full; a.stats[4] = w_acc2; a.stats[5] = w_mid; a.stats[6] = w_acc3; }
+  } else if (warp >= 4) {
+    grid_dependency_wait();
+    const int slice = (warp - 4) >> 2;
+    const int wq = warp & 3;
+    const int et = threadIdx.x - 128;
+    const int row = wq * 32 + lane;
+    float *prm = reinterpret_cast<float *>(smem + kChPrm);
+    const uint32_t prm3 = sb + kChPrm, prm2 = sb + kChPrm + 3 * kChCout * 4;
+    volatile uint32_t *s3buf = reinterpret_cast<volatile uint32_t *>(smem + kChS3);
+    const float s_mid = a.act_scales[a.mid_id];
+    const float inv_mid = __fdiv_rn(1.0f, s_mid);
+    const float inv_out = kQuant ? __fdiv_rn(1.0f, a.act_scales[a.out_id]) : 1.0f;
+    const float s_res = kQuant ? __fmul_rn(a.act_scales[a.res_id], inv_out) : a.act_scales[a.res_id];
+    if (et < kChCout) {
+      const ChanParam p = make_chan_param(a.wscale3[et], a.zf3[et], a.bias3[et], s_mid, inv_out, kQuant);
+      prm[et] = p.wsc; prm[kChCout + et] = p.zw; prm[2 * kChCout + et] = p.bias;
+    } else if (et < kChCout + kChCmid) {
+      const int oc = et - kChCout;
+      const ChanParam p = make_chan_param(a.wscale2[oc], a.zf2[oc], a.bias2[oc], a.act_scales[a.in_id], inv_mid, true);
+      prm[3 * kChCout + oc] = p.wsc; prm[3 * kChCout + kChCmid + oc] = p.zw; prm[3 * kChCout + 2 * kChCmid + oc] = p.bias;
+    }
+    named_bar_sync(1, kChCrew);
+    const uint32_t tlane = tmem_base + ((uint32_t)(wq * 32) << 16);
+    const uint32_t row_sw64 = (uint32_t)((row >> 1) & 3), row_sw128 = (uint32_t)(row & 7);
+    long long w_t2 = 0, w_t3 = 0, w_res = 0;
+
+    auto mid = [&](int t) {
+      const int p = t & 1;
+      ch_wait(tfull2_bar(p), (uint32_t)((t >> 1) & 1), &w_t2, st_on && et == 0);
+      tc_fence_after();
+      uint32_t acc[16];
+      tmem_ld16(tlane + p * 128 + slice * 16, acc);
+      const uint32_t S = tmem_ld1(tlane + p * 128 + kChCmid);
+      tmem_ld_wait();
+      tc_fence_before();
+      __syncwarp();
+      if (lane == 0) mbar_arrive(tempty2_bar(p));
+      const float2 S2 = make_float2((float)S, (float)S);
+      uint32_t pk[4];
+#pragma unroll
+      for (int q4 = 0; q4 < 4; ++q4) {
+        const uint32_t pofs = prm2 + (uint32_t)(slice * 16 + 4 * q4) * 4;
+        const uint4 pa = lds128(pofs), pz = lds128(pofs + kChCmid * 4), pb = lds128(pofs + 2 * kChCmid * 4);
+        const uint32_t pav[4] = {pa.x, pa.y, pa.z, pa.w}, pzv[4] = {pz.x, pz.y, pz.z, pz.w}, pbv[4] = {pb.x, pb.y, pb.z, pb.w};
+        float v[4];
+#pragma unroll
+        for (int b = 0; b < 4; b += 2) {
+          const int j = 4 * q4 + b;
+          const float2 accf = make_float2((float)(int)acc[j], (float)(int)acc[j + 1]);
+          const float2 c2 = ffma2(S2, make_float2(__uint_as_float(pzv[b]), __uint_as_float(pzv[b + 1])),
+                                  make_float2(__uint_as_float(pbv[b]), __uint_as_float(pbv[b + 1])));
+          const float2 y = ffma2(accf, make_float2(__uint_as_float(pav[b]), __uint_as_float(pav[b + 1])), c2);
+          v[b] = y.x; v[b + 1] = y.y;
+        }
+        pk[q4] = epi_pack4<false>(v[0], v[1], v[2], v[3]);
+      }
+      sts128(sb + kChMid + p * (kTileM * 64) + row * 64 + (((uint32_t)slice ^ row_sw64) << 4),
+             make_uint4(pk[0], pk[1], pk[2], pk[3]));
+      s3buf[(t % 3) * 512 + slice * kTileM + row] =
+          __dp4a(pk[0], 0x01010101u, __dp4a(pk[1], 0x01010101u, __dp4a(pk[2], 0x01010101u, __dp4a(pk[3], 0x01010101u, 0u))));
+      fence_proxy_async_smem();
+      __syncwarp();
+      if (lane == 0) mbar_arrive(midfull_bar(p));
+      named_bar_sync(1, kChCrew);
+    };
+
+    auto out = [&](int t) {
+      const int r = t % kChResBufs;
+      const int m_tile = first_m + t * step_m;
+      const long long m = (long long)m_tile * kTileM + row;
+      const bool valid = m < a.M;
+      ch_wait(tfull3_bar, (uint32_t)(t & 1), &w_t3, st_on && et == 0);
+      tc_fence_after();
+      ch_wait(rfull_bar(r), (uint32_t)((t / kChResBufs) & 1), &w_res, st_on && et == 0);
+      const volatile uint32_t *s3p = s3buf + (t % 3) * 512 + row;
+      const float S3 = (float)(s3p[0] + s3p[kTileM] + s3p[2 * kTileM] + s3p[3 * kTileM]);
+      const float2 S2 = make_float2(S3, S3), R2 = make_float2(s_res, s_res);
+      const uint32_t slot = sb + kChRes + r * kChResBytes;
+      const uint32_t rrow = slot + (uint32_t)(slice >> 1) * (kTileM * 128) + (uint32_t)row * 128;
+#pragma unroll 1
+      for (int u = 0; u < 2; ++u) {
+        const int cb = slice * 64 + u * 32;
+        uint32_t lo[32];
+        tmem_ld32(tlane + 256 + cb, lo);
+        uint32_t rw[8];
+        uint32_t caddr[2];
+#pragma unroll
+        for (int i = 0; i < 2; ++i) {
+          caddr[i] = rrow + (((uint32_t)(((cb & 127) >> 4) + i) ^ row_sw128) << 4);
+          const uint4 v = lds128(caddr[i]);
+          rw[4 * i] = v.x; rw[4 * i + 1] = v.y; rw[4 * i + 2] = v.z; rw[4 * i + 3] = v.w;
+        }
+        tmem_ld_wait();
+        uint32_t pk[8];
+        float4 *of = reinterpret_cast<float4 *>(a.out_f32 + m * kChCout + cb);
+#pragma unroll
+        for (int q4 = 0; q4 < 8; ++q4) {
+          const uint32_t pofs = prm3 + (uint32_t)(cb + 4 * q4) * 4;
+          const uint4 pa = lds128(pofs), pz = lds128(pofs + kChCout * 4), pb = lds128(pofs + 2 * kChCout * 4);
+          const uint32_t pav[4] = {pa.x, pa.y, pa.z, pa.w}, pzv[4] = {pz.x, pz.y, pz.z, pz.w}, pbv[4] = {pb.x, pb.y, pb.z, pb.w};
+          float v[4];
+#pragma unroll
+          for (int b = 0; b < 4; b += 2) {
+            const int j = 4 * q4 + b;
+            const float2 accf = make_float2((float)(int)lo[j], (float)(int)lo[j + 1]);
+            const float2 c2 = ffma2(S2, make_float2(__uint_as_float(pzv[b]), __uint_as_float(pzv[b + 1])),
+                                    make_float2(__uint_as_float(pbv[b]), __uint_as_float(pbv[b + 1])));
+            float2 y = ffma2(accf, make_float2(__uint_as_float(pav[b]), __uint_as_float(pav[b + 1])), c2);
+            y = ffma2(res_pair(rw[q4], b, false), R2, y);
+            v[b] = y.x; v[b + 1] = y.y;
+          }
+          if (kQuant) {
+            pk[q4] = epi_pack4<false>(v[0], v[1], v[2], v[3]);
+          } else if (valid) {
+            of[q4] = make_float4(fmaxf(v[0], 0.f), fmaxf(v[1], 0.f), fmaxf(v[2], 0.f), fmaxf(v[3], 0.f));
+          }
+        }
+        if (kQuant) {
+#pragma unroll
+          for (int i = 0; i < 2; ++i) sts128(caddr[i], make_uint4(pk[4 * i], pk[4 * i + 1], pk[4 * i + 2], pk[4 * i + 3]));
+        }
+      }
+      tc_fence_before();
+      __syncwarp();
+      if (lane == 0) mbar_arrive(tempty3_bar);
+      if (kQuant) fence_proxy_async_smem();
+      named_bar_sync(1, kChCrew);
+      if (et == 0) {
+        if (kQuant) {
+          tma_store_2d(&tmO, slot, 0, m_tile * kTileM);
+          tma_store_2d(&tmO, slot + kTileM * 128, 128, m_tile * kTileM);
+          tma_store_commit();
+          asm volatile("cp.async.bulk.wait_group.read 1;" ::: "memory");
+          if (t >= 1) mbar_arrive(rempty_bar((t - 1) % kChResBufs));
+        } else {
+          mbar_arrive(rempty_bar(r));
+        }
+      }
+    };
+
+    if (count > 0) mid(0);
+    for (int t = 0; t < count; ++t) {
+      if (t + 1 < count) mid(t + 1);
+      out(t);
+    }
+    if (kQuant && et == 0) tma_store_wait_all();
+    if (st_on && et == 0) { a.stats[7] = w_t2; a.stats[8] = w_t3; a.stats[9] = w_res; a.stats[10] = count; }
+  }
+  tc_fence_before();
+  __syncthreads();
+  if (warp == 2) {
+    tc_fence_after();
+    asm volatile("tcgen05.dealloc.cta_group::1.sync.aligned.b32 %0, %1;" ::"r"(tmem_base), "r"(512) : "memory");
+  }
+}
+
+template <int OUT>
+static int ch_launch(slq_chain *h, const ChArgs &a, cudaStream_t st) {
+  static bool attr_done[kMaxDevices] = {false};
+  const int dev = current_device();
+  if (dev >= kMaxDevices || !attr_done[dev]) {
+    SLQ_CUDA(cudaFuncSetAttribute(chain_kernel<OUT>, cudaFuncAttributeMaxDynamicSharedMemorySize, kChSmem));
+    if (dev < kMaxDevices) attr_done[dev] = true;
+  }
+  cudaLaunchConfig_t cfg = {};
+  cfg.gridDim = dim3((unsigned)h->grid);
+  cfg.blockDim = dim3(kChThreads);
+  cfg.dynamicSmemBytes = (size_t)kChSmem;
+  cfg.stream = st;
+  cudaLaunchAttribute attr[1];
+  attr[0].id = cudaLaunchAttributeProgrammaticStreamSerialization;
+  attr[0].val.programmaticStreamSerializationAllowed = 1;
+  cfg.attrs = attr;
+  cfg.numAttrs = 1;
+  SLQ_CUDA(cudaLaunchKernelEx(&cfg, chain_kernel<OUT>, h->tmA, h->tmB2, h->tmB3, h->tmR, h->tmO, a));
+  return SLQ_OK;
+}
+
+}
+
+using namespace slq;
+
+extern "C" int slq_chain_create(const slq_chain_desc *d, const uint8_t *x, const uint8_t *res, const uint8_t *wg2,
+                                const uint8_t *wg3, slq_chain **out) {
+  SLQ_CHECK_ARG(d && x && res && wg2 && wg3 && out, "slq_chain_create: null pointer argument");
+  SLQ_CHECK_ARG(d->N > 0 && d->H > 0 && d->W > 0 && d->Cin > 0 && d->Cmid > 0 && d->Cout > 0,
+                "slq_chain_create: bad shape");
+  SLQ_CHECK_ARG(d->impl == SLQ_IMPL_UMMA || d->impl == SLQ_IMPL_SIMT, "slq_chain_create: impl %d", d->impl);
+  if (d->impl != SLQ_IMPL_UMMA || d->k != 3 || d->stride != 1 || d->Cin != kChCmid || d->Cmid != kChCmid ||
+      d->Cout != kChCout || (long long)d->N * d->H * d->W >= (1LL << 31)) {
+    set_error("slq_chain_create: only the tcgen05 kernel for a 3x3 stride-1 %d -> %d -> %d chain is implemented "
+              "(got impl %d, k %d, stride %d, %d -> %d -> %d)", kChCmid, kChCmid, kChCout, d->impl, d->k, d->stride,
+              d->Cin, d->Cmid, d->Cout);
+    return SLQ_ERR_UNSUPPORTED;
+  }
+  slq_chain *h = new (std::nothrow) slq_chain();
+  SLQ_CHECK_ARG(h != nullptr, "slq_chain_create: out of host memory");
+  h->d = *d;
+  h->M = (long long)d->N * d->H * d->W;
+  h->grid = (int)std::min<long long>(sm_count(), ceil_div(h->M, kTileM));
+  h->out_ptr = nullptr;
+  int rc = bt_tiled_u8(&h->tmB2, wg2, kChCmid, kChTaps * kChCmid, 64, kChCmid, CU_TENSOR_MAP_SWIZZLE_64B, "W2");
+  if (rc == SLQ_OK) rc = bt_tiled_u8(&h->tmB3, wg3, kChCout, kChCmid, 64, kChCout, CU_TENSOR_MAP_SWIZZLE_64B, "W3");
+  if (rc == SLQ_OK) rc = bt_tiled_u8(&h->tmR, res, h->M, kChCout, 128, kTileM, CU_TENSOR_MAP_SWIZZLE_128B, "res");
+  if (rc == SLQ_OK) {
+    BtEncodeTiledFn enc;
+    BtEncodeIm2colFn enc2;
+    rc = bt_encoders(&enc, &enc2);
+    if (rc == SLQ_OK) {
+      cuuint64_t dims[4] = {(cuuint64_t)d->Cin, (cuuint64_t)d->W, (cuuint64_t)d->H, (cuuint64_t)d->N};
+      cuuint64_t strides[3] = {(cuuint64_t)d->Cin, (cuuint64_t)d->W * d->Cin, (cuuint64_t)d->H * d->W * d->Cin};
+      int lower[2] = {-1, -1}, upper[2] = {-1, -1};
+      cuuint32_t es[4] = {1, 1, 1, 1};
+      const CUresult r = enc2(&h->tmA, CU_TENSOR_MAP_DATA_TYPE_UINT8, 4, const_cast<uint8_t *>(x), dims, strides, lower,
+                              upper, 64, (cuuint32_t)kTileM, es, CU_TENSOR_MAP_INTERLEAVE_NONE, CU_TENSOR_MAP_SWIZZLE_64B,
+                              CU_TENSOR_MAP_L2_PROMOTION_L2_256B, CU_TENSOR_MAP_FLOAT_OOB_FILL_NONE);
+      if (r != CUDA_SUCCESS) {
+        set_error("cuTensorMapEncodeIm2col(x) failed: CUresult %d", (int)r);
+        rc = SLQ_ERR_CUDA;
+      }
+      int drv = 0;
+      if (rc == SLQ_OK && cudaDriverGetVersion(&drv) == cudaSuccess && drv <= 13010 &&
+          (long long)d->N * d->H * d->W * d->Cin < 131072)
+        reinterpret_cast<uint64_t *>(&h->tmA)[1] &= ~(1ull << 21);
+    }
+  }
+  if (rc != SLQ_OK) {
+    delete h;
+    return rc;
+  }
+  h->tmO = h->tmR;
+  *out = h;
+  return SLQ_OK;
+}
+
+extern "C" void slq_chain_destroy(slq_chain *h) { delete h; }
+
+extern "C" int slq_chain_launch(slq_chain *h, const slq_chain_epilogue *e, void *stream) {
+  SLQ_CHECK_ARG(h && e, "slq_chain_launch: null handle/epilogue");
+  SLQ_CHECK_ARG(e->wscale2 && e->zf2 && e->bias2 && e->wscale3 && e->zf3 && e->bias3 && e->act_scales && e->out,
+                "slq_chain_launch: epilogue vectors missing");
+  SLQ_CHECK_ARG(e->out_mode == SLQ_OUT_U8 || e->out_mode == SLQ_OUT_F32, "slq_chain_launch: out_mode %d", e->out_mode);
+  SLQ_CHECK_ARG(reinterpret_cast<uintptr_t>(e->out) % 16 == 0, "slq_chain_launch: out must be 16-byte aligned");
+  const slq_chain_desc &d = h->d;
+  ChArgs a{};
+  a.M = h->M; a.H = d.H; a.W = d.W; a.m_tiles = (int)ceil_div(h->M, kTileM);
+  a.wscale2 = e->wscale2; a.zf2 = e->zf2; a.bias2 = e->bias2;
+  a.wscale3 = e->wscale3; a.zf3 = e->zf3; a.bias3 = e->bias3; a.act_scales = e->act_scales;
+  a.in_id = e->in_id; a.mid_id = e->mid_id; a.res_id = e->res_id; a.out_id = e->out_id;
+  a.out_f32 = e->out_mode == SLQ_OUT_F32 ? reinterpret_cast<float *>(e->out) : nullptr;
+  a.stats = nullptr;
+#if SLQ_DEBUG_TRACE
+  {
+    int cap = 0;
+    debug_trace_buffer(&a.stats, &cap);
+    if (cap > -16) a.stats = nullptr;
+  }
+#endif
+  cudaStream_t st = (cudaStream_t)stream;
+  if (e->out_mode == SLQ_OUT_U8) {
+    if (h->out_ptr != e->out) {
+      int rc = bt_tiled_u8(&h->tmO, e->out, h->M, kChCout, 128, kTileM, CU_TENSOR_MAP_SWIZZLE_128B, "out");
+      if (rc != SLQ_OK) return rc;
+      h->out_ptr = e->out;
+    }
+    return ch_launch<SLQ_OUT_U8>(h, a, st);
+  }
+  return ch_launch<SLQ_OUT_F32>(h, a, st);
+}
diff --git a/semilayer-wise-mixed-precision-quantization_b200/csrc/conv_common.cuh b/semilayer-wise-mixed-precision-quantization_b200/csrc/conv_common.cuh
--- a/semilayer-wise-mixed-precision-quantization_b200/csrc/conv_common.cuh
+++ b/semilayer-wise-mixed-precision-quantization_b200/csrc/conv_common.cuh
@@ -43,6 +43,18 @@
 
 void debug_trace_buffer(long long **buf, int *cap);
 
+typedef CUresult (*BtEncodeTiledFn)(CUtensorMap *, CUtensorMapDataType, cuuint32_t, void *, const cuuint64_t *,
+                                    const cuuint64_t *, const cuuint32_t *, const cuuint32_t *, CUtensorMapInterleave,
+                                    CUtensorMapSwizzle, CUtensorMapL2promotion, CUtensorMapFloatOOBfill);
+typedef CUresult (*BtEncodeIm2colFn)(CUtensorMap *, CUtensorMapDataType, cuuint32_t, void *, const cuuint64_t *,
+                                     const cuuint64_t *, const int *, const int *, cuuint32_t, cuuint32_t,
+                                     const cuuint32_t *, CUtensorMapInterleave, CUtensorMapSwizzle,
+                                     CUtensorMapL2promotion, CUtensorMapFloatOOBfill);
+
+int bt_encoders(BtEncodeTiledFn *tiled, BtEncodeIm2colFn *im2col);
+int bt_tiled_u8(CUtensorMap *tm, const void *ptr, long long rows, int cols, int box_cols, int box_rows,
+                CUtensorMapSwizzle sw, const char *what);
+
 int launch_conv_simt(const ConvGeom &g, const uint8_t *in, const uint8_t *wg, const EpiDev &e,
                      cudaStream_t st);
 
diff --git a/semilayer-wise-mixed-precision-quantization_b200/csrc/conv_umma.cu b/semilayer-wise-mixed-precision-quantization_b200/csrc/conv_umma.cu
--- a/semilayer-wise-mixed-precision-quantization_b200/csrc/conv_umma.cu
+++ b/semilayer-wise-mixed-precision-quantization_b200/csrc/conv_umma.cu
@@ -172,15 +172,6 @@
 __device__ __forceinline__ uint32_t stage_off(int r, int c, int bn_ch) {
   return bn_ch == 128 ? (uint32_t)(r * 128 + ((c ^ (r & 7)) << 4))
                       : (uint32_t)(r * 64 + ((c ^ ((r >> 1) & 3)) << 4));
-}
-
-__device__ __forceinline__ float2 res_pair(uint32_t w, int b, bool is_signed) {
-  const uint32_t b0 = (w >> (8 * b)) & 255u, b1 = (w >> (8 * b + 8)) & 255u;
-  if (is_signed) return make_float2((float)(int)(int8_t)b0, (float)(int)(int8_t)b1);
-  if (b == 2) return make_float2((float)b0, (float)b1);
-  const uint32_t m0 = __byte_perm(w, 0x4B000000u, 0x7440), m1 = __byte_perm(w, 0x4B000000u, 0x7441);
-  return ffma2(make_float2(__uint_as_float(m0), __uint_as_float(m1)), make_float2(1.0f, 1.0f),
-               make_float2(-8388608.0f, -8388608.0f));
 }
 
 constexpr int kResNone = 0, kResU8 = 1, kResS8 = 2, kResDyn = 3;
diff --git a/semilayer-wise-mixed-precision-quantization_b200/csrc/epilogue.cuh b/semilayer-wise-mixed-precision-quantization_b200/csrc/epilogue.cuh
--- a/semilayer-wise-mixed-precision-quantization_b200/csrc/epilogue.cuh
+++ b/semilayer-wise-mixed-precision-quantization_b200/csrc/epilogue.cuh
@@ -66,6 +66,15 @@
   return d;
 }
 
+__device__ __forceinline__ float2 res_pair(uint32_t w, int b, bool is_signed) {
+  const uint32_t b0 = (w >> (8 * b)) & 255u, b1 = (w >> (8 * b + 8)) & 255u;
+  if (is_signed) return make_float2((float)(int)(int8_t)b0, (float)(int)(int8_t)b1);
+  if (b == 2) return make_float2((float)b0, (float)b1);
+  const uint32_t m0 = __byte_perm(w, 0x4B000000u, 0x7440), m1 = __byte_perm(w, 0x4B000000u, 0x7441);
+  return ffma2(make_float2(__uint_as_float(m0), __uint_as_float(m1)), make_float2(1.0f, 1.0f),
+               make_float2(-8388608.0f, -8388608.0f));
+}
+
 __device__ __forceinline__ uint32_t epi_quant_u8(float y) {
   uint32_t q;
   asm("cvt.rni.sat.u8.f32 %0, %1;" : "=r"(q) : "f"(y));
diff --git a/semilayer-wise-mixed-precision-quantization_b200/slq_build.py b/semilayer-wise-mixed-precision-quantization_b200/slq_build.py
--- a/semilayer-wise-mixed-precision-quantization_b200/slq_build.py
+++ b/semilayer-wise-mixed-precision-quantization_b200/slq_build.py
@@ -9,7 +9,7 @@
 LIB = os.path.join(HERE, "libslq_b200.so")
 STAMP = os.path.join(HERE, "build", "sources.sha256")
 SOURCES = ["quantizer.cu", "layers.cu", "conv_umma.cu", "stem_umma.cu", "eval_tail.cu", "probe.cu", "tail_umma.cu",
-           "block_tail.cu"]
+           "block_tail.cu", "chain_umma.cu"]
 NVCC_FLAGS = [
     "-gencode", "arch=compute_100a,code=sm_100a", "-lineinfo", "-O3", "-std=c++17",
     "-Xcompiler", "-fPIC", "-Xcompiler", "-fvisibility=hidden",
diff --git a/semilayer-wise-mixed-precision-quantization_b200/slq_engine.py b/semilayer-wise-mixed-precision-quantization_b200/slq_engine.py
--- a/semilayer-wise-mixed-precision-quantization_b200/slq_engine.py
+++ b/semilayer-wise-mixed-precision-quantization_b200/slq_engine.py
@@ -136,9 +136,16 @@
         self.handle, self.unsupported, self.fused, self.epi = None, False, False, {}
 
 
+class _Chain:
+
+    def __init__(self, op2, op3):
+        self.op2, self.op3 = op2, op3
+        self.handle, self.unsupported, self.fused, self.epi = None, False, False, {}
+
+
 class Engine:
     def __init__(self, net, N, H, W, device, impl=L.IMPL_UMMA, a_mode=L.A_AUTO, stem="umma", packed_b=True,
-                 fuse_tail=True):
+                 fuse_tail=True, fuse_chain="auto"):
         if device.type != "cuda":
             raise RuntimeError("slq Engine needs a CUDA device")
         self.lib = L.lib()
@@ -146,6 +153,9 @@
         self.impl, self.a_mode = impl, a_mode
         self.packed_b = packed_b
         self.fuse_tail = fuse_tail
+        if fuse_chain == "auto" and os.environ.get("SLQ_FUSE_CHAIN") in ("0", "1"):
+            fuse_chain = os.environ["SLQ_FUSE_CHAIN"] == "1"
+        self.fuse_chain = fuse_chain
         self.stem_kind = stem
         self.stem = None
         self.epoch = -1
@@ -189,6 +199,7 @@
         Hc, Wc = (self.H + 6 - 7) // 2 + 1, (self.W + 6 - 7) // 2 + 1
         Hp, Wp = (Hc + 2 - 3) // 2 + 1, (Wc + 2 - 3) // 2 + 1
         self.act, self.act_shapes, self.act_signed, self.ops, self.tails, self.schedule = [], [], [], [], [], []
+        self.chains = []
         self.stem_scratch = torch.empty(N * Hc * Wc * 64, dtype=torch.float32, device=dev)
         if self.stem_kind == "umma" and Wc > 128:
             self.stem_kind = "simt"
@@ -218,6 +229,8 @@
                     pending.insert(len(pending) - 1, dop)
                     if len(convs) == 3 and pending[-1].k == 1 and dop.k == 1:
                         self.tails.append(_BlockTail(dop, pending[-1]))
+                elif len(convs) == 3 and pending[1].k == 3 and pending[1].stride == 1:
+                    self.chains.append(_Chain(pending[1], pending[2]))
                 last = pending[-1]
                 last.res_id, last.res_signed = res_id, res_signed
                 self.ops += pending
@@ -370,21 +383,45 @@
                     bt.handle = h
             if want != bt.fused:
                 bt.fused, changed = want, True
+        sms = torch.cuda.get_device_properties(dev).multi_processor_count
+        for ch in self.chains:
+            op2, op3 = ch.op2, ch.op3
+            if self.fuse_chain == "auto":
+                want = (op3.M + 127) // 128 >= sms
+            else:
+                want = bool(self.fuse_chain)
+            want = (want and self.impl == L.IMPL_UMMA and op2.w16 == 0 and op3.w16 == 0 and not ch.unsupported
+                    and not any(lib.slq_conv_needs_rowsum(o.handle, 1 if o.res_id >= 0 else 0)
+                                for o in self.ops if o.in_id == op3.out_id))
+            if want and ch.handle is None:
+                desc = L.ChainDesc(self.N, op2.H, op2.W, op2.Cin, op2.Cout, op3.Cout, op2.k, op2.stride, self.impl)
+                h = ctypes.c_void_p()
+                rc = lib.slq_chain_create(ctypes.byref(desc), self.act[op2.in_id].data_ptr(),
+                                          self.act[op3.res_id].data_ptr(), op2.variants[0][1].data_ptr(),
+                                          op3.variants[0][1].data_ptr(), ctypes.byref(h))
+                if rc == L.SLQ_ERR_UNSUPPORTED:
+                    ch.unsupported, want = True, False
+                else:
+                    L.check(rc)
+                    ch.handle = h
+            if want != ch.fused:
+                ch.fused, changed = want, True
         inside = {id(o): bt for bt in self.tails if bt.fused for o in (bt.dop, bt.op3)}
+        inside.update({id(o): ch for ch in self.chains if ch.fused for o in (ch.op2, ch.op3)})
         self.schedule = []
         for op in self.ops:
-            bt = inside.get(id(op))
-            if bt is None:
+            it = inside.get(id(op))
+            if it is None:
                 self.schedule.append(("conv", op))
-            elif op is bt.op3:
-                self.schedule.append(("tail", bt))
+            elif op is it.op3:
+                self.schedule.append(("tail" if isinstance(it, _BlockTail) else "chain", it))
         need = {op.in_id for kind, op in self.schedule if kind == "conv"
                 and lib.slq_conv_needs_rowsum(op.handle, 1 if op.res_id >= 0 else 0)}
         planes = {0: 1}
         for kind, it in self.schedule:
             if kind == "tail":
                 planes[it.op3.out_id] = max(int(lib.slq_blocktail_rowsum_planes(it.handle)), 1)
-            elif not it.signed:
+            elif kind == "conv" and not it.signed:
                 planes[it.out_id] = max(int(lib.slq_conv_rowsum_planes(it.handle, 1 if it.res_id >= 0 else 0)), 1)
         changed = changed or set(self.rowsum) != need
         for i in need:
@@ -399,7 +436,7 @@
         if changed:
             for op in self.ops:
                 op.epi = {}
-            for bt in self.tails:
+            for bt in self.tails + self.chains:
                 bt.epi = {}
             self._graphs, self._seen = {}, set()
         self.weights_version += 1
@@ -445,9 +482,24 @@
             bt.epi[key] = e
         return e
 
+    def _chain_epilogue(self, ch, mode, out_ptr):
+        key = (mode, out_ptr)
+        e = ch.epi.get(key)
+        if e is None:
+            o2, o3 = ch.op2, ch.op3
+            e = L.ChainEpilogue(o2.wscale.data_ptr(), o2.zf.data_ptr(), o2.bias.data_ptr(),
+                                o3.wscale.data_ptr(), o3.zf.data_ptr(), o3.bias.data_ptr(),
+                                self.act_scales.data_ptr(), o2.in_id, o2.out_id, o3.res_id, o3.out_id, out_ptr, mode)
+            ch.epi[key] = e
+        return e
+
     def launch_item(self, item, st, mode=None, out_ptr=None):
         kind, it = item
-        if kind == "tail":
+        if kind == "chain":
+            mode = L.OUT_U8 if mode is None else mode
+            out_ptr = self.act[it.op3.out_id].data_ptr() if out_ptr is None else out_ptr
+            L.check(self.lib.slq_chain_launch(it.handle, ctypes.byref(self._chain_epilogue(it, mode, out_ptr)), st))
+        elif kind == "tail":
             mode = L.OUT_U8 if mode is None else mode
             out_ptr = self.act[it.op3.out_id].data_ptr() if out_ptr is None else out_ptr
             L.check(self.lib.slq_blocktail_launch(it.handle, ctypes.byref(self._tail_epilogue(it, mode, out_ptr)), st))
@@ -458,6 +510,12 @@
 
     def item_info(self, item):
         kind, it = item
+        if kind == "chain":
+            o2, o3 = it.op2, it.op3
+            return dict(kind="chain", Cin=o2.Cin, Cmid=o2.Cout, Cout=o3.Cout, k=o2.k, stride=o2.stride, H=o2.H, M=o3.M,
+                        w16=0, res=1, ops=2.0 * o2.M * o2.Cout * o2.k * o2.k * o2.Cin + 2.0 * o3.M * o3.Cout * o3.Cin,
+                        bytes=self.act[o2.in_id].numel() + self.act[o3.res_id].numel() + self.act[o3.out_id].numel()
+                        + o2.wg.numel() + o3.wg.numel())
         if kind == "tail":
             o3, od = it.op3, it.dop
             return dict(kind="tail", Cin=od.Cin, Cmid=o3.Cin, Cout=o3.Cout, k=1, stride=od.stride, H=od.H, M=o3.M,
@@ -508,7 +566,9 @@
             L.check(lib.slq_absmax_scale(f32.data_ptr(), n0, sc, 0, 255, tmp, st))
             settle(0)
             self._stem(x.data_ptr(), self.act[0].data_ptr(), L.OUT_U8, st)
-            for item in self.schedule:
+            items = [sub for item in self.schedule
+                     for sub in ((("conv", item[1].op2), ("conv", item[1].op3)) if item[0] == "chain" else (item,))]
+            for item in items:
                 op = item[1].op3 if item[0] == "tail" else item[1]
                 if item[0] == "tail":
                     dop = item[1].dop
@@ -605,6 +665,10 @@
                 if bt.handle is not None:
                     self.lib.slq_blocktail_destroy(bt.handle)
                     bt.handle = None
+            for ch in getattr(self, "chains", []):
+                if ch.handle is not None:
+                    self.lib.slq_chain_destroy(ch.handle)
+                    ch.handle = None
             if getattr(self, "stem", None) is not None:
                 self.lib.slq_stem_destroy(self.stem)
                 self.stem = None
diff --git a/semilayer-wise-mixed-precision-quantization_b200/slq_lib.py b/semilayer-wise-mixed-precision-quantization_b200/slq_lib.py
--- a/semilayer-wise-mixed-precision-quantization_b200/slq_lib.py
+++ b/semilayer-wise-mixed-precision-quantization_b200/slq_lib.py
@@ -38,6 +38,16 @@
                 ("out", _vp), ("out_mode", _i32), ("out_rowsum", _vp)]
 
 
+class ChainDesc(ctypes.Structure):
+    _fields_ = [(n, _i32) for n in ("N", "H", "W", "Cin", "Cmid", "Cout", "k", "stride", "impl")]
+
+
+class ChainEpilogue(ctypes.Structure):
+    _fields_ = [("wscale2", _vp), ("zf2", _vp), ("bias2", _vp), ("wscale3", _vp), ("zf3", _vp), ("bias3", _vp),
+                ("act_scales", _vp), ("in_id", _i32), ("mid_id", _i32), ("res_id", _i32), ("out_id", _i32),
+                ("out", _vp), ("out_mode", _i32)]
+
+
 SIGNATURES = {
     "slq_last_error": (ctypes.c_char_p, []),
     "slq_abi_version": (ctypes.c_int, []),
@@ -64,6 +74,9 @@
     "slq_blocktail_destroy": (None, [_vp]),
     "slq_blocktail_rowsum_planes": (_i32, [_vp]),
     "slq_blocktail_launch": (ctypes.c_int, [_vp, ctypes.POINTER(BlockTailEpilogue), _vp]),
+    "slq_chain_create": (ctypes.c_int, [ctypes.POINTER(ChainDesc), _vp, _vp, _vp, _vp, ctypes.POINTER(_vp)]),
+    "slq_chain_destroy": (None, [_vp]),
+    "slq_chain_launch": (ctypes.c_int, [_vp, ctypes.POINTER(ChainEpilogue), _vp]),
     "slq_debug_set_trace": (ctypes.c_int, [_vp, _i32]),
     "slq_stem_forward": (ctypes.c_int, [_vp, _i32, _i32, _i32, _vp, _vp, _vp, _vp, _i32, _vp, _vp, _i32, _vp, _vp]),
     "slq_conv_rowsum_planes": (_i32, [_vp, _i32]),
```

Result: faster. 129,400, median of 6 (+4.1%).
